# pairlab/SlotFormer

Hardware: AMD Instinct MI355X
Metric: rollout frames/sec at B=32, 128x128, 7 slots, 6+50 steps (SAVi-encode + SlotFormer rollout) (higher is better)
Workload: dtype f32 storage; matmul/conv on split-bf16 MFMA (bf16x3: hi*hi+hi*lo+lo*hi, f32 accumulate)

## Files before the change

include/slotformer_hip.h:

```cpp
#ifndef SLOTFORMER_HIP_H
#define SLOTFORMER_HIP_H
#include <stddef.h>

#ifdef __cplusplus
extern "C" {
#endif

int sf_version(void);
const char* sf_last_error_string(void);

int sf_get_precision(void);
int sf_set_precision(int mode);

int sf_profile_enable(int class_mask);
int sf_set_seam_fused(int on);
int sf_get_seam_fused(void);
int sf_set_ffn_rows64(int on);
int sf_get_ffn_rows64(void);
int sf_profile_sample(int every);
int sf_profile_read(int kernel_class, double* total_ms, long long* launches, double* work);


int sf_linear_f32(const float* A, int lda, const float* W, const float* bias, const float* ln_gamma,
                  const float* ln_beta, float ln_eps, const float* residual, int ldr, float* C, int ldc,
// ... 76 lines not shown
int sf_rle_label_maps(const unsigned* run_ends, const int* object_offsets, const int* frame_offsets, const void* tables, long long* labels_i64,
                      unsigned char* labels_u8, int* extents, int F, int num_objects, int num_runs, int h, int w, int H, int W, void* stream);
int sf_rle_boxes_pad(const int* extents, float* bbox, unsigned char* pres_mask, unsigned* flag, int F, int num, void* stream);

enum { SF_EGRESS_TRUNC = 0, SF_EGRESS_NEAREST_EVEN = 1 };
enum { SF_EGRESS_F32_CHW = 0, SF_EGRESS_U8_CHW = 1, SF_EGRESS_U8_HWC = 2 };
enum { SF_EGRESS_IMG = 0, SF_EGRESS_SLOTS = 1, SF_EGRESS_IDS = 2 };
int sf_egress_frames_u8(const float* x, unsigned char* out, long long F, int H, int W, int hwc, int to_rgb, int rounding, void* stream);
typedef struct {
  int kind;
  int N;
  const void* a;
  const void* b;
  float scale;
  int ids_i64;
  int P;
  int history_len;
} sf_egress_tile;
int sf_egress_grid_shape(int K, int H, int W, int nrow, int padding, int border, int* CH, int* CW);
int sf_egress_grid(const sf_egress_tile* tiles, int n_entries, void* out, int out_mode, int T, int H, int W, int nrow, int padding,
                   float pad_value, int border, void* stream);
int sf_egress_draw_boxes(unsigned char* frames, const float* boxes, const unsigned char* pres, const unsigned char* palette, int P, int F, int M,
                         int H, int W, int width, void* stream);

int sf_pos_embed_table_f32(const float* grid, const float* dense_w, const float* dense_b, float* table, int HW,
                           int C, void* stream);

int sf_slot_attn_num_partials(int HW);
int sf_slot_attn_iter_f32(const float* k, const float* v, int ld, long long batch_stride, const float* q,
                          float* part_num, float* part_den, float* attn_out, int B, int HW, int N, int D,
                          float scale, float eps, void* stream);
int sf_slot_attn_iter_planes_f32(const void* planes, long long batch_stride_rows, const float* q, float* part_num, float* part_den,
                                 float* attn_out, long long attn_batch_stride, int B, int HW, int N, float scale, float eps, void* stream);
int sf_slot_prologue_f32(const float* prev, const float* init, const float* pm_ln_g, const float* pm_ln_b, const float* pm_w0_t,
                         const float* pm_b0, const float* pm_w2_t, const float* pm_b2, int norm_first, const float* kd_w_t,
                         const float* kd_b, const float* noise, long long noise_bs, float* kdist_out, long long kdist_bs,
                         const float* q_ln_g, const float* q_ln_b, const float* q_w_t, float* slots_out, float* q_out, int B, int N,
                         int D, float ln_eps, void* stream);

int sf_slot_attn_iter_bf16(const void* k, const void* v, int ld, long long batch_stride, const float* q, float* part_num,
                           float* part_den, float* attn_out, int B, int HW, int N, int D, float scale, float eps, void* stream);
int sf_set_slot_attn_tile16(int on);
int sf_get_slot_attn_tile16(void);

size_t sf_slot_attn_iter_bwd_workspace_bytes(int B, int HW, int N, int D);
int sf_slot_attn_iter_bwd_f32(const float* k, const float* v, int ld, long long batch_stride, const float* q,
                              const float* part_num, const float* part_den, int P, const float* d_updates, float* dk,
                              float* dv, int accumulate, float* dq, int B, int HW, int N, int D, float scale, float eps,
                              void* ws, size_t ws_bytes, void* stream);
size_t sf_slot_attn_iter_bwd16_workspace_bytes(int B, int HW, int N, int D);
int sf_slot_attn_iter_bwd16_f32(const float* k, const float* v, int ld, long long batch_stride, const float* q,
                                const float* part_num, const float* part_den, int P, const float* d_updates, float* dk,
                                float* dv, int accumulate, float* dq, int B, int HW, int N, int D, float scale, float eps,
                                void* ws, size_t ws_bytes, void* stream);

int sf_slot_update_f32(const float* part_num, const float* part_den, int P, const float* slots_prev,
                       const float* gru_w_ih, const float* gru_w_hh, const float* gru_b_ih,
                       const float* gru_b_hh, const float* ln_g, const float* ln_b, const float* mlp_w1,
                       const float* mlp_b1, const float* mlp_w2, const float* mlp_b2, float* slots_out, int B,
                       int N, int D, int H, float ln_eps, void* stream);

int sf_slot_update_packed_f32(const float* part_num, const float* part_den, int P, const float* slots_prev,
                              const void* gru_ih_packed, const void* gru_hh_packed, const float* gru_b_ih,
                              const float* gru_b_hh, const float* ln_g, const float* ln_b, const void* mlp_w1_packed,
                              const float* mlp_b1, const void* mlp_w2_packed, const float* mlp_b2, float* slots_out,
                              const float* q_ln_g, const float* q_ln_b, const void* q_w_packed, float* q_out, int B, int N,
// ... 354 lines not shown
  const float *mlp_ln_g, *mlp_ln_b, *mlp_w1, *mlp_b1, *mlp_w2, *mlp_b2;
  const float* init_latents;
  int kd_mode;
  const float *kd_w0, *kd_b0, *kd_ln_g, *kd_ln_b, *kd_w3, *kd_b3;
  int pred_type;
  int pred_rnn, pred_norm_first, pred_num_layers, pred_num_heads, pred_ffn_dim, pred_hidden;
  const float *pm_ln_g, *pm_ln_b, *pm_w0, *pm_b0, *pm_w2, *pm_b2;
  const sf_tfm_layer* pred_layers;
  const float *lstm_w_ih, *lstm_w_hh, *lstm_b_ih, *lstm_b_hh, *proj_w, *proj_b;
  float sa_eps;
  const float* sa_q_w_t;
  const float *pm_w0_t, *pm_w2_t, *kd_w0_t;
  const void *sa_gru_ih_p, *sa_gru_hh_p, *sa_mlp_w1_p, *sa_mlp_w2_p, *sa_q_w_p;
  const float *sa_fold_q_w, *sa_fold_q_w_t, *sa_fold_gru_ih_t;
  const void *sa_fold_q_w_p, *sa_fold_gru_ih_p;
  const void** pred_packed;
  const void *enc_fc1_p, *enc_fc2_p;
  const void* conv_w_frag[8];
  const void *pm_w0_p, *pm_w2_p, *kd_w0_p;
} sf_savi_encoder;

size_t sf_savi_encode_workspace_bytes(const sf_savi_encoder* m, int B);
int sf_savi_encode_f32(const sf_savi_encoder* m, const float* img, const float* noise, const float* prev_slots,
                       float* lstm_h, float* lstm_c, int state_valid, float* post_slots, float* kernel_dist,
                       float* attn, int B, int T, void* ws, size_t ws_bytes, void* stream);

size_t sf_savi_cnn_workspace_bytes(const sf_savi_encoder* m, int B);
int sf_savi_cnn_f32(const sf_savi_encoder* m, const float* img, int B, int T, int t0, int t1, float* feat, void* ws,
                    size_t ws_bytes, void* stream);
int sf_savi_encode_pre_f32(const sf_savi_encoder* m, const float* img, const float* feat_pre, int n_pre, const float* noise,
                           const float* prev_slots, float* lstm_h, float* lstm_c, int state_valid, float* post_slots,
                           float* kernel_dist, float* attn, int B, int T, void* ws, size_t ws_bytes, void* stream);
size_t sf_savi_encode_fork_workspace_bytes(const sf_savi_encoder* m, int B, int T);
size_t sf_savi_encode_batched_workspace_bytes(const sf_savi_encoder* m, int B, int T);
int sf_set_encode_fuse_next(int on);
int sf_get_encode_fuse_next(void);
int sf_set_slot_chain(int on);
int sf_get_slot_chain(void);
int sf_set_slot_attn_planes(int on);
int sf_get_slot_attn_planes(void);
int sf_set_pixel_tok(int on);
int sf_get_pixel_tok(void);
int sf_savi_chain_ok(const sf_savi_encoder* m, int B, int T);
size_t sf_savi_planes_bytes(const sf_savi_encoder* m, int B, int T);
size_t sf_savi_features_workspace_bytes(const sf_savi_encoder* m, int B, int T);
int sf_savi_features_planes_f32(const sf_savi_encoder* m, const float* img, int B, int T, void* planes, void* ws, size_t ws_bytes, void* stream);
size_t sf_savi_slots_chain_workspace_bytes(const sf_savi_encoder* m, int videos);
int sf_savi_slots_chain_f32(const sf_savi_encoder* m, const void* planes, const float* noise, const float* prev_slots, float* post, long long post_bs,
                            float* kernel_dist, float* attn, int NB, int B, int T, void* ws, size_t ws_bytes, void* stream);
int sf_savi_encode_fork_f32(const sf_savi_encoder* m, const float* img, const float* feat_pre, int n_pre, const float* noise,
                            const float* prev_slots, float* lstm_h, float* lstm_c, int state_valid, float* post_slots,
                            float* kernel_dist, float* attn, int B, int T, void* ws, size_t ws_bytes, void* stream, void* side_stream);

typedef struct {
  int resolution;
  int dec_layers;
  int dec_channels[9];
  int dec_strides[8];
  int dec_ks, dec_res;
  int num_slots, slot_size;
  const float* deconv_w[8];
  const float* deconv_b[8];
  const float *out_w, *out_b;
  const float* pos_table;
  const float* deconv_w_flipped[8];
  const void* deconv_w_frag[8];
  const float* l0_weff;
  const float* l0_posterm;
} sf_savi_decoder;

size_t sf_savi_decode_workspace_bytes(const sf_savi_decoder* m, int F);
int sf_savi_decode_f32(const sf_savi_decoder* m, const float* slots, float* recon_combined, float* recons,
                       float* masks, int F, void* ws, size_t ws_bytes, void* stream);
int sf_savi_decode_seg_f32(const sf_savi_decoder* m, const float* slots, float* recon_combined, float* recons, float* masks,
                           long long* seg_i64, unsigned char* seg_u8, float fg_thre, int F, void* ws, size_t ws_bytes, void* stream);
// ... 78 lines not shown
```

slotformer_amd/_lib.py:

```python
import ctypes as C
import os

_HERE = os.path.dirname(os.path.abspath(__file__))
LIB_PATH = os.environ.get('SF_LIB_PATH') or os.path.join(_HERE, 'libslotformer_hip.so')

FP = C.c_void_p


class sf_tfm_layer(C.Structure):
    _fields_ = [(n, FP) for n in (
        'norm1_g', 'norm1_b', 'in_proj_w', 'in_proj_b', 'out_proj_w', 'out_proj_b',
        'norm2_g', 'norm2_b', 'lin1_w', 'lin1_b', 'lin2_w', 'lin2_b', 'lin1_packed', 'lin2_packed', 'attn_in_packed', 'attn_out_packed', 'tok_packed')]


class sf_rollouter(C.Structure):
    _fields_ = [(n, C.c_int) for n in (
        'num_slots', 'slot_size', 'd_model', 'num_layers', 'num_heads', 'ffn_dim', 'norm_first',
        'window_len', 'single_step')] + [(n, FP) for n in (
            'in_proj_w', 'in_proj_b', 'out_proj_w', 'out_proj_b', 'pe_tok')] + [
                ('layers', C.POINTER(sf_tfm_layer)), ('in_proj_packed', C.c_void_p), ('out_proj_packed', C.c_void_p)]


class sf_aloe(C.Structure):
    _fields_ = [(n, C.c_int) for n in ('num_slots', 'slot_size', 'T', 'text_len', 'question_len', 'd_model', 'num_heads', 'ffn_dim', 'num_layers',
# ... 53 lines not shown
        ('conv_w', FP * 8), ('conv_b', FP * 8)] + [(n, FP) for n in ('pos_grid', 'pos_w', 'pos_b', 'ln_g', 'ln_b', 'fc1_w', 'fc1_b',
                                                                      'fc2_w', 'fc2_b')]


class sf_savi_features_grads(C.Structure):
    _fields_ = [('conv_w', FP * 8), ('conv_b', FP * 8)] + [(n, FP) for n in ('pos_w', 'pos_b', 'ln_g', 'ln_b', 'fc1_w', 'fc1_b',
                                                                              'fc2_w', 'fc2_b')]


class sf_savi_encoder(C.Structure):
    _fields_ = (
        [('resolution', C.c_int), ('enc_layers', C.c_int), ('enc_channels', C.c_int * 9),
         ('enc_ks', C.c_int)] +
        [(n, C.c_int) for n in ('enc_out_channels', 'num_slots', 'slot_size', 'slot_mlp_size',
                                'num_iterations')] +
        [('conv_w', FP * 8), ('conv_b', FP * 8), ('pos_table', FP)] +
        [(n, FP) for n in ('enc_ln_g', 'enc_ln_b', 'enc_fc1_w', 'enc_fc1_b', 'enc_fc2_w', 'enc_fc2_b',
                           'sa_norm_in_g', 'sa_norm_in_b', 'sa_q_ln_g', 'sa_q_ln_b', 'sa_q_w', 'sa_kv_w',
                           'gru_w_ih', 'gru_w_hh', 'gru_b_ih', 'gru_b_hh',
                           'mlp_ln_g', 'mlp_ln_b', 'mlp_w1', 'mlp_b1', 'mlp_w2', 'mlp_b2',
                           'init_latents')] +
        [('kd_mode', C.c_int)] +
        [(n, FP) for n in ('kd_w0', 'kd_b0', 'kd_ln_g', 'kd_ln_b', 'kd_w3', 'kd_b3')] +
        [(n, C.c_int) for n in ('pred_type', 'pred_rnn', 'pred_norm_first', 'pred_num_layers',
                                'pred_num_heads', 'pred_ffn_dim', 'pred_hidden')] +
        [(n, FP) for n in ('pm_ln_g', 'pm_ln_b', 'pm_w0', 'pm_b0', 'pm_w2', 'pm_b2')] +
        [('pred_layers', C.POINTER(sf_tfm_layer))] +
        [(n, FP) for n in ('lstm_w_ih', 'lstm_w_hh', 'lstm_b_ih', 'lstm_b_hh', 'proj_w', 'proj_b')] +
        [('sa_eps', C.c_float), ('sa_q_w_t', FP), ('pm_w0_t', FP), ('pm_w2_t', FP), ('kd_w0_t', FP),
         ('sa_gru_ih_p', C.c_void_p), ('sa_gru_hh_p', C.c_void_p), ('sa_mlp_w1_p', C.c_void_p), ('sa_mlp_w2_p', C.c_void_p),
         ('sa_q_w_p', C.c_void_p), ('sa_fold_q_w', FP), ('sa_fold_q_w_t', FP), ('sa_fold_gru_ih_t', FP), ('sa_fold_q_w_p', C.c_void_p),
         ('sa_fold_gru_ih_p', C.c_void_p), ('pred_packed', C.POINTER(C.c_void_p)), ('enc_fc1_p', C.c_void_p), ('enc_fc2_p', C.c_void_p),
         ('conv_w_frag', C.c_void_p * 8), ('pm_w0_p', C.c_void_p), ('pm_w2_p', C.c_void_p), ('kd_w0_p', C.c_void_p)])


class sf_slate_block(C.Structure):
    _fields_ = [(n, FP) for n in ('ln1_g', 'ln1_b', 'wqkv', 'wo', 'ln2_g', 'ln2_b', 'wq_c', 'wkv_c', 'wo_c', 'ln3_g', 'ln3_b',
                                  'w1', 'b1', 'w2', 'b2')] + [('is_first', C.c_int)]


class sf_slate_decoder(C.Structure):
    _fields_ = [(n, C.c_int) for n in ('d_model', 'num_heads', 'num_layers', 'vocab_size', 'num_slots', 'max_len')] + [
        (n, FP) for n in ('in_proj_w', 'in_proj_b', 'tok_emb', 'pos_emb', 'lnf_g', 'lnf_b', 'head_w')] + [
            ('blocks', C.POINTER(sf_slate_block))]


class sf_savi_decoder(C.Structure):
    _fields_ = ([('resolution', C.c_int), ('dec_layers', C.c_int), ('dec_channels', C.c_int * 9),
                 ('dec_strides', C.c_int * 8), ('dec_ks', C.c_int), ('dec_res', C.c_int), ('num_slots', C.c_int),
                 ('slot_size', C.c_int), ('deconv_w', FP * 8), ('deconv_b', FP * 8), ('out_w', FP), ('out_b', FP),
                 ('pos_table', FP), ('deconv_w_flipped', FP * 8), ('deconv_w_frag', C.c_void_p * 8), ('l0_weff', FP), ('l0_posterm', FP)])


class sf_egress_tile(C.Structure):
    _fields_ = [('kind', C.c_int), ('N', C.c_int), ('a', C.c_void_p), ('b', C.c_void_p), ('scale', C.c_float), ('ids_i64', C.c_int), ('P', C.c_int),
                ('history_len', C.c_int)]


class sf_lpips_model(C.Structure):
    _fields_ = [('conv_w', C.c_void_p * 13), ('conv_b', FP * 13), ('lin_w', FP * 5), ('shift', FP), ('scale', FP)]


I, LL, F32, SZ, VP = C.c_int, C.c_longlong, C.c_float, C.c_size_t, C.c_void_p

SIGNATURES = {
    'sf_version': (I, []),
# ... 31 lines not shown
    'sf_decode_combine_f32': (I, [FP, FP, FP, FP, I, I, I, VP]),
    'sf_savi_decode_workspace_bytes': (SZ, [C.POINTER(sf_savi_decoder), I]),
    'sf_savi_decode_f32': (I, [C.POINTER(sf_savi_decoder), FP, FP, FP, FP, I, VP, SZ, VP]),
    'sf_savi_decode_seg_f32': (I, [C.POINTER(sf_savi_decoder), FP, FP, FP, FP, VP, VP, F32, I, VP, SZ, VP]),
    'sf_decode_combine_seg_f32': (I, [FP, FP, FP, FP, VP, VP, F32, VP, I, I, I, VP]),
    'sf_postproc_mask_f32': (I, [FP, VP, VP, F32, VP, I, I, I, VP]),
    'sf_vp_metrics_workspace_bytes': (SZ, [I, I, I]),
    'sf_vp_image_metrics_f32': (I, [FP, FP, VP, VP, VP, I, I, I, I, VP, SZ, VP]),
    'sf_vp_mask_metrics': (I, [VP, VP, I, VP, FP, VP, VP, VP, VP, I, I, I, I, VP, SZ, VP]),
    'sf_vp_bbox_pr_f32': (I, [FP, VP, FP, VP, VP, I, I, I, F32, VP]),
    'sf_masks_to_boxes': (I, [VP, I, FP, VP, I, I, I, I, VP]),
    'sf_vp_mean_over_videos_f64': (I, [VP, VP, I, I, I, VP]),
    'sf_lpips_pack_conv_weights': (I, [FP, VP, I, I, VP]),
    'sf_lpips_pack_conv_weights_host': (I, [VP, VP, I, I]),
    'sf_lpips_workspace_bytes': (SZ, [I, I, I]),
    'sf_lpips_f32': (I, [C.POINTER(sf_lpips_model), FP, FP, FP, I, I, I, I, I, VP, SZ, VP]),
    'sf_lpips_mean_over_videos_f32': (I, [FP, VP, VP, I, I, VP]),
    'sf_ingest_tables_bytes': (SZ, [I, I, I, I, I]),
    'sf_ingest_tables_host': (I, [VP, SZ, I, I, I, I, I]),
    'sf_ingest_frames_u8': (I, [VP, VP, I, VP, FP, FP, FP, I, I, I, I, I, I, I, VP]),
    'sf_resize_masks_nearest': (I, [VP, I, VP, VP, VP, I, I, I, I, I, VP]),
    'sf_rle_label_maps': (I, [VP, VP, VP, VP, VP, VP, VP, I, I, I, I, I, I, I, VP]),
    'sf_rle_boxes_pad': (I, [VP, FP, VP, VP, I, I, VP]),
    'sf_egress_frames_u8': (I, [FP, VP, LL, I, I, I, I, I, VP]),
    'sf_egress_grid_shape': (I, [I, I, I, I, I, I, C.POINTER(I), C.POINTER(I)]),
    'sf_egress_grid': (I, [C.POINTER(sf_egress_tile), I, VP, I, I, I, I, I, I, F32, I, VP]),
    'sf_egress_draw_boxes': (I, [VP, FP, VP, VP, I, I, I, I, I, I, VP]),
    'sf_pos_embed_table_f32': (I, [FP, FP, FP, FP, I, I, VP]),
    'sf_slot_attn_num_partials': (I, [I]),
    'sf_slot_attn_iter_f32': (I, [FP, FP, I, LL, FP, FP, FP, FP, I, I, I, I, F32, F32, VP]),
    'sf_slot_update_f32': (I, [FP, FP, I, FP] + [FP] * 10 + [FP, I, I, I, I, F32, VP]),
    'sf_slot_update_packed_f32': (I, [FP, FP, I, FP, VP, VP, FP, FP, FP, FP, VP, FP, VP, FP, FP, FP, FP, VP, FP, I, I, I, I, F32, VP]),
    'sf_slot_attn_iter_planes_f32': (I, [VP, LL, FP, FP, FP, FP, LL, I, I, I, F32, F32, VP]),
    'sf_slot_prologue_f32': (I, [FP] * 8 + [I, FP, FP, FP, LL, FP, LL, FP, FP, FP, FP, FP, I, I, I, F32, VP]),
    'sf_slot_update_packed_next_f32': (I, [FP, FP, I, FP, VP, VP, FP, FP, FP, FP, VP, FP, VP, FP, FP, FP, FP, VP, FP, I, I, I, I, F32,
                                           FP, LL, I, FP, FP, VP, FP, VP, FP, I, VP, FP, FP, LL, FP, LL, FP, VP]),
    'sf_mha_f32': (I, [FP, FP, I, I, I, I, I, VP]),
    'sf_qkv_attention_f32': (I, [FP, FP, FP, F32, FP, FP, FP, I, I, I, I, I, VP]),
    'sf_lstm_pointwise_f32': (I, [FP, FP, FP, FP, I, I, VP]),
    'sf_sample_dist_f32': (I, [FP, FP, FP, I, I, VP]),
    'sf_bilinear_resize_f32': (I, [FP, FP, LL, I, I, I, I, VP]),
    'sf_rollout_workspace_bytes': (SZ, [C.POINTER(sf_rollouter), I]),
    'sf_rollout_f32': (I, [C.POINTER(sf_rollouter), FP, I, I, I, VP, SZ, VP]),
    'sf_rollout_opts_f32': (I, [C.POINTER(sf_rollouter), FP, I, I, I, VP, SZ, VP, C.POINTER(sf_rollout_opts)]),
    'sf_rollout_phases_workspace_bytes': (SZ, [C.POINTER(sf_rollouter), I, I]),
    'sf_rollout_phases_f32': (I, [C.POINTER(sf_rollouter), FP, I, I, I, I, I, VP, SZ, VP, C.POINTER(sf_rollout_opts)]),
    'sf_rollout_uses_seam': (I, [C.POINTER(sf_rollouter), I]),
    'sf_rollout_uses_seam_opts': (I, [C.POINTER(sf_rollouter), I, C.POINTER(sf_rollout_opts)]),
    'sf_rollout_is_fused': (I, [C.POINTER(sf_rollouter)]),
    'sf_rollout_tok_ok': (I, [C.POINTER(sf_rollouter)]),
    'sf_rollout_tok_layers': (I, [C.POINTER(sf_rollouter), I, C.POINTER(sf_rollout_opts)]),
    'sf_ffn_chunk_partials_f32': (I, [C.POINTER(sf_tfm_layer), FP, LL, FP, LL, I, I, I, VP]),
    'sf_attn_block_f32': (I, [C.POINTER(sf_tfm_layer), FP, FP, I, I, I, I, VP]),
    'sf_ffn_block_rows_f32': (I, [C.POINTER(sf_tfm_layer), FP, FP, I, I, VP]),
    'sf_set_layer_tok': (I, [I]),
    'sf_get_layer_tok': (I, []),
    'sf_layer_tok_packed_bytes': (SZ, []),
    'sf_layer_tok_packed_bytes_ex': (SZ, [I, I, I]),
    'sf_pack_layer_tok_weights': (I, [C.POINTER(sf_tfm_layer), VP, I, I, I, VP]),
    'sf_layer_tok_block_f32': (I, [C.POINTER(sf_tfm_layer), I, FP, FP, I, I, VP]),
    'sf_layer_tok_block_ex_f32': (I, [C.POINTER(sf_tfm_layer), I, I, I, I, FP, FP, I, I, VP]),
    'sf_debug_read_ts_layer_tok': (I, [C.POINTER(C.c_longlong)]),
    'sf_attn_rows_planes_bytes': (SZ, [I]),
    'sf_attn_block_rows_f32': (I, [C.POINTER(sf_tfm_layer), FP, FP, VP, I, I, I, VP]),
    'sf_slot_attn_iter_bwd_workspace_bytes': (SZ, [I, I, I, I]),
    'sf_slot_attn_iter_bwd_f32': (I, [FP, FP, I, LL, FP, FP, FP, I, FP, FP, FP, I, FP, I, I, I, I, F32, F32, VP, SZ, VP]),
# ... 83 lines not shown
    'sf_head_ce_bwd_f32': (I, [FP, LL, VP, VP, VP, FP, I, FP, FP, FP, LL, LL, I, I, VP]),
    'sf_physion_readout_ok': (I, [I, I, I]),
    'sf_physion_readout_fwd_f32': (I, [FP, LL, LL, I, VP, FP, FP, FP, FP, FP, VP, FP, VP, I, I, I, I, I, I, I, VP]),
    'sf_physion_readout_bwd_workspace_bytes': (SZ, [I, I, I]),
    'sf_physion_readout_bwd_f32': (I, [FP, LL, LL, I, VP, FP, FP, FP, FP, VP, VP, FP, FP, FP, FP, I, I, I, I, I, I, VP, SZ, VP]),
    'sf_physion_readout_score_f32': (I, [FP, FP, VP, C.POINTER(F32), I, I, FP, FP, VP, VP, I, I, VP]),
    'sf_phyre_readout_ok': (I, [I, I, I, I, I, I, I]),
    'sf_phyre_readout_workspace_bytes': (SZ, [I, I, I]),
    'sf_phyre_readout_fwd_f32': (I, [FP, LL, LL, I, I, VP, C.POINTER(C.c_int), FP, FP, FP, FP, C.POINTER(sf_tfm_layer), I, I, I, I, FP, FP, FP, FP, FP,
                                     FP, VP, FP, LL, I, I, I, I, VP, SZ, VP]),
    'sf_phyre_auccess_f32': (I, [FP, VP, VP, I, I, VP]),
    'sf_phyre_readout_train_workspace_bytes': (SZ, [C.POINTER(sf_phyre_readout_model), I, I]),
    'sf_phyre_readout_train_fwd_f32': (I, [C.POINTER(sf_phyre_readout_model), FP, LL, LL, I, I, VP, C.POINTER(C.c_int), I, I, F32, C.c_ulonglong, FP,
                                           VP, VP, VP, SZ, VP]),
    'sf_phyre_readout_train_bwd_f32': (I, [C.POINTER(sf_phyre_readout_model), FP, LL, LL, I, I, VP, C.POINTER(C.c_int), I, I, FP,
                                           C.POINTER(sf_phyre_readout_grads), F32, C.c_ulonglong, VP, SZ, VP]),
    'sf_aloe_ok': (I, [I, I, I, I, I, I, I, I]),
    'sf_aloe_workspace_bytes': (SZ, [I, I, I, I, I, I]),
    'sf_aloe_text_table_f32': (I, [FP, FP, FP, FP, I, I, I, VP]),
    'sf_aloe_fwd_f32': (I, [C.POINTER(sf_aloe), FP, LL, LL, I, I, VP, VP, I, VP, VP, I, FP, FP, FP, FP, I, I, FP, VP, I, VP, SZ, VP]),
    'sf_aloe_score_f32': (I, [FP, VP, I, I, FP, FP, VP, I, VP, I, FP, VP, VP, VP]),
    'sf_packed_linear_bytes': (SZ, [I, I]),
    'sf_pack_linear_weights': (I, [FP, VP, I, I, VP]),
    'sf_attn_packed_bytes': (SZ, [I, I]),
    'sf_pack_attn_weights': (I, [FP, FP, VP, VP, I, I, VP]),
    'sf_ffn_packed_bytes': (SZ, [I, I]),
    'sf_pack_ffn_weights': (I, [FP, FP, VP, VP, I, I, VP]),
    'sf_savi_cnn_workspace_bytes': (SZ, [C.POINTER(sf_savi_encoder), I]),
    'sf_savi_cnn_f32': (I, [C.POINTER(sf_savi_encoder), FP, I, I, I, I, FP, VP, SZ, VP]),
    'sf_savi_encode_pre_f32': (I, [C.POINTER(sf_savi_encoder), FP, FP, I, FP, FP, FP, FP, I, FP, FP, FP, I, I, VP, SZ,
                                   VP]),
    'sf_savi_encode_fork_workspace_bytes': (SZ, [C.POINTER(sf_savi_encoder), I, I]),
    'sf_savi_encode_batched_workspace_bytes': (SZ, [C.POINTER(sf_savi_encoder), I, I]),
    'sf_set_encode_fuse_next': (I, [I]),
    'sf_get_encode_fuse_next': (I, []),
    'sf_set_slot_chain': (I, [I]),
    'sf_get_slot_chain': (I, []),
    'sf_set_slot_attn_planes': (I, [I]),
    'sf_get_slot_attn_planes': (I, []),
    'sf_set_pixel_tok': (I, [I]),
    'sf_get_pixel_tok': (I, []),
    'sf_savi_chain_ok': (I, [C.POINTER(sf_savi_encoder), I, I]),
    'sf_savi_planes_bytes': (SZ, [C.POINTER(sf_savi_encoder), I, I]),
    'sf_savi_features_workspace_bytes': (SZ, [C.POINTER(sf_savi_encoder), I, I]),
    'sf_savi_features_planes_f32': (I, [C.POINTER(sf_savi_encoder), FP, I, I, VP, VP, SZ, VP]),
    'sf_savi_slots_chain_workspace_bytes': (SZ, [C.POINTER(sf_savi_encoder), I]),
    'sf_savi_slots_chain_f32': (I, [C.POINTER(sf_savi_encoder), VP, FP, FP, FP, LL, FP, FP, I, I, I, VP, SZ, VP]),
    'sf_savi_encode_fork_f32': (I, [C.POINTER(sf_savi_encoder), FP, FP, I, FP, FP, FP, FP, I, FP, FP, FP, I, I, VP, SZ,
                                    VP, VP]),
    'sf_kv_producer_workspace_bytes': (SZ, [I, I]),
    'sf_kv_producer_f32': (I, [FP] * 11 + [I, I, I, I, F32, VP, SZ, VP]),
    'sf_device_alloc': (I, [C.POINTER(VP), SZ]),
    'sf_device_free': (I, [VP]),
    'sf_device_upload': (I, [VP, VP, SZ]),
    'sf_device_download': (I, [VP, VP, SZ]),
    'sf_device_synchronize': (I, []),
    'sf_stream_create_cu_mask': (I, [C.POINTER(VP), C.POINTER(C.c_uint), I]),
    'sf_stream_cus': (I, [VP]),
    'sf_stream_set_cus': (I, [VP, I]),
    'sf_debug_spin': (I, [I, VP]),
    'sf_debug_clock_probe': (I, [I, VP, VP]),
    'sf_stream_destroy': (I, [VP]),
    'sf_slot_attn_iter_f32_host': (I, [FP, FP, I, LL, FP, FP, FP, FP, I, I, I, I, F32, F32, VP]),
    'sf_rollout_f32_host': (I, [C.POINTER(sf_rollouter), FP, I, I, I, VP, SZ, VP]),
    'sf_savi_encode_f32_host': (I, [C.POINTER(sf_savi_encoder), FP, FP, FP, FP, FP, I, FP, FP, FP, I, I, VP, SZ,
                                    VP]),
    'sf_savi_decode_f32_host': (I, [C.POINTER(sf_savi_decoder), FP, FP, FP, FP, I, VP, SZ, VP]),
    'sf_seam_timeouts': (I, []),
    'sf_slot_attn_iter_bf16': (I, [VP, VP, I, LL, FP, FP, FP, FP, I, I, I, I, F32, F32, VP]),
    'sf_rollout_bf16': (I, [C.POINTER(sf_rollouter), FP, I, I, I, VP, SZ, VP]),
    'sf_rollout_bf16_host': (I, [C.POINTER(sf_rollouter), FP, I, I, I, VP, SZ, VP]),
    'sf_slot_update_f32_host': (I, [FP, FP, I, FP] + [FP] * 10 + [FP, I, I, I, I, F32, VP]),
    'sf_kv_producer_f32_host': (I, [FP] * 11 + [I, I, I, I, F32, VP, SZ, VP]),
}
# ... 99 lines not shown
```

slotformer_amd/csrc/conv_first.hip:

```cpp
#include "sf_internal.h"

namespace {
constexpr int CF_NT = 512, CF_CO = 64, CF_CI = 3, CF_KS = 5, CF_K = CF_CI * CF_KS * CF_KS, CF_KP = 80;
constexpr int CF_TW = 64, CF_TR = 2;
constexpr int CF_PP = CF_KP + 8;

template <int STRIDE>
struct CfGeo {
  static constexpr int HR = (CF_TR - 1) * STRIDE + CF_KS;
  static constexpr int HC = (CF_TW - 1) * STRIDE + CF_KS;
  static constexpr int HCP = (HC + 3) / 4 * 4 + 4;
  static constexpr size_t lds = (size_t)(CF_CI * HR * HCP + 4) * 4 + (size_t)2 * (CF_TR * CF_TW + CF_CO) * CF_PP * 2;
};

}

#ifndef CF_WPS
#define CF_WPS 4
#endif
template <int STRIDE>
__global__ __launch_bounds__(CF_NT, CF_WPS) void conv_first_kernel(const float* __restrict__ img, long long frame_stride,
                                                           const float* __restrict__ w, const float* __restrict__ bias,
                                                           const float* __restrict__ add, float* __restrict__ out, int Ho,
                                                           int Hin, int Win, int relu, int fgroup, long long group_stride, int ntiles) {
  using G = CfGeo<STRIDE>;
  constexpr int HR = G::HR, HC = G::HC, HCP = G::HCP;
  constexpr int NH = (CF_CI * HR * HC + CF_NT - 1) / CF_NT;
  extern __shared__ __attribute__((aligned(16))) float smem[];
  float* In = smem;
  constexpr int ZERO = CF_CI * HR * HCP;
  __bf16* Ah = (__bf16*)(In + ZERO + 4);
  __bf16* Al = Ah + CF_TR * CF_TW * CF_PP;
  __bf16* Wh = Al + CF_TR * CF_TW * CF_PP;
  __bf16* Wl = Wh + CF_CO * CF_PP;
  const int t = threadIdx.x, lane = t & 63, wave = t >> 6;
  const int tiles = Ho / CF_TR;
  if (t < 4) In[ZERO + t] = 0.f;

  for (int idx = t; idx < CF_CO * (CF_KP / 4); idx += CF_NT) {
    const int co = idx / (CF_KP / 4), k4 = idx - co * (CF_KP / 4);
    f32x4 v;
#pragma unroll
    for (int e = 0; e < 4; ++e) {
      const int k = 4 * k4 + e;
      v[e] = k < CF_K ? w[co * CF_K + k] : 0.f;
    }
    sf_split4(Wh, Wl, co * CF_PP + 4 * k4, v);
  }
  const int p = t & 127, kg = t >> 7;
  unsigned poff[10];
  {
    const int prow = p >> 6, x = p & 63;
#pragma unroll
    for (int q = 0; q < 10; ++q) {
      unsigned pr[2];
#pragma unroll
      for (int e = 0; e < 2; ++e) {
        const int k = kg * 20 + 2 * q + e;
// ... 47 lines not shown
    if (tile + (int)gridDim.x < ntiles) fetch(tile + gridDim.x);
#pragma unroll
    for (int q = 0; q < 5; ++q) {
      f32x4 v;
#pragma unroll
      for (int e = 0; e < 4; ++e) v[e] = In[(poff[2 * q + (e >> 1)] >> (16 * (e & 1))) & 0xffffu];
      sf_split4(Ah, Al, p * CF_PP + kg * 20 + 4 * q, v);
    }
    __syncthreads();
    f32x16 acc;
#pragma unroll
    for (int r = 0; r < 16; ++r) acc[r] = 0.f;
#pragma unroll
    for (int ks = 0; ks < CF_KP / 16; ++ks) {
      const bf16x8 xh = *(const bf16x8*)(Ah + ao + ks * 16), xl = *(const bf16x8*)(Al + ao + ks * 16);
      const bf16x8 yh = *(const bf16x8*)(Wh + bo + ks * 16), yl = *(const bf16x8*)(Wl + bo + ks * 16);
      acc = __builtin_amdgcn_mfma_f32_32x32x16_bf16(xl, yh, acc, 0, 0, 0);
      acc = __builtin_amdgcn_mfma_f32_32x32x16_bf16(xh, yl, acc, 0, 0, 0);
      acc = __builtin_amdgcn_mfma_f32_32x32x16_bf16(xh, yh, acc, 0, 0, 0);
    }
    const int f = tile / tiles, y = (tile % tiles) * CF_TR + row;
#pragma unroll
    for (int r = 0; r < 16; ++r) {
      const int px = pxb + (r & 3) + 8 * (r >> 2) + 4 * (lane >> 5);
      float v = fmaxf(acc[r] + bv, lo);
      if (add) v += add[((long long)y * CF_TW + px) * CF_CO + co];
      out[(((long long)f * Ho + y) * CF_TW + px) * CF_CO + co] = v;
    }
  }
}

template <int STRIDE>
static int launch_cf(const float* img, long long frame_stride, const float* w, const float* bias, const float* add,
                     float* out, int F, int Ho, int Hin, int Win, int relu, int fgroup, long long group_stride, hipStream_t st) {
  auto kern = conv_first_kernel<STRIDE>;
  constexpr size_t lds = CfGeo<STRIDE>::lds;
  static_assert(lds <= 80 * 1024, "first conv: two workgroups per CU");
  SF_TRY(sf_ensure_dyn_lds((const void*)kern, (size_t)(lds)));
  sf_prof_begin(SF_K_CONV_FIRST, st, 2.0 * (double)F * Ho * CF_TW * CF_CO * CF_K);
  const int ntiles = F * (Ho / CF_TR);
  int grid = (CF_WPS / 2) * sf_stream_cus((void*)st);
  if (grid > ntiles) grid = ntiles;
  if (grid < 1) grid = 1;
  hipLaunchKernelGGL(kern, dim3(grid), dim3(CF_NT), lds, st, img, frame_stride, w, bias, add, out, Ho, Hin, Win, relu, fgroup, group_stride, ntiles);
  sf_prof_end(SF_K_CONV_FIRST, st);
  SF_CHECK_LAUNCH();
  return 0;
}

int sf_conv_first_ex(const float* img, long long frame_stride, const float* w, const float* bias, const float* add,
                     float* out, int F, int Cin, int Hin, int Win, int Cout, int ks, int stride, int relu, hipStream_t st) {
  return sf_conv_first_grouped_ex(img, frame_stride, F > 0 ? F : 1, 0, w, bias, add, out, F, Cin, Hin, Win, Cout, ks, stride, relu, st);
}
int sf_conv_first_grouped_ex(const float* img, long long frame_stride, int fgroup, long long group_stride, const float* w, const float* bias,
                             const float* add, float* out, int F, int Cin, int Hin, int Win, int Cout, int ks, int stride, int relu, hipStream_t st) {
  if (Cin != CF_CI || Cout != CF_CO || ks != CF_KS || F <= 0 || fgroup <= 0) return 1;
  if (stride == 2 && Hin == 128 && Win == 128) return launch_cf<2>(img, frame_stride, w, bias, add, out, F, 64, Hin, Win, relu, fgroup, group_stride, st);
  if (stride == 1 && Hin == 64 && Win == 64) return launch_cf<1>(img, frame_stride, w, bias, add, out, F, 64, Hin, Win, relu, fgroup, group_stride, st);
  return 1;
}

extern "C" int sf_conv2d_nchw_in_grouped_f32(const float* img, long long frame_stride, int fgroup, long long group_stride, const float* weight,
                                             const float* bias, const float* add, float* out, int F, int Cin, int Hin, int Win, int Cout, int ks,
                                             int stride, int relu, void* stream) {
  SF_REQUIRE(img && weight && out, "sf_conv2d_nchw_in_grouped_f32: null pointer");
  SF_REQUIRE(sf_get_precision() >= 1, "sf_conv2d_nchw_in_grouped_f32: split-bf16 mode only");
  const int rc = sf_conv_first_grouped_ex(img, frame_stride, fgroup, group_stride, weight, bias, add, out, F, Cin, Hin, Win, Cout, ks, stride, relu,
                                          (hipStream_t)stream);
  SF_REQUIRE(rc != 1, "sf_conv2d_nchw_in_grouped_f32: 3 -> 64 channels, 5 x 5, 64 x 64 at stride 1 or 128 x 128 at stride 2, F >= 1, fgroup >= 1");
  return rc;
}
```

slotformer_amd/csrc/engine.hip:

```cpp
#include "../../include/slotformer_hip.h"
#include "sf_internal.h"
#include "sf_arena.h"
#include <map>
#include <vector>
#include "layer_fused.h"
#include "slot_chain.h"
#include <stdlib.h>

namespace {

inline bool plain_gemms(const SfThreadOpts& o) { return o.precision == 2 || o.precision == 3; }

struct TfmWs {
  float *x2, *qkv, *att, *hid, *y;
};

bool tfm_ws_take(SfArena& bp, TfmWs& w, int M, int d, int ffn) {
  w.x2 = bp.take((size_t)M * d);
  w.qkv = bp.take((size_t)M * 3 * d);
  w.att = bp.take((size_t)M * d);
  w.hid = bp.take((size_t)M * ffn);
  w.y = bp.take((size_t)M * d);
  return bp.ok;
}
// ... 489 lines not shown

}

namespace {
int enc_chunk(int B) { return B < 32 ? B : 32; }
constexpr int ENC_FORK_AHEAD = 4;
int enc_fork_steps(int T) { return T < 2 ? 2 : (T < ENC_FORK_AHEAD ? T : ENC_FORK_AHEAD); }
constexpr int ENC_HW = 64 * 64;

int enc_cmax(const sf_savi_encoder* m) {
  int cmax = 0;
  for (int i = 1; i <= m->enc_layers && i < 9; ++i) cmax = m->enc_channels[i] > cmax ? m->enc_channels[i] : cmax;
  return cmax;
}
void enc_cnn_take(SfArena& bp, float** buf, int n, const sf_savi_encoder* m, size_t frames) {
  for (int i = 0; i < n; ++i) buf[i] = bp.take(frames * ENC_HW * enc_cmax(m));
}

struct SlotRows { float *a, *b, *lat, *q; };
void slot_rows_take(SfArena& bp, SlotRows& r, size_t rows, int D) {
  for (float** f : {&r.a, &r.b, &r.lat, &r.q}) *f = bp.take(rows * D);
}

struct EncodePlan {
  bool fork = false;
  int KV = 2;
  int n_pre = 0;
  bool batched = false;
  enum Feat { KV_GEMMS, KV_FUSED, FOLD_ROWS, FOLD_192, FOLD_PLANES } feat = KV_GEMMS;
  const float *q_w = nullptr, *q_w_t = nullptr, *gru_ih_t = nullptr;
  const void *q_w_p = nullptr, *gru_ih_p = nullptr;
  enum Update { VALU, WIDE, MFMA } update = VALU;
  int p_step = 1;
  bool pred_step = false;
  bool prologue = false;
  bool fuse_next = false;
  bool chain_model = false;
  bool chain = false;
  bool fold() const { return feat >= FOLD_ROWS; }
};

struct EncodeWs {
  float* feat[2];
  float *h1, *h2;
  float* kv;
  SlotRows rows;
  float *lnbuf, *px;
  float *kdist, *kdtmp;
  float *pnum, *pden;
  TfmWs tw;
  float* gates;
  float* big[3];
  float* planes;
};

bool enc_ws_take(SfArena& bp, EncodeWs& w, const sf_savi_encoder* m, int B, int T, const EncodePlan& p) {
  const int N = m->num_slots, D = m->slot_size, Ce = m->enc_out_channels, P = sf_sa_pick_partials(ENC_HW);
  const size_t R = (size_t)B * N, Bc = enc_chunk(B), HW = ENC_HW;
  enc_cnn_take(bp, w.feat, 2, m, Bc);
  w.h1 = bp.take(Bc * HW * Ce);
  w.h2 = bp.take(Bc * HW * Ce);
  w.kv = bp.take((size_t)p.KV * B * HW * 2 * D);
  slot_rows_take(bp, w.rows, R, D);
  w.lnbuf = bp.take(R * D);
  w.px = bp.take(R * D);
  w.kdist = bp.take(R * 2 * D);
// ... 14 lines not shown
  return bp.bytes() + 8192;
}

bool enc_batched_ok(const sf_savi_encoder* m, int B, int T, int precision) {
  if (T < 2 || B > enc_chunk(B) || (long long)B * T > 384 || m->enc_layers < 2 || precision != 1) return false;
  for (int i = 1; i < m->enc_layers; ++i)
    if (!m->conv_w_frag[i] || m->enc_channels[i] != 64 || m->enc_channels[i + 1] != 64) return false;
  return true;
}

EncodePlan plan_encode(const sf_savi_encoder* m, int B, int T, int n_pre, bool fork, size_t ws_bytes) {
  EncodePlan p;
  p.fork = fork;
  p.KV = fork ? enc_fork_steps(T) : 2;
  p.n_pre = n_pre;
  if (!m || m->enc_layers < 1 || m->enc_layers > 8) return p;
  const int precision = sf_get_precision();
  const int HW = ENC_HW, N = m->num_slots, D = m->slot_size, Ce = m->enc_out_channels, Hm = m->slot_mlp_size, P = sf_sa_pick_partials(HW);
  const int Cl = m->enc_channels[m->enc_layers];
  const bool feat192 = Cl == 64 && Ce == 192 && m->enc_fc1_p && m->enc_fc2_p;
  const bool fold = precision >= 1 && m->sa_fold_q_w && m->sa_fold_q_w_t && m->sa_fold_gru_ih_t && Ce == D && (sf_pixel_mlp_feat_ok(Cl, Ce) || feat192);
  const bool planes = fold && !feat192 && sf_switch(SF_SW_SLOT_ATTN_PLANES) && sf_slot_attn_planes_ok(HW, D, N) && Cl == 64 && P == HW / 256;
  p.feat = fold ? (feat192 ? EncodePlan::FOLD_192 : planes ? EncodePlan::FOLD_PLANES : EncodePlan::FOLD_ROWS)
                : (precision >= 1 ? EncodePlan::KV_FUSED : EncodePlan::KV_GEMMS);
  p.q_w = fold ? m->sa_fold_q_w : m->sa_q_w;
  p.q_w_t = fold ? m->sa_fold_q_w_t : m->sa_q_w_t;
  p.gru_ih_t = fold ? m->sa_fold_gru_ih_t : m->gru_w_ih;
  p.q_w_p = fold ? m->sa_fold_q_w_p : m->sa_q_w_p;
  p.gru_ih_p = fold ? m->sa_fold_gru_ih_p : m->sa_gru_ih_p;
  const bool su_packed = precision >= 1 && p.gru_ih_p && m->sa_gru_hh_p && m->sa_mlp_w1_p && m->sa_mlp_w2_p && p.q_w_p;
  p.update = !su_packed ? EncodePlan::VALU : sf_slot_update_mfma_ok(D, Hm, P) ? EncodePlan::MFMA
            : sf_slot_update_wide_ok(D, Hm, P) ? EncodePlan::WIDE : EncodePlan::VALU;
  if (fold && P == HW / 256 && (planes || sf_slot_attn_sparse_records_n(nullptr, nullptr, HW, D, N))) p.p_step = 2;
  p.pred_step = m->pred_type == 1 && m->pred_packed && precision >= 1;
  p.prologue = m->pred_type == 0 && !m->pred_rnn && m->kd_mode == 1 && m->pm_w0_t && m->pm_w2_t && m->kd_w0_t && p.q_w_t;
  p.fuse_next = p.prologue && p.update == EncodePlan::MFMA && m->pm_w0_p && m->pm_w2_p && m->kd_w0_p && m->pm_ln_g && m->pm_ln_b && m->pm_b0 &&
                m->pm_b2 && m->kd_b0 && sf_switch(SF_SW_ENCODE_FUSE_NEXT);
  p.chain_model = precision == 1 && fold && p.feat != EncodePlan::FOLD_192 && p.update == EncodePlan::MFMA && p.fuse_next &&
                  sf_slot_chain_ok(D, Hm, HW, N) && m->init_latents && m->enc_fc1_w && m->enc_fc2_w;
  p.batched = !fork && n_pre == 0 && enc_batched_ok(m, B, T, precision);
  p.chain = p.batched && p.chain_model && sf_switch(SF_SW_SLOT_CHAIN);
  if (p.chain && ws_bytes < enc_ws_bytes(m, B, T, p)) p.chain = false;
  if (p.batched && ws_bytes < enc_ws_bytes(m, B, T, p)) p.batched = false;
  return p;
}

int run_cnn_layers(const sf_savi_encoder* m, const float* src, long long frame_stride, int nb, float* dst, float* featA, float* featB,
                   int i0, int i1, hipStream_t st) {
  const int res = m->resolution;
  for (int i = i0; i < i1; ++i) {
    const bool lastc = (i == m->enc_layers - 1);
    const int cin = m->enc_channels[i], cout = m->enc_channels[i + 1];
    const float* add = lastc ? m->pos_table : nullptr;
    float* out = lastc ? dst : ((i & 1) ? featB : featA);
    const float* cur = i == 0 ? nullptr : (((i - 1) & 1) ? featB : featA);
    if (i == 0) {
      SF_TRY(sf_conv2d_nchw_in_f32(src, frame_stride, m->conv_w[0], m->conv_b[0], add, out, nb, cin, res, res, cout,
                                   m->enc_ks, res == 128 ? 2 : 1, lastc ? 0 : 1, st));
    } else {
      int rc = 1;
      if (rc == 1 && m->conv_w_frag[i])
        rc = sf_conv5x5_ws_ex(cur, m->conv_w_frag[i], m->conv_b[i], add, out, nb, 64, 64, cin, cout, m->enc_ks, lastc ? 0 : 1, 0, st);
      if (rc == 1 && m->conv_w_frag[i])
        rc = sf_conv5x5_rows4_ex(cur, m->conv_w_frag[i], m->conv_b[i], add, out, nb, 64, 64, cin, cout, m->enc_ks, lastc ? 0 : 1, st);
      if (rc < 0 || rc > 1) return rc;
      if (rc == 1)
        SF_TRY(sf_conv2d_nhwc_f32(cur, m->conv_w[i], m->conv_b[i], add, out, nb, 64, 64, cin, cout, m->enc_ks, lastc ? 0 : 1, st));
    }
  }
  return 0;
}

int enc_cnn_all_steps(const sf_savi_encoder* m, const float* img, int B, int T, float* const* big, hipStream_t st) {
  const int res = m->resolution, c1 = m->enc_channels[1];
  const long long frame_elems = (long long)3 * res * res;
  const int rc = sf_conv_first_grouped_ex(img, (long long)T * frame_elems, B, frame_elems, m->conv_w[0], m->conv_b[0], nullptr, big[0], B * T,
                                          m->enc_channels[0], res, res, c1, m->enc_ks, res == 128 ? 2 : 1, 1, st);
  if (rc < 0 || rc > 1) return rc;
  for (int t = 0; t < T && rc == 1; ++t)
    SF_TRY(sf_conv2d_nchw_in_f32(img + (long long)t * frame_elems, (long long)T * frame_elems, m->conv_w[0], m->conv_b[0], nullptr,
                                 big[0] + (long long)t * B * ENC_HW * c1, B, m->enc_channels[0], res, res, c1, m->enc_ks, res == 128 ? 2 : 1, 1, st));
  return run_cnn_layers(m, nullptr, 0, B * T, big[2], big[0], big[1], 1, m->enc_layers, st);
}

int enc_feature_planes(const sf_savi_encoder* m, const float* img, int B, int T, float* const* big, void* planes, hipStream_t st) {
  SF_TRY(enc_cnn_all_steps(m, img, B, T, big, st));
  return sf_pixel_mlp_feat_planes_ex(big[2], m->enc_ln_g, m->enc_ln_b, m->enc_fc1_w, m->enc_fc1_b, m->enc_fc2_w, m->enc_fc2_b, m->sa_norm_in_g, m->sa_norm_in_b,
                                     planes, B * T * ENC_HW, 1e-5f, st);
}
int enc_slots_chain(const sf_savi_encoder* m, const void* planes, const float* noise, const float* prev, float* post, long long post_bs, float* kernel_dist,
                    float* attn, int NB, int B, int T, const SlotRows& r, hipStream_t st) {
  const int N = m->num_slots, D = m->slot_size;
  const float ln_eps = 1e-5f;
  const int pr = sf_slot_prologue_ex(prev, m->init_latents, m->pm_ln_g, m->pm_ln_b, m->pm_w0_t, m->pm_b0, m->pm_w2_t, m->pm_b2, m->pred_norm_first, m->kd_w0_t,
                                     m->kd_b0, noise, (long long)T * N * D, kernel_dist, (long long)T * N * 2 * D, m->sa_q_ln_g, m->sa_q_ln_b, m->sa_fold_q_w_t,
                                     r.a, r.q, NB * B, N, D, ln_eps, st);
  if (pr != 0) return pr < 0 ? pr : sf_set_err(-1, "the one-launch slot prologue does not apply to this model", __FILE__, __LINE__);
  SfChainWeights cw;
  cw.gru_ih_p = m->sa_fold_gru_ih_p; cw.gru_hh_p = m->sa_gru_hh_p; cw.gru_b_ih = m->gru_b_ih; cw.gru_b_hh = m->gru_b_hh; cw.ln_g = m->mlp_ln_g; cw.ln_b = m->mlp_ln_b;
  cw.w1_p = m->sa_mlp_w1_p; cw.b1 = m->mlp_b1; cw.w2_p = m->sa_mlp_w2_p; cw.b2 = m->mlp_b2; cw.q_ln_g = m->sa_q_ln_g; cw.q_ln_b = m->sa_q_ln_b; cw.q_w_p = m->sa_fold_q_w_p;
  cw.pm_ln_g = m->pm_ln_g; cw.pm_ln_b = m->pm_ln_b; cw.pm_w0_p = m->pm_w0_p; cw.pm_b0 = m->pm_b0; cw.pm_w2_p = m->pm_w2_p; cw.pm_b2 = m->pm_b2;
  cw.pm_norm_first = m->pred_norm_first; cw.kd_w_p = m->kd_w0_p; cw.kd_b = m->kd_b0;
  return sf_slot_chain_ex(planes, NB, B, T, ENC_HW, N, m->num_iterations, 1.0f / sqrtf((float)D), m->sa_eps, ln_eps, r.a, r.b, r.lat, r.q, post, post_bs, attn,
                          noise, kernel_dist, &cw, st);
}

hipEvent_t enc_fork_event(int i) {
  thread_local std::map<int, std::vector<hipEvent_t>> per_dev;
  int dev = 0;
  if (hipGetDevice(&dev) != hipSuccess) return nullptr;
  std::vector<hipEvent_t>& ev = per_dev[dev];
  while ((int)ev.size() <= i) {
    hipEvent_t e = nullptr;
    if (hipEventCreateWithFlags(&e, hipEventDisableTiming) != hipSuccess) return nullptr;
    ev.push_back(e);
  }
  return ev[i];
}
int enc_fork_record(int i, hipStream_t s) {
  const hipEvent_t e = enc_fork_event(i);
  SF_REQUIRE(e != nullptr, "hipEventCreate failed");
  return hipEventRecord(e, s) == hipSuccess ? 0 : sf_set_err((int)hipGetLastError(), "hipEventRecord", __FILE__, __LINE__);
}
int enc_fork_wait(int i, hipStream_t s) {
  return hipStreamWaitEvent(s, enc_fork_event(i), 0) == hipSuccess ? 0 : sf_set_err((int)hipGetLastError(), "hipStreamWaitEvent", __FILE__, __LINE__);
}

struct EncodeArgs {
  const sf_savi_encoder* m;
  const float *img, *feat_pre, *noise;
  float *lstm_h, *lstm_c, *post, *kernel_dist, *attn;
  int B, T;
};

int enc_step_features(const EncodeArgs& a, const EncodePlan& p, const EncodeWs& w, int t, float* kv, hipStream_t st) {
  const sf_savi_encoder* m = a.m;
  const int HW = ENC_HW, B = a.B, Bc = enc_chunk(B), Cl = m->enc_channels[m->enc_layers], Ce = m->enc_out_channels, D = m->slot_size;
  const long long frame_elems = (long long)3 * m->resolution * m->resolution;
  const float ln_eps = 1e-5f;
  for (int b0 = 0; b0 < B; b0 += Bc) {
    const int nb = (B - b0 < Bc) ? (B - b0) : Bc, Mp = nb * HW;
    const float* cur;
    if (t < p.n_pre) {
      cur = a.feat_pre + ((long long)t * B + b0) * HW * Cl;
    } else if (p.batched) {
      cur = w.big[2] + ((long long)t * B + b0) * HW * Cl;
    } else {
      float* dstf = (m->enc_layers & 1) ? w.feat[0] : w.feat[1];
      SF_TRY(run_cnn_layers(m, a.img + ((long long)b0 * a.T + t) * frame_elems, (long long)a.T * frame_elems, nb, dstf, w.feat[0], w.feat[1], 0,
                            m->enc_layers, st));
      cur = dstf;
    }
    if (p.feat == EncodePlan::FOLD_192) {
      SF_TRY(sf_pixel_mlp_feat192_ex(cur, m->enc_ln_g, m->enc_ln_b, m->enc_fc1_p, m->enc_fc1_b, m->enc_fc2_p, m->enc_fc2_b,
                                     m->sa_norm_in_g, m->sa_norm_in_b, kv + (long long)b0 * HW * Ce, Mp, ln_eps, st));
    } else if (p.feat == EncodePlan::FOLD_PLANES) {
      SF_TRY(sf_pixel_mlp_feat_planes_ex(cur, m->enc_ln_g, m->enc_ln_b, m->enc_fc1_w, m->enc_fc1_b, m->enc_fc2_w, m->enc_fc2_b, m->sa_norm_in_g, m->sa_norm_in_b,
                                         (char*)kv + (size_t)b0 * HW * 512, Mp, ln_eps, st));
    } else if (p.feat == EncodePlan::FOLD_ROWS) {
      SF_TRY(sf_pixel_mlp_feat_ex(cur, m->enc_ln_g, m->enc_ln_b, m->enc_fc1_w, m->enc_fc1_b, m->enc_fc2_w, m->enc_fc2_b,
                                  m->sa_norm_in_g, m->sa_norm_in_b, kv + (long long)b0 * HW * Ce, Mp, ln_eps, st));
    } else {
      float* kv_dst = kv + (long long)b0 * HW * 2 * D;
      int rc = 1;
      if (p.feat == EncodePlan::KV_FUSED)
// ... 32 lines not shown
                        w.tw.hid, sf_rows(2 * D), R, 2 * D, D, 1, st));
    SF_TRY(sf_linear_ex(w.tw.hid, sf_rows(2 * D), m->pm_w2, m->pm_b2, nullptr, nullptr, ln_eps,
                        m->pred_norm_first ? w.lnbuf : prev, sf_rows(D), 0, w.px, sf_rows(D), R, D, 2 * D, 0, st));
    pout = w.px;
  } else {
    SF_TRY(sf_copy_rows_ex(prev, sf_rows(D), w.px, sf_rows(D), R, D, st));
    float* cur = w.px;
    TfmWs tw = w.tw;
    for (int l = 0; l < m->pred_num_layers; ++l)
      SF_TRY(tfm_layer(m->pred_layers[l], cur, tw, a.B, N, N, D, m->pred_num_heads, m->pred_ffn_dim, m->pred_norm_first, st, &cur));
    pout = cur;
  }
  *lat = m->pred_rnn ? w.rows.lat : pout;
  if (!m->pred_rnn) return 0;
  const int Hh = m->pred_hidden;
  SF_TRY(sf_linear_ex(pout, sf_rows(D), m->lstm_w_ih, m->lstm_b_ih, nullptr, nullptr, ln_eps, nullptr,
                      sf_rows(4 * Hh), 0, w.gates, sf_rows(4 * Hh), R, 4 * Hh, D, 0, st));
  SF_TRY(sf_linear_ex(a.lstm_h, sf_rows(Hh), m->lstm_w_hh, m->lstm_b_hh, nullptr, nullptr, ln_eps, w.gates,
                      sf_rows(4 * Hh), 0, w.gates, sf_rows(4 * Hh), R, 4 * Hh, Hh, 0, st));
  SF_TRY(sf_lstm_pointwise_ex(w.gates, a.lstm_c, a.lstm_h, a.lstm_c, R, Hh, st));
  return sf_linear_ex(a.lstm_h, sf_rows(Hh), m->proj_w, m->proj_b, nullptr, nullptr, ln_eps, nullptr,
                      sf_rows(D), 0, w.rows.lat, sf_rows(D), R, D, Hh, 0, st);
}

int enc_slot_init(const EncodeArgs& a, const EncodePlan& p, const EncodeWs& w, const float* prev, int t, hipStream_t st, bool* one_launch) {
  const sf_savi_encoder* m = a.m;
  const int N = m->num_slots, D = m->slot_size, R = a.B * N, T = a.T;
  const float ln_eps = 1e-5f;
  int rc = 1;
  if (p.prologue)
    rc = sf_slot_prologue_ex(prev, m->init_latents, m->pm_ln_g, m->pm_ln_b, m->pm_w0_t, m->pm_b0, m->pm_w2_t, m->pm_b2, m->pred_norm_first, m->kd_w0_t,
                             m->kd_b0, a.noise ? a.noise + (long long)t * N * D : nullptr, (long long)T * N * D,
                             a.kernel_dist ? a.kernel_dist + (long long)t * N * 2 * D : nullptr, (long long)T * N * 2 * D, m->sa_q_ln_g, m->sa_q_ln_b,
                             p.q_w_t, w.rows.a, w.rows.q, a.B, N, D, ln_eps, st);
  *one_launch = rc == 0;
  if (rc != 1) return rc;
  const float* lat;
  SF_TRY(enc_predict(a, p, w, prev, st, &lat));
  if (m->kd_mode == 0) {
    SF_TRY(sf_copy_rows_ex(lat, sf_rows(D), w.rows.a, sf_rows(D), R, D, st));
  } else {
    SF_TRY(sf_linear_ex(lat, sf_rows(D), m->kd_w0, m->kd_b0, nullptr, nullptr, ln_eps, nullptr, sf_rows(2 * D), 0,
                        m->kd_mode == 1 ? w.kdist : w.kdtmp, sf_rows(2 * D), R, 2 * D, D, 0, st));
    if (m->kd_mode == 2)
      SF_TRY(sf_linear_ex(w.kdtmp, sf_rows(2 * D), m->kd_w3, m->kd_b3, m->kd_ln_g, m->kd_ln_b, ln_eps, nullptr,
                          sf_rows(2 * D), 0, w.kdist, sf_rows(2 * D), R, 2 * D, 2 * D, 0, st, 1));
    const SfRowMap nmap = sf_rows_batched(D, N, (long long)T * N * D, (long long)t * N * D);
    SF_TRY(sf_sample_dist_ex(w.kdist, a.noise, nmap, w.rows.a, R, D, st));
    if (a.kernel_dist)
      SF_TRY(sf_copy_rows_ex(w.kdist, sf_rows(2 * D), a.kernel_dist, sf_rows_batched(2 * D, N, (long long)T * N * 2 * D, (long long)t * N * 2 * D), R,
                             2 * D, st));
  }
  return sf_linear_ex(w.rows.a, sf_rows(D), p.q_w, nullptr, m->sa_q_ln_g, m->sa_q_ln_b, ln_eps, nullptr, sf_rows(D), 0, w.rows.q, sf_rows(D), R, D, D, 0, st);
}

int enc_iterations(const EncodeArgs& a, const EncodePlan& p, const EncodeWs& w, const float* kv, int t, bool next, hipStream_t st, const float** out) {
  const sf_savi_encoder* m = a.m;
  const int HW = ENC_HW, N = m->num_slots, D = m->slot_size, Hm = m->slot_mlp_size, Ce = m->enc_out_channels, T = a.T, B = a.B, P = sf_sa_pick_partials(HW);
  const float ln_eps = 1e-5f, scale = 1.0f / sqrtf((float)D);
  const long long attn_bs = (long long)T * N * HW, post_bs = (long long)T * N * D;
  float *s_in = w.rows.a, *s_out = w.rows.b;
  for (int it = 0; it < m->num_iterations; ++it) {
    const bool last_it = (it == m->num_iterations - 1), nx_on = next && last_it;
    float* aout = (a.attn && last_it) ? a.attn + (long long)t * N * HW : nullptr;
    float* post = last_it ? a.post + (long long)t * N * D : nullptr;
    if (p.feat == EncodePlan::FOLD_PLANES)
      SF_TRY(sf_slot_attn_planes_ex(kv, HW, w.rows.q, w.pnum, w.pden, aout, attn_bs, B, HW, N, scale, m->sa_eps, st));
    else if (p.fold())
      SF_TRY(sf_slot_attn_iter_ex(kv, kv, Ce, (long long)HW * Ce, w.rows.q, w.pnum, w.pden, aout, attn_bs, B, HW, N, D, scale, m->sa_eps, st));
    else
      SF_TRY(sf_slot_attn_iter_ex(kv, kv + D, 2 * D, (long long)HW * 2 * D, w.rows.q, w.pnum, w.pden, aout, attn_bs, B, HW, N, D, scale, m->sa_eps, st));
    if (p.update == EncodePlan::MFMA) {
      SfNextStep nx;
      nx.pm_ln_g = m->pm_ln_g; nx.pm_ln_b = m->pm_ln_b; nx.pm_w0_p = m->pm_w0_p; nx.pm_b0 = m->pm_b0; nx.pm_w2_p = m->pm_w2_p; nx.pm_b2 = m->pm_b2;
      nx.norm_first = m->pred_norm_first; nx.kd_w_p = m->kd_w0_p; nx.kd_b = m->kd_b0;
      nx.noise = a.noise ? a.noise + (long long)(t + 1) * N * D : nullptr; nx.noise_bs = (long long)T * N * D;
      nx.kdist_out = a.kernel_dist ? a.kernel_dist + (long long)(t + 1) * N * 2 * D : nullptr; nx.kdist_bs = (long long)T * N * 2 * D;
      nx.slots = w.rows.a;
      SF_TRY(sf_slot_update_mfma_ex(w.pnum, w.pden, P, s_in, p.gru_ih_p, m->sa_gru_hh_p, m->gru_b_ih, m->gru_b_hh, m->mlp_ln_g, m->mlp_ln_b,
                                    m->sa_mlp_w1_p, m->mlp_b1, m->sa_mlp_w2_p, m->mlp_b2, (nx_on && s_out == w.rows.a) ? w.rows.lat : s_out, post, post_bs,
                                    m->sa_q_ln_g, m->sa_q_ln_b, p.q_w_p, (last_it && !nx_on) ? nullptr : w.rows.q, B, N, ln_eps, st, nx_on ? &nx : nullptr,
                                    p.p_step));
    } else if (p.update == EncodePlan::WIDE) {
      SF_TRY(sf_slot_update_wide_ex(w.pnum, w.pden, P, s_in, p.gru_ih_p, m->sa_gru_hh_p, m->gru_b_ih, m->gru_b_hh, m->mlp_ln_g, m->mlp_ln_b,
                                    m->sa_mlp_w1_p, m->mlp_b1, m->sa_mlp_w2_p, m->mlp_b2, s_out, post, post_bs, m->sa_q_ln_g, m->sa_q_ln_b,
                                    p.q_w_p, last_it ? nullptr : w.rows.q, B, N, ln_eps, st));
    } else {
      SF_TRY(sf_slot_update_ex(w.pnum, w.pden, P, s_in, p.gru_ih_t, m->gru_w_hh, m->gru_b_ih, m->gru_b_hh, m->mlp_ln_g, m->mlp_ln_b, m->mlp_w1,
                               m->mlp_b1, m->mlp_w2, m->mlp_b2, s_out, post, post_bs, m->sa_q_ln_g, m->sa_q_ln_b, p.q_w_t,
                               (last_it || !p.q_w_t) ? nullptr : w.rows.q, B, N, D, Hm, ln_eps, st));
      if (!last_it && !p.q_w_t)
        SF_TRY(sf_linear_ex(s_out, sf_rows(D), p.q_w, nullptr, m->sa_q_ln_g, m->sa_q_ln_b, ln_eps, nullptr, sf_rows(D), 0, w.rows.q,
                            sf_rows(D), B * N, D, D, 0, st));
    }
    std::swap(s_in, s_out);
  }
  *out = s_in;
  return 0;
}
}

extern "C" {

size_t sf_savi_encode_workspace_bytes(const sf_savi_encoder* m, int B) {
  return (m && B > 0) ? enc_ws_bytes(m, B, 1, plan_encode(m, B, 1, 0, false, 0)) : 0;
}
size_t sf_savi_encode_fork_workspace_bytes(const sf_savi_encoder* m, int B, int T) {
  return (m && B > 0 && T >= 1) ? enc_ws_bytes(m, B, T, plan_encode(m, B, T, 0, true, 0)) : 0;
}
size_t sf_savi_encode_batched_workspace_bytes(const sf_savi_encoder* m, int B, int T) {
  return (m && B > 0 && T > 0) ? enc_ws_bytes(m, B, T, plan_encode(m, B, T, 0, false, ~(size_t)0)) : 0;
}

size_t sf_savi_cnn_workspace_bytes(const sf_savi_encoder* m, int B) {
  if (!m || B <= 0) return 0;
// ... 57 lines not shown
  SlotRows r;
  slot_rows_take(bp, r, (size_t)videos * m->num_slots, m->slot_size);
  return bp.bytes() + 4096;
}
int sf_savi_slots_chain_f32(const sf_savi_encoder* m, const void* planes, const float* noise, const float* prev_slots, float* post, long long post_bs,
                            float* kernel_dist, float* attn, int NB, int B, int T, void* ws, size_t ws_bytes, void* stream) {
  SF_REQUIRE(m && planes && post && ws, "sf_savi_slots_chain_f32: null pointer");
  SF_REQUIRE(NB >= 1 && B >= 1 && T >= 1 && plan_encode(m, B, T, 0, false, 0).chain_model,
             "sf_savi_slots_chain_f32: the video-stationary slot branch does not apply (sf_savi_chain_ok)");
  SF_REQUIRE(noise == nullptr || m->kd_mode != 0, "noise given but the model has no kernel_dist layer");
  SF_REQUIRE(ws_bytes >= sf_savi_slots_chain_workspace_bytes(m, NB * B), "workspace too small");
  SfArena bp(ws, ws_bytes);
  SlotRows r;
  slot_rows_take(bp, r, (size_t)NB * B * m->num_slots, m->slot_size);
  if (!bp.ok) return sf_set_err(-1, "workspace too small", __FILE__, __LINE__);
  return enc_slots_chain(m, planes, noise, prev_slots, post, post_bs, kernel_dist, attn, NB, B, T, r, (hipStream_t)stream);
}

int sf_savi_encode_f32(const sf_savi_encoder* m, const float* img, const float* noise, const float* prev_slots,
                       float* lstm_h, float* lstm_c, int state_valid, float* post_slots, float* kernel_dist,
                       float* attn, int B, int T, void* ws, size_t ws_bytes, void* stream) {
  return sf_savi_encode_pre_f32(m, img, nullptr, 0, noise, prev_slots, lstm_h, lstm_c, state_valid, post_slots, kernel_dist,
                                attn, B, T, ws, ws_bytes, stream);
}

int sf_savi_encode_pre_f32(const sf_savi_encoder* m, const float* img, const float* feat_pre, int n_pre, const float* noise,
                           const float* prev_slots, float* lstm_h, float* lstm_c, int state_valid, float* post_slots,
                           float* kernel_dist, float* attn, int B, int T, void* ws, size_t ws_bytes, void* stream) {
  return sf_savi_encode_fork_f32(m, img, feat_pre, n_pre, noise, prev_slots, lstm_h, lstm_c, state_valid, post_slots, kernel_dist, attn,
                                 B, T, ws, ws_bytes, stream, nullptr);
}


int sf_savi_encode_fork_f32(const sf_savi_encoder* m, const float* img, const float* feat_pre, int n_pre, const float* noise,
                            const float* prev_slots, float* lstm_h, float* lstm_c, int state_valid, float* post_slots,
                            float* kernel_dist, float* attn, int B, int T, void* ws, size_t ws_bytes, void* stream, void* side_stream) {
  SF_REQUIRE(m && img && post_slots && ws, "null pointer");
  SF_REQUIRE(n_pre >= 0 && n_pre <= T && (n_pre == 0 || feat_pre != nullptr), "bad precomputed-feature arguments");
  SF_REQUIRE(B >= 1 && T >= 1, "bad batch / clip length");
  SF_REQUIRE(m->resolution == 64 || m->resolution == 128, "resolution must be 64 or 128 (savi.py:226,236)");
  SF_REQUIRE(m->enc_layers >= 1 && m->enc_layers <= 8 && m->enc_channels[0] > 0 && (m->enc_ks & 1), "bad CNN config");
  SF_REQUIRE(m->num_slots >= 1 && m->num_slots <= 16 && m->num_iterations >= 1, "bad slot config (1 <= num_slots <= 16)");
  SF_REQUIRE(m->pos_table && m->enc_ln_g && m->enc_ln_b && m->enc_fc1_w && m->enc_fc1_b && m->enc_fc2_w &&
                 m->enc_fc2_b && m->sa_norm_in_g && m->sa_norm_in_b && m->sa_q_ln_g && m->sa_q_ln_b &&
                 m->sa_q_w && m->sa_kv_w && m->init_latents, "null encoder weight");
  SF_REQUIRE(m->kd_mode >= 0 && m->kd_mode <= 2, "bad kd_mode");
  SF_REQUIRE(m->kd_mode == 0 || (m->kd_w0 && m->kd_b0), "null kernel_dist weight");
  SF_REQUIRE(m->kd_mode != 2 || (m->kd_ln_g && m->kd_ln_b && m->kd_w3 && m->kd_b3), "null kernel_dist weight");
  SF_REQUIRE(noise == nullptr || m->kd_mode != 0, "noise given but the model has no kernel_dist layer");
  if (m->pred_type == 0)
    SF_REQUIRE(m->pm_ln_g && m->pm_ln_b && m->pm_w0 && m->pm_b0 && m->pm_w2 && m->pm_b2, "null predictor weight");
  else
    SF_REQUIRE(check_layers(m->pred_layers, m->pred_num_layers) == 0, "null predictor weight");
  if (m->pred_rnn)
    SF_REQUIRE(lstm_h && lstm_c && m->pred_hidden > 0 && m->lstm_w_ih && m->lstm_w_hh && m->lstm_b_ih &&
                   m->lstm_b_hh && m->proj_w && m->proj_b, "null LSTM state / weight");
  const EncodePlan p = plan_encode(m, B, T, n_pre, side_stream != nullptr && side_stream != stream, ws_bytes);
  for (int i = 0; i < m->enc_layers; ++i) SF_REQUIRE(m->conv_w[i] != nullptr, "null conv weight");
  SfArena bp(ws, ws_bytes);
  EncodeWs w;
  SF_REQUIRE(ws_bytes >= enc_ws_bytes(m, B, T, p) && enc_ws_take(bp, w, m, B, T, p), "workspace too small");
  const hipStream_t st_main = (hipStream_t)stream, st = p.fork ? (hipStream_t)side_stream : st_main;
  const EncodeArgs a{m, img, feat_pre, noise, lstm_h, lstm_c, post_slots, kernel_dist, attn, B, T};
  const int N = m->num_slots, D = m->slot_size;
  const float* prev = prev_slots;
  if (m->pred_rnn && (prev == nullptr || !state_valid)) {
    const long long nz = (long long)B * N * m->pred_hidden;
    hipLaunchKernelGGL(zero_f32_kernel, dim3((unsigned)(((nz + 3) / 4 + 255) / 256)), dim3(256), 0, st_main, lstm_h, lstm_c, nz);
    SF_CHECK_LAUNCH();
  }
  if (p.chain) {
    SF_TRY(enc_feature_planes(m, img, B, T, w.big, w.planes, st_main));
    return enc_slots_chain(m, w.planes, noise, prev, post_slots, (long long)T * N * D, kernel_dist, attn, 1, B, T, w.rows, st_main);
  }
  if (p.batched) SF_TRY(enc_cnn_all_steps(m, img, B, T, w.big, st_main));
  bool next_done = false;
  for (int t = 0; t < T; ++t) {
    float* kv = w.kv + (size_t)(t % p.KV) * B * ENC_HW * 2 * D;
    if (p.fork && t >= p.KV) SF_TRY(enc_fork_wait(T + 1 + (t - p.KV), st_main));
    SF_TRY(enc_step_features(a, p, w, t, kv, st_main));
    if (p.fork) {
      SF_TRY(enc_fork_record(t, st_main));
      SF_TRY(enc_fork_wait(t, st));
    }
    bool one_launch = next_done;
    if (!next_done) SF_TRY(enc_slot_init(a, p, w, prev, t, st, &one_launch));
    next_done = p.fuse_next && one_launch && t + 1 < T;
    SF_TRY(enc_iterations(a, p, w, kv, t, next_done, st, &prev));
    if (p.fork && t + p.KV < T) SF_TRY(enc_fork_record(T + 1 + t, st));
  }
  if (p.fork) {
    SF_TRY(enc_fork_record(T, st));
    SF_TRY(enc_fork_wait(T, st_main));
  }
  return 0;
}

static size_t dec_maxact(const sf_savi_decoder* m) {
  size_t best = (size_t)m->dec_res * m->dec_res * m->dec_channels[0];
  int size = m->dec_res;
  for (int i = 0; i < m->dec_layers && i < 8; ++i) {
    size *= m->dec_strides[i] > 0 ? m->dec_strides[i] : 1;
    const size_t a = (size_t)size * size * m->dec_channels[i + 1];
    best = a > best ? a : best;
  }
  const size_t tab = (size_t)25 * m->dec_channels[1];
  return best > tab ? best : tab;
}
// ... 108 lines not shown
```

slotformer_amd/csrc/sf_internal.h:

```cpp
#pragma once
#include "../../include/slotformer_hip.h"
#include "sf_common.h"
#include "sf_switches.h"

struct SfThreadOpts {
  int precision = -1;
  int seam = -1;
  int ffn_rows = 0;
  int attn_heads = 0;
  int attn_rows = 0;
  int ffn_tile = 0;
  int layer_tok = 0;
  int cus = 0;
};
SfThreadOpts& sf_thread_opts();
inline int sf_precision(const SfThreadOpts& o) { return o.precision < 0 ? sf_switch(SF_SW_PRECISION) : o.precision; }
inline bool sf_seam_on(const SfThreadOpts& o) { return (o.seam < 0 ? sf_switch(SF_SW_SEAM_FUSED) : o.seam) != 0; }
inline bool sf_layer_tok_on(const SfThreadOpts& o) { return (o.layer_tok == 0 ? sf_switch(SF_SW_LAYER_TOK) : o.layer_tok) > 0; }
inline int sf_ffn_rows(const SfThreadOpts& o) { return o.ffn_rows > 0 ? o.ffn_rows : (sf_switch(SF_SW_FFN_ROWS64) ? 64 : 32); }
int sf_ensure_dyn_lds(const void* kernel, size_t bytes);

int sf_linear_ex(const float* A, SfRowMap amap, const float* W, const float* bias, const float* ln_g,
                 const float* ln_b, float ln_eps, const float* res, SfRowMap rmap, int res_mod,
                 float* C, SfRowMap cmap, int M, int N, int K, int relu, hipStream_t stream, int ln_relu = 0);
// ... 4 lines not shown
int sf_mha_ex(const float* qkv, float* out, int B, int L, int Lq, int d, int nheads, hipStream_t st);
int sf_lstm_pointwise_ex(const float* gates, const float* c_prev, float* h_out, float* c_out, int R, int H,
                         hipStream_t st);
int sf_sample_dist_ex(const float* dist, const float* noise, SfRowMap nmap, float* out, int R, int D,
                      hipStream_t st);
int sf_copy_rows_ex(const float* src, SfRowMap smap, float* dst, SfRowMap dmap, int rows, int cols,
                    hipStream_t st);
int sf_sa_pick_partials(int HW);
bool sf_pixel_mlp_feat_ok(int C0, int C1);
int sf_pixel_mlp_feat192_ex(const float* x, const float* ln0_g, const float* ln0_b, const void* w1p, const float* b1, const void* w2p,
                            const float* b2, const float* ln1_g, const float* ln1_b, float* feat, int M, float eps, hipStream_t st);
int sf_pixel_mlp_feat_ex(const float* x, const float* ln0_g, const float* ln0_b, const float* w1, const float* b1, const float* w2,
                         const float* b2, const float* ln1_g, const float* ln1_b, float* feat, int M, float eps, hipStream_t st);
bool sf_slot_update_mfma_ok(int D, int H, int P);
struct SfNextStep {
  const float *pm_ln_g, *pm_ln_b;
  const void* pm_w0_p;
  const float* pm_b0;
  const void* pm_w2_p;
  const float* pm_b2;
  int norm_first;
  const void* kd_w_p;
  const float* kd_b;
  const float* noise;
  long long noise_bs;
  float* kdist_out;
  long long kdist_bs;
  float* slots;
};
int sf_slot_update_mfma_ex(const float* part_num, const float* part_den, int P, const float* slots_prev, const void* gru_ih_p,
                           const void* gru_hh_p, const float* gru_b_ih, const float* gru_b_hh, const float* ln_g, const float* ln_b,
                           const void* w1_p, const float* b1, const void* w2_p, const float* b2, float* slots_out, float* out2,
                           long long out2_bs, const float* q_ln_g, const float* q_ln_b, const void* q_w_p, float* q_out, int B, int N,
                           float ln_eps, hipStream_t st, const SfNextStep* next = nullptr, int p_step = 1);
bool sf_slot_attn_sparse_records(const float* k, const float* v, int HW, int D);
bool sf_slot_attn_sparse_records_n(const float* k, const float* v, int HW, int D, int N);
bool sf_slot_update_wide_ok(int D, int H, int P);
int sf_slot_update_wide_ex(const float* part_num, const float* part_den, int P, const float* slots_prev, const void* gru_ih_p, const void* gru_hh_p,
                           const float* gru_b_ih, const float* gru_b_hh, const float* ln_g, const float* ln_b, const void* w1_p, const float* b1,
                           const void* w2_p, const float* b2, float* slots_out, float* out2, long long out2_bs, const float* q_ln_g,
                           const float* q_ln_b, const void* q_w_p, float* q_out, int B, int N, float ln_eps, hipStream_t st);
int sf_slot_update_ex(const float* part_num, const float* part_den, int P, const float* slots_prev,
                      const float* gru_w_ih, const float* gru_w_hh, const float* gru_b_ih, const float* gru_b_hh,
                      const float* ln_g, const float* ln_b, const float* mlp_w1, const float* mlp_b1, const float* mlp_w2,
                      const float* mlp_b2, float* slots_out, float* out2, long long out2_bs, const float* q_ln_g,
                      const float* q_ln_b, const float* q_w, float* q_out, int B, int N, int D, int H, float ln_eps,
                      hipStream_t st);
int sf_slot_prologue_ex(const float* prev, const float* init, const float* pm_ln_g, const float* pm_ln_b, const float* pm_w0_t,
                        const float* pm_b0, const float* pm_w2_t, const float* pm_b2, int norm_first, const float* kd_w_t,
                        const float* kd_b, const float* noise, long long noise_bs, float* kdist_out, long long kdist_bs,
                        const float* q_ln_g, const float* q_ln_b, const float* q_w_t, float* slots_out, float* q_out, int B,
                        int N, int D, float ln_eps, hipStream_t st);
int sf_slot_attn_iter_ex(const float* k, const float* v, int ld, long long batch_stride, const float* q,
                         float* part_num, float* part_den, float* attn_out, long long attn_batch_stride, int B,
                         int HW, int N, int D, float scale, float eps, hipStream_t st);

enum { SF_K_CONV_NHWC = 0, SF_K_CONV_FIRST = 1, SF_K_LINEAR = 2, SF_K_SA_ITER = 3, SF_K_SA_UPDATE = 4,
       SF_K_MHA = 5, SF_K_FFN = 6, SF_K_SEAM = 7, SF_K_DECONV = 8, SF_K_LAYER_TOK = 9, SF_K_NUM = 10 };
void sf_prof_begin(int cls, hipStream_t st, double work);
void sf_prof_end(int cls, hipStream_t st);
void sf_prof_suppress(int on);
int sf_qkv_attn_ex(const float* x, const float* ln_g, const float* ln_b, float ln_eps, const float* in_proj_w,
                   const float* in_proj_b, float* out, int B, int L, int Lq, int d, int nheads, hipStream_t st);
int sf_conv5x5_ws_ex(const float* in, const void* w_frag, const float* bias, const float* add, float* out, int F, int H, int W, int Cin, int Cout, int ks,
                     int relu, int n_workgroups, hipStream_t st);
extern "C" int sf_stream_cus(void* stream);
int sf_dbg(const char* key);
extern "C" int sf_stream_cus_known(void* stream);
int sf_conv5x5_rows4_ex(const float* in, const void* w_frag, const float* bias, const float* add, float* out, int F, int H, int W,
                        int Cin, int Cout, int ks, int relu, hipStream_t st);
int sf_conv5x5_rows4_ohwi_ex(const float* in, const float* w_ohwi, void* w_frag, const float* bias, const float* add, float* out, int F, int H,
                             int W, int Cin, int Cout, int ks, int relu, hipStream_t st);
struct SfSlateGenWs {
  float *mem, *memkv[16], *cache[16], *x, *xn, *att, *qc, *x2, *x3, *hid, *lg;
  size_t bytes;
};
SfSlateGenWs sf_slate_gen_carve(void* ws, const sf_slate_decoder* m, int B, int steps, size_t cache_w, bool chain);
int sf_deconv5x5s2_ex(const float* in, const void* w_frag, const float* bias, const float* head_w, const float* head_b, float* out, int R,
                      int H, int W, int Cin, int Cout, int ks, int stride, int relu, hipStream_t st);
int sf_conv5x5_rows4_head_ex(const float* in, const void* w_frag, const float* bias, const float* head_w, const float* head_b, float* dec,
                             int F, int H, int W, int Cin, int Cout, int ks, hipStream_t st);
int sf_conv5x5_halo_ex(const float* in, const float* w_packed, const float* bias, const float* add, float* out, int F,
                       int H, int W, int Cin, int Cout, int ks, int relu, hipStream_t st);
int sf_pixel_mlp_kv_ex(const float* x, const float* ln0_g, const float* ln0_b, const float* w1, const float* b1,
                       const float* w2, const float* b2, const float* ln1_g, const float* ln1_b, const float* wkv,
                       float* kv, int M, int C0, int C1, int ND, float eps, hipStream_t st);

bool sf_layer_fused_ok(int d, int heads, int ffn, int L);
int sf_conv_first_grouped_ex(const float* img, long long frame_stride, int fgroup, long long group_stride, const float* w, const float* bias,
                             const float* add, float* out, int F, int Cin, int Hin, int Win, int Cout, int ks, int stride, int relu, hipStream_t st);
int sf_conv_first_ex(const float* img, long long frame_stride, const float* w, const float* bias, const float* add,
                     float* out, int F, int Cin, int Hin, int Win, int Cout, int ks, int stride, int relu, hipStream_t st);
```

slotformer_amd/csrc/sf_switches.cpp:

```cpp
#include <stdlib.h>
#include <atomic>

#include "../../include/slotformer_hip.h"
#include "sf_internal.h"

namespace {
enum Parse { NO_ENV, FLAG, PRECISION };
struct Row {
  const char* env;
  int def;
  Parse parse;
};
constexpr Row ROWS[SF_SW_NUM] = {
     {"SF_PRECISION", 1, PRECISION},
     {"SF_LAYER_TOK", 0, FLAG},
     {"SF_SEAM_FUSED", 1, FLAG},
     {nullptr, 0, NO_ENV},
     {"SF_CONV_FP16X2", 0, FLAG},
     {nullptr, 1, NO_ENV},
     {nullptr, 1, NO_ENV},
     {nullptr, 0, NO_ENV},
     {nullptr, 1, NO_ENV},
     {nullptr, 1, NO_ENV},
     {"SF_CONV_WS", 1, FLAG},
};

std::atomic<int> g_slot[SF_SW_NUM];

int initial(const Row& r) {
  const char* e = r.env ? getenv(r.env) : nullptr;
  if (!e) return r.def;
  if (r.parse == PRECISION) return (e[0] == 'f' || e[0] == '0') ? 0 : (strcmp(e, "bf16") == 0 ? 2 : 1);
  return r.def ? e[0] != '0' : e[0] == '1';
}
}

int sf_switch(SfSwitch s) {
  int v = g_slot[s].load(std::memory_order_relaxed);
  if (v == 0) {
    v = initial(ROWS[s]) + 1;
    int seen = 0;
    if (!g_slot[s].compare_exchange_strong(seen, v, std::memory_order_relaxed)) v = seen;
  }
  return v - 1;
}

int sf_switch_set(SfSwitch s, int v) {
  g_slot[s].store(v + 1, std::memory_order_relaxed);
  return 0;
}

extern "C" {
int sf_get_precision(void) { return sf_precision(sf_thread_opts()); }
int sf_set_precision(int mode) {
  if (mode < 0 || mode > 2) return sf_set_err(-1, "invalid argument: precision mode must be 0 (f32), 1 (bf16x3) or 2 (bf16)", __FILE__, __LINE__);
  return sf_switch_set(SF_SW_PRECISION, mode);
}
int sf_get_layer_tok(void) { return sf_switch(SF_SW_LAYER_TOK); }
int sf_set_layer_tok(int on) { return sf_switch_set(SF_SW_LAYER_TOK, on != 0); }
int sf_get_seam_fused(void) { return sf_switch(SF_SW_SEAM_FUSED); }
int sf_set_seam_fused(int on) { return sf_switch_set(SF_SW_SEAM_FUSED, on != 0); }
int sf_get_ffn_rows64(void) { return sf_switch(SF_SW_FFN_ROWS64); }
int sf_set_ffn_rows64(int on) { return sf_switch_set(SF_SW_FFN_ROWS64, on != 0); }
int sf_get_conv_fp16x2(void) { return sf_switch(SF_SW_CONV_FP16X2); }
int sf_set_conv_fp16x2(int on) { return sf_switch_set(SF_SW_CONV_FP16X2, on != 0); }
int sf_get_slot_attn_tile16(void) { return sf_switch(SF_SW_SLOT_ATTN_TILE16); }
int sf_set_slot_attn_tile16(int on) { return sf_switch_set(SF_SW_SLOT_ATTN_TILE16, on != 0); }
int sf_get_encode_fuse_next(void) { return sf_switch(SF_SW_ENCODE_FUSE_NEXT); }
int sf_set_encode_fuse_next(int on) { return sf_switch_set(SF_SW_ENCODE_FUSE_NEXT, on != 0); }
int sf_get_slot_chain(void) { return sf_switch(SF_SW_SLOT_CHAIN); }
int sf_set_slot_chain(int on) { return sf_switch_set(SF_SW_SLOT_CHAIN, on != 0); }
int sf_get_slot_attn_planes(void) { return sf_switch(SF_SW_SLOT_ATTN_PLANES); }
int sf_set_slot_attn_planes(int on) { return sf_switch_set(SF_SW_SLOT_ATTN_PLANES, on != 0); }
int sf_get_pixel_tok(void) { return sf_switch(SF_SW_PIXEL_TOK); }
int sf_set_pixel_tok(int on) { return sf_switch_set(SF_SW_PIXEL_TOK, on != 0); }
}
```

slotformer_amd/csrc/sf_switches.h:

```cpp
#pragma once

enum SfSwitch {
  SF_SW_PRECISION,
  SF_SW_LAYER_TOK,
  SF_SW_SEAM_FUSED,
  SF_SW_FFN_ROWS64,
  SF_SW_CONV_FP16X2,
  SF_SW_SLOT_ATTN_TILE16,
  SF_SW_ENCODE_FUSE_NEXT,
  SF_SW_SLOT_CHAIN,
  SF_SW_SLOT_ATTN_PLANES,
  SF_SW_PIXEL_TOK,
  SF_SW_CONV_WS,
  SF_SW_NUM
};

int sf_switch(SfSwitch s);
int sf_switch_set(SfSwitch s, int v);

extern "C" int sf_get_precision(void);
```

slotformer_amd/csrc/slot_attn.hip:

```cpp
#include "sf_internal.h"
#include <stdlib.h>

#define SA_NMAX 8
#define SA_NMAX16 16
#define SA_DMAX 256
#define SA_HMAX 512


template <int VPT, int NS = SA_NMAX>
__global__ __launch_bounds__(256) void sa_attn_partial_kernel(
    const float* __restrict__ k, const float* __restrict__ v, int ld, long long batch_stride,
    const float* __restrict__ q, float scale, float eps, float* __restrict__ part_num,
    float* __restrict__ part_den, float* __restrict__ attn_out, long long attn_bs, int HW, int N,
    int P) {
  constexpr int D = 64 * VPT;
  const int b = blockIdx.y, chunk = blockIdx.x;
  const int lane = threadIdx.x & 63, wave = threadIdx.x >> 6;
  const int pix_per_wg = HW / P, pix_per_wave = pix_per_wg / 4;
  const int pix0 = chunk * pix_per_wg + wave * pix_per_wave;

  float qr[NS][VPT], num[NS][VPT], den[NS];
#pragma unroll
  for (int n = 0; n < NS; ++n) {
#pragma unroll
// ... 441 lines not shown
  su_ln_stats(s_u, s_stat, D, ln_eps, wave, lane, nwaves);
  __syncthreads();
  for (int idx = t; idx < SU_R * D; idx += nt) {
    const int d = idx / SU_R, r = idx - d * SU_R;
    s_ln[idx] = (s_u[idx] - s_stat[2 * r]) * s_stat[2 * r + 1] * ex.q_ln_g[d] + ex.q_ln_b[d];
  }
  __syncthreads();
  su_gemm(ex.q_w, D, D, s_ln, s_pa, t, nt);
  __syncthreads();
  {
    const int ks = su_kslices(nt, D, D);
    for (int idx = t; idx < SU_R * D; idx += nt) {
      const int r = idx / D, d = idx - r * D;
      if (row0 + r < R) ex.q_out[(long long)(row0 + r) * D + d] = su_sum(s_pa, ks, D, d, r);
    }
  }
}

struct SpArgs {
  const float* prev;
  const float* init;
  const float *pm_ln_g, *pm_ln_b, *pm_w0_t, *pm_b0, *pm_w2_t, *pm_b2;
  int norm_first;
  const float *kd_w_t, *kd_b;
  const float* noise;
  long long noise_bs;
  float* kdist_out;
  long long kdist_bs;
  const float *q_ln_g, *q_ln_b, *q_w_t;
  float* slots_out;
  float* q_out;
};

__global__ __launch_bounds__(768) void sa_slot_prologue_kernel(SpArgs a, int R, int N, int D, int pmax, float ln_eps) {
  extern __shared__ __attribute__((aligned(16))) float su_lds[];
  const int D2 = 2 * D;
  float* s_x = su_lds;
  float* s_ln = s_x + D * SU_R;
  float* s_lat = s_ln + D * SU_R;
  float* s_hid = s_lat + D * SU_R;
  float* s_stat = s_hid + D2 * SU_R;
  float* s_pa = s_stat + 2 * SU_R;
  const int row0 = blockIdx.x * SU_R;
  const int t = threadIdx.x, lane = t & 63, wave = t >> 6, nt = blockDim.x, nwaves = nt >> 6;
  for (int idx = t; idx < SU_R * D; idx += nt) {
    const int r = idx / D, d = idx - r * D, row = row0 + r;
    float v = 0.f;
    if (row < R) v = a.prev ? a.prev[(long long)row * D + d] : a.init[(long long)(row % N) * D + d];
    s_x[d * SU_R + r] = v;
  }
  __syncthreads();
  if (a.prev) {
    su_ln_stats(s_x, s_stat, D, ln_eps, wave, lane, nwaves);
    __syncthreads();
    for (int idx = t; idx < SU_R * D; idx += nt) {
      const int d = idx / SU_R, r = idx - d * SU_R;
      s_ln[idx] = (s_x[idx] - s_stat[2 * r]) * s_stat[2 * r + 1] * a.pm_ln_g[d] + a.pm_ln_b[d];
    }
    __syncthreads();
    su_gemm(a.pm_w0_t, D2, D, s_ln, s_pa, t, nt);
    __syncthreads();
    {
      const int ks = su_kslices(nt, D2, D);
      for (int idx = t; idx < SU_R * D2; idx += nt) {
        const int j = idx / SU_R, r = idx - j * SU_R;
        s_hid[idx] = fmaxf(su_sum(s_pa, ks, D2, j, r) + a.pm_b0[j], 0.f);
      }
    }
// ... 24 lines not shown
  }
  __syncthreads();
  for (int idx = t; idx < SU_R * D; idx += nt) {
    const int r = idx / D, d = idx - r * D, row = row0 + r;
    float v = s_hid[d * SU_R + r];
    if (a.noise && row < R)
      v += a.noise[(long long)(row / N) * a.noise_bs + (long long)(row % N) * D + d] * expf(s_hid[(D + d) * SU_R + r] * 0.5f);
    s_x[d * SU_R + r] = v;
    if (row < R) a.slots_out[(long long)row * D + d] = v;
  }
  __syncthreads();
  su_ln_stats(s_x, s_stat, D, ln_eps, wave, lane, nwaves);
  __syncthreads();
  for (int idx = t; idx < SU_R * D; idx += nt) {
    const int d = idx / SU_R, r = idx - d * SU_R;
    s_ln[idx] = (s_x[idx] - s_stat[2 * r]) * s_stat[2 * r + 1] * a.q_ln_g[d] + a.q_ln_b[d];
  }
  __syncthreads();
  su_gemm(a.q_w_t, D, D, s_ln, s_pa, t, nt);
  __syncthreads();
  {
    const int ks = su_kslices(nt, D, D);
    for (int idx = t; idx < SU_R * D; idx += nt) {
      const int r = idx / D, d = idx - r * D;
      if (row0 + r < R) a.q_out[(long long)(row0 + r) * D + d] = su_sum(s_pa, ks, D, d, r);
    }
  }
}

int sf_slot_prologue_ex(const float* prev, const float* init, const float* pm_ln_g, const float* pm_ln_b, const float* pm_w0_t,
                        const float* pm_b0, const float* pm_w2_t, const float* pm_b2, int norm_first, const float* kd_w_t,
                        const float* kd_b, const float* noise, long long noise_bs, float* kdist_out, long long kdist_bs,
                        const float* q_ln_g, const float* q_ln_b, const float* q_w_t, float* slots_out, float* q_out, int B,
                        int N, int D, float ln_eps, hipStream_t st) {
  if ((D % 64) != 0 || 2 * D > 768 || !kd_w_t || !kd_b || !q_w_t || !q_ln_g || !q_ln_b || !slots_out || !q_out || !init) return 1;
  if (prev && (!pm_ln_g || !pm_ln_b || !pm_w0_t || !pm_b0 || !pm_w2_t || !pm_b2)) return 1;
  if (B == 0) return 0;
  const int threads = 768, R = B * N, D2 = 2 * D;
  auto pmaxf = [&](int Nout, int K) { return su_kslices(threads, Nout, K) * Nout * SU_R; };
  int pmax = pmaxf(D2, D);
  if (pmaxf(D, D2) > pmax) pmax = pmaxf(D, D2);
  if (pmaxf(D, D) > pmax) pmax = pmaxf(D, D);
  const size_t lds = ((size_t)3 * D * SU_R + (size_t)D2 * SU_R + 2 * SU_R + (size_t)pmax) * sizeof(float);
  SF_TRY(sf_ensure_dyn_lds((const void*)sa_slot_prologue_kernel, lds));
  SpArgs a{prev, init, pm_ln_g, pm_ln_b, pm_w0_t, pm_b0, pm_w2_t, pm_b2, norm_first, kd_w_t, kd_b, noise, noise_bs, kdist_out,
           kdist_bs, q_ln_g, q_ln_b, q_w_t, slots_out, q_out};
  hipLaunchKernelGGL(sa_slot_prologue_kernel, dim3((R + SU_R - 1) / SU_R), dim3(threads), lds, st, a, R, N, D, pmax, ln_eps);
  SF_CHECK_LAUNCH();
  return 0;
}

int sf_sa_pick_partials(int HW) {
  if (HW % 256 == 0) return HW / 256;
  int P = HW / 128;
  while (P > 1 && (HW % P != 0 || (HW / P) % 16 != 0)) --P;
  if (P < 1) P = 1;
  return P;
}

extern "C" {

int sf_slot_attn_num_partials(int HW) { return sf_sa_pick_partials(HW); }

int sf_slot_attn_iter_f32(const float* k, const float* v, int ld, long long batch_stride, const float* q,
                          float* part_num, float* part_den, float* attn_out, int B, int HW, int N, int D,
                          float scale, float eps, void* stream) {
  return sf_slot_attn_iter_ex(k, v, ld, batch_stride, q, part_num, part_den, attn_out, (long long)N * HW, B, HW,
                              N, D, scale, eps, (hipStream_t)stream);
}

int sf_slot_prologue_f32(const float* prev, const float* init, const float* pm_ln_g, const float* pm_ln_b, const float* pm_w0_t,
                         const float* pm_b0, const float* pm_w2_t, const float* pm_b2, int norm_first, const float* kd_w_t,
                         const float* kd_b, const float* noise, long long noise_bs, float* kdist_out, long long kdist_bs,
                         const float* q_ln_g, const float* q_ln_b, const float* q_w_t, float* slots_out, float* q_out, int B, int N,
                         int D, float ln_eps, void* stream) {
  SF_REQUIRE(B >= 0 && N >= 1 && D >= 1, "sf_slot_prologue_f32: bad shape");
  const int rc = sf_slot_prologue_ex(prev, init, pm_ln_g, pm_ln_b, pm_w0_t, pm_b0, pm_w2_t, pm_b2, norm_first, kd_w_t, kd_b, noise, noise_bs,
                                     kdist_out, kdist_bs, q_ln_g, q_ln_b, q_w_t, slots_out, q_out, B, N, D, ln_eps, (hipStream_t)stream);
  SF_REQUIRE(rc != 1, "sf_slot_prologue_f32: slot size 64, 128, 192, ... 384; init, the kernel-distribution and q operands, and with prev the predictor's");
  return rc;
// ... 301 lines not shown
```

slotformer_amd/csrc/slot_chain.h:

```cpp
#pragma once
#include "sf_internal.h"

struct SfChainWeights {
  const void *gru_ih_p, *gru_hh_p;
  const float *gru_b_ih, *gru_b_hh, *ln_g, *ln_b;
  const void* w1_p;
  const float* b1;
  const void* w2_p;
  const float* b2;
  const float *q_ln_g, *q_ln_b;
  const void* q_w_p;
  const float *pm_ln_g, *pm_ln_b;
  const void* pm_w0_p;
  const float* pm_b0;
  const void* pm_w2_p;
  const float* pm_b2;
  int pm_norm_first;
  const void* kd_w_p;
  const float* kd_b;
};

bool sf_slot_chain_ok(int D, int H, int HW, int N);
int sf_slot_chain_ex(const void* feat_planes, int NB, int B, int T, int HW, int N, int iters, float scale, float eps, float ln_eps, float* slotsA, float* slotsB,
                     float* lat, float* q, float* post, long long post_bs, float* attn, const float* noise, float* kdist, const SfChainWeights* w,
                     hipStream_t st);
bool sf_slot_attn_planes_ok(int HW, int D, int N);
int sf_slot_attn_planes_ex(const void* planes, long long batch_stride_rows, const float* q, float* part_num, float* part_den, float* attn_out,
                           long long attn_batch_stride, int B, int HW, int N, float scale, float eps, hipStream_t st);
int sf_pixel_mlp_feat_planes_ex(const float* x, const float* ln0_g, const float* ln0_b, const float* w1, const float* b1, const float* w2,
                                const float* b2, const float* ln1_g, const float* ln1_b, void* planes, int M, float eps, hipStream_t st);
```

slotformer_amd/csrc/slot_chain.hip:

```cpp
#include "slot_update_body.h"
#include "slot_chain.h"

namespace {

constexpr int SC_D = 128, SC_NT = 512, SC_NW = 8, SC_TP = 32;
constexpr int SC_TILE = 2 * SC_TP * 256;
constexpr int SC_ATP = 20;
constexpr int SC_AT = SC_TP * SC_ATP * 4;
constexpr int SC_REDP = SC_D + 4;
constexpr size_t SC_LDS_SA = (size_t)SC_NW * (SC_TILE + SC_AT);
static_assert((size_t)SC_NW * 8 * SC_REDP * 4 + SC_NW * 8 * 4 <= (size_t)SC_NW * SC_TILE, "the reduction rows fit over the dead tiles");
constexpr size_t SC_REC = SC_LDS_SA > UM_LDS_NEXT ? SC_LDS_SA : UM_LDS_NEXT;
constexpr size_t SC_ARGS = SC_REC + (size_t)(8 * SC_D + 32 + 8 * SC_D) * 4;
constexpr size_t SC_LDS = SC_ARGS + ((sizeof(UmArgs) + 15) / 16) * 16 + ((sizeof(UmVar) + 15) / 16) * 16;
static_assert(SC_LDS <= 160 * 1024, "slot chain: LDS budget");

__device__ __forceinline__ int sc_swz(int row) { return 2 * ((row & 3) | (((row >> 3) & 1) << 2)); }

#define SC_MFMA(a, b, c) __builtin_amdgcn_mfma_f32_16x16x32_bf16(a, b, c, 0, 0, 0)

#ifdef SC_STAMPS
__device__ long long sc_ts[32];
__device__ int sc_tsn;
#define SCTS() do { if (blockIdx.x == 0 && threadIdx.x == 0 && sc_tsn < 32) sc_ts[sc_tsn++] = wall_clock64(); } while (0)
// ... 138 lines not shown
      const bf16x4 h0 = __builtin_amdgcn_ds_read_tr16_b64_v4bf16((lp)(bp)), h1 = __builtin_amdgcn_ds_read_tr16_b64_v4bf16((lp)(bp + 1024));
      const bf16x4 l0 = __builtin_amdgcn_ds_read_tr16_b64_v4bf16((lp)(bp + 8192)), l1 = __builtin_amdgcn_ds_read_tr16_b64_v4bf16((lp)(bp + 8192 + 1024));
      const bf16x8 bh = __builtin_shufflevector(h0, h1, 0, 1, 2, 3, 4, 5, 6, 7), bl = __builtin_shufflevector(l0, l1, 0, 1, 2, 3, 4, 5, 6, 7);
      nacc[cb] = SC_MFMA(ath, bl, nacc[cb]);
      nacc[cb] = SC_MFMA(atl, bh, nacc[cb]);
      nacc[cb] = SC_MFMA(ath, bh, nacc[cb]);
    }
    __builtin_amdgcn_wave_barrier();
  }
  SCTS();
#pragma unroll
  for (int r = 0; r < 4; ++r) den4[r] = sf_sum16(den4[r]);
  float* red = (float*)smem;
  float* redd = red + NW * 8 * SC_REDP;
  __syncthreads();
  if (sl0 < 8) {
#pragma unroll
    for (int cb = 0; cb < 8; ++cb)
#pragma unroll
      for (int r = 0; r < 4; ++r) red[(wave * 8 + sl0 + r) * SC_REDP + 16 * cb + i16] = nacc[cb][r];
  }
  if (sl0 < 8 && i16 == 0) {
#pragma unroll
    for (int r = 0; r < 4; ++r) redd[wave * 8 + sl0 + r] = den4[r];
  }
  __syncthreads();
  for (int idx = t; idx < N * SC_D; idx += 64 * NW) {
    const int n = idx >> 7, d = idx & 127;
    float s = 0.f;
#pragma unroll
    for (int w = 0; w < NW; ++w) s += red[(w * 8 + n) * SC_REDP + d];
    if constexpr (GIO) {
      ((float __attribute__((address_space(1)))*)pnum)[idx] = s;
      ((float __attribute__((address_space(1)))*)pnum)[zero_off_num + idx] = 0.f;
    } else {
      pnL[idx] = s;
    }
  }
  if (t < N) {
    float s = 0.f;
#pragma unroll
    for (int w = 0; w < NW; ++w) s += redd[w * 8 + t];
    if constexpr (GIO) {
      ((float __attribute__((address_space(1)))*)pden)[t] = s;
      ((float __attribute__((address_space(1)))*)pden)[zero_off_den + t] = 0.f;
    } else {
      pdL[t] = s;
    }
  }
}

template <bool ATTN>
__device__ __attribute__((noinline)) void sc_attend(const __bf16* __restrict__ frame, const float* qg, float scale, float eps, int HW, int N, float* pnum,
                                                    float* pden, float* __restrict__ attn, char* smem, int rev) {
  HW = __builtin_amdgcn_readfirstlane(HW);
  N = __builtin_amdgcn_readfirstlane(N);
  rev = __builtin_amdgcn_readfirstlane(rev);
  sc_attend_core<ATTN, SC_NW, false>(frame, qg, scale, eps, HW, N, 0, HW / SC_NW, pnum, pden, 0, 0, attn, smem, rev);
}

typedef __attribute__((address_space(3))) UmArgs LUmArgs;
typedef __attribute__((address_space(3))) UmVar LUmVar;
template <bool NEXT>
__device__ __attribute__((noinline)) void sc_update(const LUmArgs* ap, const LUmVar* vp, float* lds) {
  um_rows<NEXT, LUmArgs, LUmVar>(*ap, *vp, lds, 0);
}

__device__ __forceinline__ void sc_put_var(LUmVar* lv, const UmVar& um) {
  static_assert(sizeof(UmVar) % 4 == 0 && sizeof(UmVar) / 4 <= 64, "UmVar: one word per lane of a wave");
  const unsigned* srcw = (const unsigned*)&um;
  unsigned __attribute__((address_space(3)))* dstw = (unsigned __attribute__((address_space(3)))*)lv;
  unsigned w = 0;
#pragma unroll
  for (int i = 0; i < (int)(sizeof(UmVar) / 4); ++i)
    if ((int)threadIdx.x == i) w = srcw[i];
  if (threadIdx.x < sizeof(UmVar) / 4) dstw[threadIdx.x] = w;
}

// ... 59 lines not shown
        um.out2 = post_t;
        um.q_out = qv;
        um.nx_slots = sA;
        um.noise = A.noise ? A.noise + (((long long)v * T + t + 1) * N) * SC_D : nullptr;
        um.kdist_out = A.kdist ? A.kdist + (((long long)v * T + t + 1) * N) * 2 * SC_D : nullptr;
        sc_put_var(lv, um);
        __syncthreads();
        sc_update<true>(la, lv, sc_lds);
      } else {
        um.slots_out = s_out;
        um.out2 = last_it ? post_t : nullptr;
        um.q_out = last_it ? nullptr : qv;
        um.noise = nullptr;
        um.kdist_out = nullptr;
        um.nx_slots = nullptr;
        sc_put_var(lv, um);
        __syncthreads();
        sc_update<false>(la, lv, sc_lds);
      }
      __syncthreads();
      SCTS();
      float* tmp = s_in;
      s_in = s_out;
      s_out = tmp;
    }
  }
}

constexpr int SP_NW = 4, SP_PIX = 512;
constexpr size_t SP_LDS = (size_t)SP_NW * (SC_TILE + SC_AT);
template <bool ATTN>
__global__ __launch_bounds__(64 * SP_NW, 2) void sa_attn_planes_kernel(const __bf16* __restrict__ planes, long long batch_stride_rows, const float* __restrict__ q,
                                                                       float scale, float eps, float* __restrict__ part_num, float* __restrict__ part_den,
                                                                       float* __restrict__ attn, long long attn_bs, int HW, int N, int P) {
  extern __shared__ __attribute__((aligned(16))) float sp_lds[];
  const int b = blockIdx.y, chunk = blockIdx.x;
  const __bf16* frame = planes + (long long)b * batch_stride_rows * 256;
  float* pn = part_num + (((long long)b * P + 2 * chunk) * N) * SC_D;
  float* pd = part_den + ((long long)b * P + 2 * chunk) * N;
  sc_attend_core<ATTN, SP_NW, true>(frame, q + (long long)b * N * SC_D, scale, eps, HW, N, chunk * SP_PIX, SP_PIX / SP_NW, pn, pd, (long long)N * SC_D, N,
                                    ATTN ? attn + (long long)b * attn_bs : nullptr, (char*)sp_lds, 0);
}

bool sf_slot_attn_planes_ok(int HW, int D, int N) { return D == SC_D && HW % SP_PIX == 0 && N >= 1 && N <= 8; }

int sf_slot_attn_planes_ex(const void* planes, long long batch_stride_rows, const float* q, float* part_num, float* part_den, float* attn_out,
                           long long attn_batch_stride, int B, int HW, int N, float scale, float eps, hipStream_t st) {
  SF_REQUIRE(planes && q && part_num && part_den, "sf_slot_attn_planes_ex: null pointer");
  SF_REQUIRE(sf_slot_attn_planes_ok(HW, SC_D, N) && B >= 0, "sf_slot_attn_planes_ex: slot size 128, HW a multiple of 512, at most 8 slots");
  if (B == 0) return 0;
  const int P = HW / 256;
  sf_prof_begin(SF_K_SA_ITER, st, (double)B * HW * 512.0);
  if (attn_out) {
    SF_TRY(sf_ensure_dyn_lds((const void*)sa_attn_planes_kernel<true>, SP_LDS));
    hipLaunchKernelGGL(sa_attn_planes_kernel<true>, dim3(HW / SP_PIX, B), dim3(64 * SP_NW), SP_LDS, st, (const __bf16*)planes, batch_stride_rows, q, scale, eps,
                       part_num, part_den, attn_out, attn_batch_stride, HW, N, P);
  } else {
    SF_TRY(sf_ensure_dyn_lds((const void*)sa_attn_planes_kernel<false>, SP_LDS));
    hipLaunchKernelGGL(sa_attn_planes_kernel<false>, dim3(HW / SP_PIX, B), dim3(64 * SP_NW), SP_LDS, st, (const __bf16*)planes, batch_stride_rows, q, scale, eps,
                       part_num, part_den, nullptr, 0, HW, N, P);
  }
  sf_prof_end(SF_K_SA_ITER, st);
  SF_CHECK_LAUNCH();
  return 0;
}

extern "C" int sf_slot_attn_iter_planes_f32(const void* planes, long long batch_stride_rows, const float* q, float* part_num, float* part_den,
                                            float* attn_out, long long attn_batch_stride, int B, int HW, int N, float scale, float eps, void* stream) {
  return sf_slot_attn_planes_ex(planes, batch_stride_rows, q, part_num, part_den, attn_out, attn_batch_stride, B, HW, N, scale, eps, (hipStream_t)stream);
}

bool sf_slot_chain_ok(int D, int H, int HW, int N) { return D == SC_D && H == UM_H && HW >= 256 && HW % (SC_NW * SC_TP) == 0 && N >= 1 && N <= 8; }

int sf_slot_chain_ex(const void* feat_planes, int NB, int B, int T, int HW, int N, int iters, float scale, float eps, float ln_eps, float* slotsA, float* slotsB,
                     float* lat, float* q, float* post, long long post_bs, float* attn, const float* noise, float* kdist, const SfChainWeights* w,
                     hipStream_t st) {
  SF_REQUIRE(feat_planes && slotsA && slotsB && lat && q && post && w, "sf_slot_chain_ex: null pointer");
  SF_REQUIRE(sf_slot_chain_ok(SC_D, UM_H, HW, N) && NB >= 1 && B >= 1 && T >= 1 && iters >= 1 && post_bs >= (long long)T * N * SC_D, "sf_slot_chain_ex: bad shape");
  SF_REQUIRE(w->gru_ih_p && w->gru_hh_p && w->gru_b_ih && w->gru_b_hh && w->ln_g && w->ln_b && w->w1_p && w->b1 && w->w2_p && w->b2 && w->q_ln_g && w->q_ln_b &&
                 w->q_w_p && w->pm_ln_g && w->pm_ln_b && w->pm_w0_p && w->pm_b0 && w->pm_w2_p && w->pm_b2 && w->kd_w_p && w->kd_b,
             "sf_slot_chain_ex: null weight");
  ScArgs A;
  memset(&A, 0, sizeof(A));
  A.feat = (const __bf16*)feat_planes; A.B = B; A.T = T; A.HW = HW; A.N = N; A.iters = iters; A.scale = scale; A.eps = eps;
  A.slotsA = slotsA; A.slotsB = slotsB; A.lat = lat; A.q = q; A.post = post; A.post_bs = post_bs; A.attn = attn; A.noise = noise; A.kdist = kdist;
  UmArgs& a = A.um;
  a.w_ih_p = (const uint4*)w->gru_ih_p; a.w_hh_p = (const uint4*)w->gru_hh_p; a.b_ih = w->gru_b_ih; a.b_hh = w->gru_b_hh; a.ln_g = w->ln_g; a.ln_b = w->ln_b;
  a.w1_p = (const uint4*)w->w1_p; a.b1 = w->b1; a.w2_p = (const uint4*)w->w2_p; a.b2 = w->b2; a.q_ln_g = w->q_ln_g; a.q_ln_b = w->q_ln_b;
  a.q_w_p = (const uint4*)w->q_w_p; a.ln_eps = ln_eps; a.N = N; a.out2_bs = 0; a.noise_bs = 0; a.kdist_bs = 0;
  a.pm_ln_g = w->pm_ln_g; a.pm_ln_b = w->pm_ln_b; a.pm_w0_p = (const uint4*)w->pm_w0_p; a.pm_b0 = w->pm_b0; a.pm_w2_p = (const uint4*)w->pm_w2_p; a.pm_b2 = w->pm_b2;
  a.pm_norm_first = w->pm_norm_first; a.kd_w_p = (const uint4*)w->kd_w_p; a.kd_b = w->kd_b;
  SF_TRY(sf_ensure_dyn_lds((const void*)slot_chain_kernel, SC_LDS));
  sf_prof_begin(SF_K_SA_ITER, st, (double)NB * B * T * iters * HW * 512.0);
  hipLaunchKernelGGL(slot_chain_kernel, dim3(NB * B), dim3(SC_NT), SC_LDS, st, A);
  sf_prof_end(SF_K_SA_ITER, st);
  SF_CHECK_LAUNCH();
  return 0;
}

#ifdef SC_STAMPS
extern "C" int sf_debug_read_ts_chain(long long* out32) {
  int zero = 0;
// ... 6 lines not shown
```

slotformer_amd/csrc/slot_update_mfma.hip:

```cpp
#include "slot_update_body.h"

template <bool NEXT>
__global__ __launch_bounds__(UM_NT) void sa_slot_update_mfma_kernel(UmArgs a) {
  extern __shared__ __attribute__((aligned(16))) float um_lds[];
  um_body<NEXT>(a, um_lds, blockIdx.x);
}

bool sf_slot_update_mfma_ok(int D, int H, int P) { return D == UM_D && H == UM_H && P >= 1 && P <= 64; }

int sf_slot_update_mfma_ex(const float* part_num, const float* part_den, int P, const float* slots_prev, const void* gru_ih_p,
                           const void* gru_hh_p, const float* gru_b_ih, const float* gru_b_hh, const float* ln_g, const float* ln_b,
                           const void* w1_p, const float* b1, const void* w2_p, const float* b2, float* slots_out, float* out2,
                           long long out2_bs, const float* q_ln_g, const float* q_ln_b, const void* q_w_p, float* q_out, int B, int N,
                           float ln_eps, hipStream_t st, const SfNextStep* next, int p_step) {
  SF_REQUIRE(part_num && part_den && slots_prev && slots_out && gru_ih_p && gru_hh_p && gru_b_ih && gru_b_hh && ln_g && ln_b && w1_p &&
                 b1 && w2_p && b2, "sf_slot_update_mfma_ex: null pointer");
  SF_REQUIRE(!next || (q_out && next->pm_ln_g && next->pm_ln_b && next->pm_w0_p && next->pm_b0 && next->pm_w2_p && next->pm_b2 && next->kd_w_p &&
                       next->kd_b && next->slots && next->slots != slots_out),
             "sf_slot_update_mfma_ex: the next-step form needs q_out, the predictor / kernel-distribution operands and its own slot buffer");
  SF_REQUIRE(q_out == nullptr || (q_ln_g && q_ln_b && q_w_p), "q projection requested without its weights");
  SF_REQUIRE(N >= 1 && P >= 1 && P <= 64 && (p_step == 1 || (p_step == 2 && P % 2 == 0)), "bad slot shape");
  if (B == 0) return 0;
  static_assert(UM_LDS_NEXT <= 160 * 1024, "slot update: LDS budget");
  SF_TRY(next ? sf_ensure_dyn_lds((const void*)sa_slot_update_mfma_kernel<true>, (size_t)(UM_LDS_NEXT))
              : sf_ensure_dyn_lds((const void*)sa_slot_update_mfma_kernel<false>, (size_t)(UM_LDS)));
  UmArgs a;
  memset(&a, 0, sizeof(a));
  a.part_num = part_num; a.part_den = part_den; a.P = P / p_step; a.pstep = p_step; a.slots_prev = slots_prev;
  a.w_ih_p = (const uint4*)gru_ih_p; a.w_hh_p = (const uint4*)gru_hh_p; a.b_ih = gru_b_ih; a.b_hh = gru_b_hh; a.ln_g = ln_g; a.ln_b = ln_b;
  a.w1_p = (const uint4*)w1_p; a.b1 = b1; a.w2_p = (const uint4*)w2_p; a.b2 = b2; a.slots_out = slots_out; a.out2 = out2; a.out2_bs = out2_bs;
  a.q_ln_g = q_ln_g; a.q_ln_b = q_ln_b; a.q_w_p = (const uint4*)q_w_p; a.q_out = q_out; a.R = B * N; a.N = N; a.ln_eps = ln_eps;
  const int R = B * N;
  if (next) {
    a.pm_ln_g = next->pm_ln_g; a.pm_ln_b = next->pm_ln_b; a.pm_w0_p = (const uint4*)next->pm_w0_p; a.pm_b0 = next->pm_b0;
    a.pm_w2_p = (const uint4*)next->pm_w2_p; a.pm_b2 = next->pm_b2; a.pm_norm_first = next->norm_first; a.kd_w_p = (const uint4*)next->kd_w_p;
    a.kd_b = next->kd_b; a.noise = next->noise; a.noise_bs = next->noise_bs; a.kdist_out = next->kdist_out; a.kdist_bs = next->kdist_bs;
    a.nx_slots = next->slots;
  }
  sf_prof_begin(SF_K_SA_UPDATE, st,
                2.0 * R * ((double)6 * UM_D * UM_D + 2.0 * UM_D * UM_H + (q_out ? (double)UM_D * UM_D : 0.0) + (next ? 6.0 * UM_D * UM_D : 0.0)));
  if (next)
    hipLaunchKernelGGL(sa_slot_update_mfma_kernel<true>, dim3((R + UM_ROWS - 1) / UM_ROWS), dim3(UM_NT), UM_LDS_NEXT, st, a);
  else
    hipLaunchKernelGGL(sa_slot_update_mfma_kernel<false>, dim3((R + UM_ROWS - 1) / UM_ROWS), dim3(UM_NT), UM_LDS, st, a);
  sf_prof_end(SF_K_SA_UPDATE, st);
  SF_CHECK_LAUNCH();
  return 0;
}

extern "C" int sf_slot_update_packed_f32(const float* part_num, const float* part_den, int P, const float* slots_prev, const void* gru_ih_packed,
                                         const void* gru_hh_packed, const float* gru_b_ih, const float* gru_b_hh, const float* ln_g,
                                         const float* ln_b, const void* mlp_w1_packed, const float* mlp_b1, const void* mlp_w2_packed,
                                         const float* mlp_b2, float* slots_out, const float* q_ln_g, const float* q_ln_b,
                                         const void* q_w_packed, float* q_out, int B, int N, int D, int H, float ln_eps, void* stream) {
  if (sf_slot_update_wide_ok(D, H, P))
    return sf_slot_update_wide_ex(part_num, part_den, P, slots_prev, gru_ih_packed, gru_hh_packed, gru_b_ih, gru_b_hh, ln_g, ln_b, mlp_w1_packed,
                                  mlp_b1, mlp_w2_packed, mlp_b2, slots_out, nullptr, 0, q_ln_g, q_ln_b, q_w_packed, q_out, B, N, ln_eps,
                                  (hipStream_t)stream);
  SF_REQUIRE(sf_slot_update_mfma_ok(D, H, P),
             "sf_slot_update_packed_f32: slot size 128 with slot MLP size 256, or 192 with 384, and at most 64 partial records");
  return sf_slot_update_mfma_ex(part_num, part_den, P, slots_prev, gru_ih_packed, gru_hh_packed, gru_b_ih, gru_b_hh, ln_g, ln_b, mlp_w1_packed,
                                mlp_b1, mlp_w2_packed, mlp_b2, slots_out, nullptr, 0, q_ln_g, q_ln_b, q_w_packed, q_out, B, N, ln_eps,
                                (hipStream_t)stream);
}

extern "C" int sf_slot_update_packed_next_f32(const float* part_num, const float* part_den, int P, const float* slots_prev, const void* gru_ih_packed,
                                              const void* gru_hh_packed, const float* gru_b_ih, const float* gru_b_hh, const float* ln_g,
                                              const float* ln_b, const void* mlp_w1_packed, const float* mlp_b1, const void* mlp_w2_packed,
                                              const float* mlp_b2, float* slots_out, const float* q_ln_g, const float* q_ln_b,
                                              const void* q_w_packed, float* q_out, int B, int N, int D, int H, float ln_eps, float* out2,
                                              long long out2_bs, int p_step, const float* pm_ln_g, const float* pm_ln_b, const void* pm_w0_packed,
                                              const float* pm_b0, const void* pm_w2_packed, const float* pm_b2, int norm_first,
                                              const void* kd_w_packed, const float* kd_b, const float* noise, long long noise_bs, float* kdist_out,
                                              long long kdist_bs, float* next_slots, void* stream) {
// ... 17 lines not shown
```

slotformer_amd/engine.py:

```python
import ctypes as C
import os

import torch

from . import _lib
from ._call import ptr, require_device, scratch, stream
from ._lib import lib, check, sf_tfm_layer, sf_rollouter, sf_savi_encoder, sf_savi_decoder
from . import ops, plans

_WORKSPACES = {}


def workspace(device, nbytes, slot=0):
    key = (device.type, device.index, slot)
    cur = _WORKSPACES.get(key)
    if cur is None or cur.numel() < nbytes:
        cur = torch.empty(int(nbytes), dtype=torch.uint8, device=device)
        _WORKSPACES[key] = cur
    return cur


def workspace_for(device, slot, query, *args, at_least=0):
    key = (device.type, device.index, slot)
    ws = _WORKSPACES[key] = scratch(query, *args, device=device, reuse=_WORKSPACES.get(key), at_least=at_least)
# ... 333 lines not shown
    if s.pred_rnn:
        pred = m.predictor
        if prev_slots is None:
            pred.reset()
        st = pred.hidden_state
        if st is not None and st[0].shape[1] == B * N and st[0].device == dev:
            h, c, valid = st[0], st[1], 1
        else:
            h = torch.empty(1, B * N, s.pred_hidden, device=dev, dtype=torch.float32)
            c = torch.empty_like(h)
        pred.hidden_state = (h, c)
        pred.step += T if prev_slots is not None else T - 1
    if isinstance(side_stream, str):
        side_stream = _auto_side_stream(dev) if side_stream == 'auto' else None
    if side_stream is not None:
        query = (lib().sf_savi_encode_fork_workspace_bytes, C.byref(plan.struct), B, T)
    elif feat_pre is None:
        query = (lib().sf_savi_encode_batched_workspace_bytes, C.byref(plan.struct), B, T)
    else:
        query = (lib().sf_savi_encode_workspace_bytes, C.byref(plan.struct), B)
    ws = workspace_for(dev, ('enc', ws_slot), *query)
    n_pre = 0
    if feat_pre is not None:
        ops._chk(feat_pre)
        n_pre = feat_pre.shape[0]
        if feat_pre.shape[1] != B or feat_pre.shape[2] != 64 * 64:
            raise RuntimeError(f'feat_pre must be [n_pre,{B},4096,C], got {tuple(feat_pre.shape)}')
    check(lib().sf_savi_encode_fork_f32(C.byref(plan.struct), img.data_ptr(), ptr(feat_pre), n_pre, ptr(noise), ptr(prev_slots), ptr(h),
                                        ptr(c), valid, post.data_ptr(), ptr(kdist), ptr(attn), B, T, ws.data_ptr(), ws.numel(),
                                        stream(), None if side_stream is None else side_stream.cuda_stream))
    return post, kdist, attn


def savi_chain_ok(m, B, T):
    plan = encoder_plan(m)
    return bool(lib().sf_savi_chain_ok(C.byref(plan.struct), int(B), int(T)))


def savi_planes_bytes(m, B, T):
    return int(lib().sf_savi_planes_bytes(C.byref(encoder_plan(m).struct), int(B), int(T)))


def savi_features(m, img, out, ws_slot=0):
    _require_inference(m, img)
    ops._chk(img)
    plan = encoder_plan(m)
    B, T = img.shape[:2]
    ws = workspace_for(img.device, ('encf', ws_slot), lib().sf_savi_features_workspace_bytes, C.byref(plan.struct), B, T)
    check(lib().sf_savi_features_planes_f32(C.byref(plan.struct), img.data_ptr(), B, T, out.data_ptr(), ws.data_ptr(), ws.numel(),
                                            stream()))
    return out


def savi_slots_chain(m, planes, nb, B, T, post, noise=None, prev_slots=None, kdist=None, attn=None, ws_slot=0):
    plan = encoder_plan(m)
    s = plan.struct
    ops._chk(post, noise, prev_slots, kdist, attn)
    V = int(nb) * int(B)
    if post.shape[0] != V or post.shape[1] < T or post.stride(0) < T * s.num_slots * s.slot_size or post.stride(1) != s.num_slots * s.slot_size:
        raise RuntimeError(f'post must be [{V}, >= {T}, N, D] float32 with contiguous steps, got {tuple(post.shape)} strides {post.stride()}')
    ws = workspace_for(post.device, ('encs', ws_slot), lib().sf_savi_slots_chain_workspace_bytes, C.byref(plan.struct), V)
    check(lib().sf_savi_slots_chain_f32(C.byref(plan.struct), planes.data_ptr(), ptr(noise), ptr(prev_slots), post.data_ptr(), post.stride(0), ptr(kdist),
                                        ptr(attn), int(nb), int(B), int(T), ws.data_ptr(), ws.numel(), stream()))
    return post


# ... 106 lines not shown
```

slotformer_amd/ops.py:

```python
import torch

from ._call import ptr, scratch, stream
from ._lib import lib, check


def _chk(*ts):
    for t in ts:
        if t is None:
            continue
        if not (torch.is_tensor(t) and t.is_cuda and t.dtype == torch.float32 and t.is_contiguous()):
            raise RuntimeError('slotformer_amd ops need contiguous float32 tensors on a HIP device '
                               f'(got {type(t).__name__} {getattr(t, "dtype", None)} '
                               f'{getattr(t, "device", None)}); there is no CPU fallback')


def linear(x, weight, bias=None, ln=None, residual=None, relu=False, ln_eps=1e-5):
    _chk(x, weight, bias, residual, *(ln or ()))
    K = x.shape[-1]
    N = weight.shape[0]
    M = x.numel() // K
    out = torch.empty(*x.shape[:-1], N, device=x.device, dtype=torch.float32)
    g, b = (ln if ln is not None else (None, None))
    check(lib().sf_linear_f32(ptr(x), K, ptr(weight), ptr(bias), ptr(g), ptr(b), ln_eps, ptr(residual), N, ptr(out), N,
                              M, N, K, int(relu), stream()))
# ... 174 lines not shown
    F_, HW, C_ = d.shape
    dw, db = torch.empty(C_, 4, device=d.device), torch.empty(C_, device=d.device)
    dtab = torch.empty(HW, C_, device=d.device)
    check(lib().sf_pos_dense_grad_f32(ptr(d), F_, HW, C_, ptr(grid), ptr(dw), ptr(db), ptr(dtab), stream()))
    return dw, db, dtab


def savi_decode_head_bwd(dec, d_recon, act, out_w, want_param_grads=True):
    _chk(dec, d_recon, act, out_w)
    F_, N, HW, _ = dec.shape
    Cl = out_w.shape[1]
    d_dec, d_act = torch.empty_like(dec), torch.empty_like(act)
    gw = torch.empty(4, Cl, device=dec.device) if want_param_grads else None
    gb = torch.empty(4, device=dec.device) if want_param_grads else None
    ws = scratch(lib().sf_savi_decode_head_bwd_workspace_bytes, Cl, device=dec.device, at_least=16)
    check(lib().sf_savi_decode_head_bwd_f32(ptr(dec), ptr(d_recon), ptr(act), ptr(out_w), ptr(d_dec), ptr(d_act), ptr(gw), ptr(gb), F_, N, HW, Cl,
                                            ws.data_ptr(), ws.numel(), stream()))
    return d_dec, d_act, gw, gb


def slot_attn_iter(k, v, q, eps=1e-6, want_attn=False):
    _chk(k, v, q)
    B, HW, D = k.shape
    N = q.shape[1]
    P = lib().sf_slot_attn_num_partials(HW)
    pn = torch.empty(B, P, N, D, device=k.device, dtype=torch.float32)
    pd = torch.empty(B, P, N, device=k.device, dtype=torch.float32)
    attn = torch.empty(B, N, HW, device=k.device, dtype=torch.float32) if want_attn else None
    check(lib().sf_slot_attn_iter_f32(ptr(k), ptr(v), D, HW * D, ptr(q), ptr(pn), ptr(pd), ptr(attn), B, HW, N, D,
                                      float(D)**-0.5, eps, stream()))
    return pn, pd, attn


def slot_attn_iter_planes(planes, q, eps=1e-6, want_attn=False):
    _chk(q)
    if not (planes.is_cuda and planes.dtype == torch.bfloat16 and planes.is_contiguous() and planes.shape[-1] == 256):
        raise RuntimeError('slot_attn_iter_planes needs contiguous bfloat16 rows [B, HW, 256] on a HIP device')
    B, HW, _ = planes.shape
    N, P = q.shape[1], HW // 256
    pn = torch.empty(B, P, N, 128, device=q.device, dtype=torch.float32)
    pd = torch.empty(B, P, N, device=q.device, dtype=torch.float32)
    attn = torch.empty(B, N, HW, device=q.device, dtype=torch.float32) if want_attn else None
    check(lib().sf_slot_attn_iter_planes_f32(planes.data_ptr(), HW, ptr(q), ptr(pn), ptr(pd), ptr(attn), N * HW, B, HW, N, 128.0**-0.5, eps,
                                             stream()))
    return pn, pd, attn


def slot_prologue(prev, init, pm, kd, q, noise=None, norm_first=True, want_kdist=False, B=None, ln_eps=1e-5):
    pm = pm or (None, ) * 6
    _chk(prev, init, *pm, *kd, *q, noise)
    N, D = init.shape
    B = prev.shape[0] if prev is not None else B
    t = lambda w: None if w is None else w.t().contiguous()
    w0_t, w2_t, kd_t, q_t = t(pm[2]), t(pm[4]), t(kd[0]), t(q[2])
    slots, q_out = torch.empty(B, N, D, device=init.device), torch.empty(B, N, D, device=init.device)
    kdist = torch.empty(B, N, 2 * D, device=init.device) if want_kdist else None
    check(lib().sf_slot_prologue_f32(ptr(prev), ptr(init), ptr(pm[0]), ptr(pm[1]), ptr(w0_t), ptr(pm[3]), ptr(w2_t), ptr(pm[5]), int(norm_first), ptr(kd_t),
                                     ptr(kd[1]), ptr(noise), N * D, ptr(kdist), N * 2 * D, ptr(q[0]), ptr(q[1]), ptr(q_t), ptr(slots), ptr(q_out), B, N, D,
                                     ln_eps, stream()))
    return slots, q_out, kdist


def slot_attn_iter_bwd(k, v, q, pn, pd, d_updates, dk=None, dv=None, eps=1e-6):
    _chk(k, v, q, pn, pd, d_updates)
    B, HW, D = k.shape
    N, P = q.shape[1], pn.shape[1]
    acc = dk is not None
    if not acc:
        dk, dv = torch.empty_like(k), torch.empty_like(v)
    dq = torch.empty_like(q)
    ws_bytes, bwd = ((lib().sf_slot_attn_iter_bwd_workspace_bytes, lib().sf_slot_attn_iter_bwd_f32) if N <= 8 else
                     (lib().sf_slot_attn_iter_bwd16_workspace_bytes, lib().sf_slot_attn_iter_bwd16_f32))
    ws = scratch(ws_bytes, B, HW, N, D, device=k.device)
    check(bwd(ptr(k), ptr(v), D, HW * D, ptr(q), ptr(pn), ptr(pd), P, ptr(d_updates), ptr(dk), ptr(dv),
              int(acc), ptr(dq), B, HW, N, D, float(D)**-0.5, eps, ws.data_ptr(), ws.numel(), stream()))
    return dq, dk, dv

# ... 613 lines not shown
```

slotformer_amd/pipeline.py:

```python
import ctypes as C
import math
import os
import threading
import time

import torch

from . import _lib, engine

_STREAMS = {}
_STREAMS_LOCK = threading.Lock()
_POOL = True


def encode_mask_words(spec):
    if isinstance(spec, str) and spec.startswith('rows'):
        r = int(spec[4:])
        if not 1 <= r <= 7:
            raise ValueError('slotformer_amd: rows<R> needs 1 <= R <= 7')
        return [0xffffffff if w < r else 0 for w in range(8)]
    if isinstance(spec, str):
        spec = int(spec, 16)
    if isinstance(spec, (list, tuple)):
        if len(spec) != 8:
# ... 160 lines not shown
        self._masked_taken = {}
        self._lib = _lib.lib()
        self._enc_words_pair = ENC_WORDS_P
        if partition == 'pair':
            if isinstance(encode_cu_word, str) and encode_cu_word.startswith('rows'):
                self._enc_words_pair = encode_mask_words(encode_cu_word)
            elif os.environ.get('SF_PIPE_CU_SPLIT'):
                self._enc_words_pair = encode_mask_words(os.environ['SF_PIPE_CU_SPLIT'])
            elif self._encode_rows() != 4:
                self._enc_words_pair = encode_mask_words(f'rows{self._encode_rows()}')
        if rollout_opts is None and partition == 'pair':
            roll_cus = 256 - sum(bin(w).count('1') for w in self._enc_words_pair)
            rollout_opts = pair_unit_options(self.roll, self.B, self.G, roll_cus, self.tok, self.T)
            self._row_tiles = bool(rollout_opts['attn_rows'])
        if partition in ('three', 'two') and (rollout_opts is None or (isinstance(rollout_opts, dict) and 'cus' not in rollout_opts)):
            cus = 168 if partition == 'three' else 256 - sum(bin(w).count('1') for w in encode_mask_words(encode_cu_word))
            rollout_opts = dict(rollout_opts or {}, cus=cus)
        if isinstance(rollout_opts, dict) and 'layer_tok' not in rollout_opts:
            rollout_opts = dict(rollout_opts, layer_tok=False)
        self.rollout_opts = engine.rollout_opts(rollout_opts)
        self.tok = self.tok and self.rollout_opts is not None and self.rollout_opts.layer_tok > 0
        self.row_opts = self.rollout_opts
        if self.tok:
            o = self.rollout_opts
            self.row_opts = _lib.sf_rollout_opts(o.precision, o.seam_fused, o.ffn_rows, o.attn_heads_per_wg, o.attn_qkv_rows, o.ffn_tile, o.cus_available, -1)
        self.tail_opts = self.rollout_opts
        if self.rollout_opts is not None and (self.rollout_opts.ffn_rows > 64 or self.rollout_opts.attn_heads_per_wg == 8 or
                                              self.rollout_opts.attn_qkv_rows or self.rollout_opts.ffn_tile):
            self.tail_opts = _lib.sf_rollout_opts(self.rollout_opts.precision, self.rollout_opts.seam_fused, min(self.rollout_opts.ffn_rows or 64, 64), 2, 0, 0,
                                                  self.rollout_opts.cus_available, -1)
        self.use_graph = bool(use_graph)
        self.encode_graph = bool(int(os.environ.get('SF_PIPE_ENCODE_GRAPH', '1'))) if encode_graph is None else bool(encode_graph)
        self._enc_graphs = {}
        self.encode_fork = bool(encode_fork)
        self.drain_latency_form = self.G * self.B < 128
        self._key = ('pipe', id(self))
        want_split = bool(split)
        self.split = bool(want_split and partition == 'pair' and self.fused and engine.savi_chain_ok(savi, self.B, self.T))
        self._with_noise = engine.kernel_noise(self.savi, torch.empty(0), 1, self.T, self.dev) is not None
        self.chain_on = 'roll' if chain_on == 'roll' else 'enc'
        if self.split:
            self.steal = 0.0
        self._plan = None
        self.units = []
        self.spread_remainder = True
        hist_ = getattr(rollouter, 'cond_len', None) or getattr(rollouter, 'history_len', None) or self.T
        self._rows_per_batch = self.B * int(rollouter.num_slots) * int(hist_)
        self._tails = {}
        self._capture_all()
        self.cu_split = False
        self.partition = 'none'
        self.s_roll = None
        self.roll_streams = []
        self.lanes = []
        if partition != 'none':
            try:
                if partition == 'pair':
                    enc_words = self._enc_words_pair
                    roll_words = [~w & 0xffffffff for w in enc_words]
                    self.roll_streams = [self._masked_stream(roll_words) for _ in range(self._nroll)]
                    self.s_roll = self.roll_streams[0]
                    self.lanes = [(self._masked_stream(enc_words), 0, self.B)]
                    self.encode_cus = sum(bin(w).count('1') for w in enc_words)
                    self.rollout_cus = 256 - self.encode_cus
                elif partition == 'three':
                    nb = max(1, round(self.B * 24 / 88))
# ... 221 lines not shown
        if self.tok:
            if u.buf.shape[0] < 96 or u.latency_form:
                opts = self.tail_opts
            elif u.row_form:
                opts = self.row_opts
            else:
                opts = self.rollout_opts
        elif full and not u.latency_form:
            opts = self.rollout_opts
        else:
            opts = self.tail_opts
        engine.rollout(self.roll, u.buf, self.T, self.H, ws_slot=u.key, opts=opts)

    def _rollout(self, u):
        if u.graph is not None:
            u.graph.replay()
        else:
            self._rollout_eager(u)

    def _encode(self, img, noise, dst, feat_pre, lo=0, hi=None, lane=0, unit=None):
        hi = self.B if hi is None else hi
        if self.split:
            u, h = unit
            if u.noise is not None:
                u.noise[h * self.B:(h + 1) * self.B].copy_(engine.kernel_noise(self.savi, noise, self.B, self.T, self.dev))
            engine.savi_features(self.savi, img, u.planes[h], ws_slot=self._key + ('feat', lane))
            return
        if lo != 0 or hi != self.B:
            img = img[lo:hi]
            noise = None if noise is None else noise[lo:hi]
        noise = engine.kernel_noise(self.savi, noise, hi - lo, self.T, self.dev)
        if self.encode_graph:
            eg = self._encode_graph_for(lane, hi - lo, 0 if feat_pre is None else feat_pre.shape[0], img.shape[-1], noise is not None)
            eg['img'].copy_(img)
            if noise is not None:
                eg['noise'].copy_(noise)
            if feat_pre is not None:
                eg['feat'].copy_(feat_pre)
            eg['graph'].replay()
            dst[lo:hi, :self.T].copy_(eg['post'])
            return
        side = None
        if self.encode_fork:
            cache = self.__dict__.setdefault('_fork_side', {})
            side = cache.get(lane)
            if side is None:
                if isinstance(lane, int) and self.cu_split:
                    side = self._masked_stream(self._lane_words(lane))
                else:
                    side = self._pool_stream('fork', k=len(cache))
                cache[lane] = side
        post, _, _ = engine.savi_encode(self.savi, img, noise=noise, feat_pre=feat_pre, ws_slot=self._key + ('enc', lane), side_stream=side)
        dst[lo:hi, :self.T].copy_(post)

    def _lane_words(self, lane):
        if self.partition == 'pair':
            return self._enc_words_pair
        if self.partition == 'three':
            return LANE0_WORDS_3 if lane == 0 else LANE1_WORDS_3
        return [0xffffffff] * 8

    def _encode_graph_for(self, lane, nv, k, res, with_noise):
        key = (lane, nv, k, res, with_noise)
        eg = self._enc_graphs.get(key)
        if eg is None:
            cur = torch.cuda.current_stream(self.dev)
            cl = list(self.savi.enc_channels)[-1]
            eg = {'img': torch.zeros(nv, self.T, 3, res, res, device=self.dev),
                  'noise': torch.zeros(nv, self.T, self.N, self.D, device=self.dev) if with_noise else None,
                  'feat': torch.zeros(k, nv, 64 * 64, cl, device=self.dev) if k else None}
            ws = self._key + ('encg', ) + key
            side = torch.cuda.Stream(device=self.dev)
            side.wait_stream(cur)
            fork_here = self.encode_fork
            side2 = torch.cuda.Stream(device=self.dev) if fork_here else None
            lane_cus = int(self.encode_cus // max(len(self.lanes), 1)) if (isinstance(lane, int) and self.cu_split) else 0
            if not isinstance(lane, int) and self.cu_split and self.tok:
                lane_cus = int(self._lib.sf_stream_cus(None))
            if lane_cus:
                self._lib.sf_stream_set_cus(C.c_void_p(side.cuda_stream), lane_cus)
            try:
                with torch.cuda.stream(side):
                    engine.savi_encode(self.savi, eg['img'], noise=eg['noise'], feat_pre=eg['feat'], ws_slot=ws, side_stream=side2)
                    side.synchronize()
                    g = torch.cuda.CUDAGraph()
                    with _lib.CAPTURE_GATE, torch.cuda.graph(g, stream=side, capture_error_mode='thread_local'):
                        post, _, _ = engine.savi_encode(self.savi, eg['img'], noise=eg['noise'], feat_pre=eg['feat'], ws_slot=ws, side_stream=side2)
                cur.wait_stream(side)
            finally:
                if lane_cus:
                    self._lib.sf_stream_set_cus(C.c_void_p(side.cuda_stream), 0)
            eg['graph'], eg['post'] = g, post
            self._enc_graphs[key] = eg
        return eg

    def _unit_plan(self, n):
        G = self.G
        sizes, n_tail = unit_sizes_for(n, G, self._rows_per_batch, ramp=self.ramp, spread=self.spread_remainder)
        probe = getattr(self, 'unit_sizes_override', None)
        if probe and sum(int(x) for x in probe.split(',')) == n:
            sizes = [int(x) for x in probe.split(',')]
        plan, u0, nfull, ntail = [], 0, 0, {}
        n_drain = n_tail
        if self.tok and len(sizes) >= 3 and sizes[-1] <= getattr(self, 'hybrid_tail', 2):
            n_drain = max(n_drain, 2)
        for i, nb in enumerate(sizes):
            if nb == G:
                u = self.units[nfull % self.NU]
                nfull += 1
            else:
                u = self._tail_unit(nb, ntail.get(nb, 0) % 2, row_form=self.tok and i == len(sizes) - 1)
                ntail[nb] = ntail.get(nb, 0) + 1
            drain = i >= len(sizes) - max(n_drain, 1)
            if drain and nb == G and len(sizes) > 1 and self.tail_opts is not self.rollout_opts and self.drain_latency_form:
                if 'drain' not in self._tails:
                    self._tails['drain'] = self._new_unit(G, ('drain', ), latency_form=True)
                u = self._tails['drain']
            elif drain and nb == G and len(sizes) > 1 and self.tok and i == len(sizes) - 1:
                if 'drain' not in self._tails:
                    self._tails['drain'] = self._new_unit(G, ('drain', ), row_form=True)
# ... 359 lines not shown
```

slotformer_amd/switches.py:

```python
import os

SWITCHES = {
    'SF_PRECISION': ('product', "process default of the matrix arithmetic: 'bf16x3' (default; split-bf16, fp32-equivalent) | 'f32' (exact-f32 MFMA) | 'bf16' (single pass)"),
    'SF_LAYER_TOK': ('product', "process default of sf_rollout_opts.layer_tok for DIRECT rollout calls (0, default: the row-tile / latency forms; 1: the layers before the last as token-stationary launches -- d_model 256 rollouters on the fused / long-window paths, and the OBJ3D shape (128, 8, 512) on the generic path, where it pays from ~64 videos per call and costs 7 % at 32: `sf_rollout_tok_layers` tells what a call takes). The pipeline passes its own choice per unit"),
    'SF_SEAM_FUSED': ('product', "process default of the seam launches of the latency forms (1; 0: two launches instead)"),
    'SF_CONV_FP16X2': ('product', "OPT-IN two-product fp16 form of the 5x5 convolutions (weights rounded to fp16: 3-6e-5 from the fixtures instead of 1e-5); default 0"),
    'SF_CONV_WS': ('product', "0: the 4-row-tile convolution everywhere (default 1: the weights-stationary kernel on streams with CUs of their own; the same bits)"),
    'SF_ENCODE_FORK': ('product', "direct encode calls as two branches on two streams (1, default) or one stream (0)"),
    'SF_PIPE_TOK': ('product', "0: the pipeline never uses the token-stationary layer launches (every unit bit-identical to the serial module calls)"),
    'SF_PIPE_GROUP': ('product', "batches per rollout unit (default: 6 for token-stationary units of 32-video batches, else 4 / unit_batches_for)"),
    'SF_PIPE_HYBRID': ('product', "every k-th batch behind the fill is encoded on an unmasked stream beside the CU-masked lane (default 8 with token-stationary units, 3 / 5 / 0 otherwise)"),
    'SF_PIPE_FILL': ('product', "batches encoded on the whole chip at the start of a run (default: three units' worth)"),
    'SF_PIPE_CU_SPLIT': ('product', "CU mask of the encode partition, e.g. rows4 (default: sized from the two sides' CU time)"),
    'SF_PIPE_ENCODE_GRAPH': ('product', "replay the encode of a batch from a hipGraph (1, default) or launch it eagerly (0)"),
    'SF_PIPE_TRACE': ('tools', "record the device timeline of a run (tools/pipe_timeline.py)"),
    'SF_LIB_PATH': ('tools', "load another build of libslotformer_hip.so (tools/build_variant.sh: -D variants of a kernel)"),
    'SF_DBG': ('tools', "in-kernel time stamps and tuning overrides of the probes, comma separated: conv, lt, lf=<bits>, deconv, gemm, gemmcfg=<id>, convcfg=<id>, sab1 / flash1 (the packed-word attention backward / exact-f32 flash forward the bf16-plane kernels replaced), sabts (tools/*_probe.py)"),
}

PROCESS = {
    'precision': ('sf_set_precision', 'sf_get_precision', 'SF_PRECISION', 1, "matrix arithmetic: 0 exact-f32 MFMA, 1 split-bf16 (bf16x3), 2 single-pass bf16; the getter answers the calling thread's per-call precision while one is set"),
    'layer_tok': ('sf_set_layer_tok', 'sf_get_layer_tok', 'SF_LAYER_TOK', 0, "sf_rollout_opts.layer_tok == 0: the layers before the last of a rollout as token-stationary launches"),
    'seam_fused': ('sf_set_seam_fused', 'sf_get_seam_fused', 'SF_SEAM_FUSED', 1, "sf_rollout_opts.seam_fused == -1: seam launches of the rollout's latency forms"),
    'ffn_rows64': ('sf_set_ffn_rows64', 'sf_get_ffn_rows64', None, 0, "sf_rollout_opts.ffn_rows == 0: 64 instead of 32 rows per workgroup of the chunk-partial FFN launches (the same bits)"),
    'conv_fp16x2': ('sf_set_conv_fp16x2', 'sf_get_conv_fp16x2', 'SF_CONV_FP16X2', 0, "OPT-IN two-product fp16 arithmetic of the 64 -> 64 5x5 convolutions"),
    'slot_attn_tile16': ('sf_set_slot_attn_tile16', 'sf_get_slot_attn_tile16', None, 1, "9 .. 16 slots, keys == values: the one-pass tile kernel of Slot Attention (0: the two-pass kernel)"),
    'encode_fuse_next': ('sf_set_encode_fuse_next', 'sf_get_encode_fuse_next', None, 1, "the slot prologue of step t + 1 at the tail of step t's last slot update (0: its own launch; split-bf16 rounding apart)"),
    'slot_chain': ('sf_set_slot_chain', 'sf_get_slot_chain', None, 0, "OPT-IN: the slot branch of a batched encode as one video-stationary launch"),
    'slot_attn_planes': ('sf_set_slot_attn_planes', 'sf_get_slot_attn_planes', None, 1, "Slot-Attention iterations of the encode on feature rows kept as two bf16 planes, split-bf16 MFMAs (0: f32 rows, exact-f32 tile kernel)"),
    'pixel_tok': ('sf_set_pixel_tok', 'sf_get_pixel_tok', None, 1, "the per-pixel chain of the encoder in its pixel-stationary form (0: the tile kernels; another summation order)"),
}


def check_environment(environ=None):
    environ = os.environ if environ is None else environ
    seen = {k: v for k, v in environ.items() if k.startswith('SF_')}
    return {k: v for k, v in seen.items() if k in SWITCHES}, sorted(k for k in seen if k not in SWITCHES)


def markdown_table():
    rows = ['| variable | kind | what it does |', '|---|---|---|']
    rows += [f'| `{k}` | {kind} | {text} |' for k, (kind, text) in SWITCHES.items()]
    return '\n'.join(rows)


def process_table():
    rows = ['| switch | setter / getter | environment | default | what it selects |', '|---|---|---|---|---|']
    rows += [f"| {k} | `{s}` / `{g}` | {f'`{env}`' if env else '-'} | {default} | {text} |" for k, (s, g, env, default, text) in PROCESS.items()]
    return '\n'.join(rows)


if __name__ == '__main__':
    print(markdown_table())
    print()
    print(process_table())
```

Baseline: 725,500.

## Read encode inputs and outputs through a device pointer record to skip staging copies

Adds an sf_encode_io pointer record that the captured encode graph's kernels (first conv, slot prologue, slot update) dereference at run time. The pipeline can then point a replayed graph straight at the caller's image, noise and output tensors instead of copying into and out of graph-owned buffers. It also adds a dense-records variant of the plane Slot-Attention kernel that emits P/2 partial records rather than interleaved zero records, so the slot update reads fewer partials. Each replay now pays a small pointer-set launch, and the kernels do an extra pointer indirection.

```diff
diff --git a/include/slotformer_hip.h b/include/slotformer_hip.h
--- a/include/slotformer_hip.h
+++ b/include/slotformer_hip.h
@@ -132,6 +132,8 @@
                           float scale, float eps, void* stream);
 int sf_slot_attn_iter_planes_f32(const void* planes, long long batch_stride_rows, const float* q, float* part_num, float* part_den,
                                  float* attn_out, long long attn_batch_stride, int B, int HW, int N, float scale, float eps, void* stream);
+int sf_slot_attn_iter_planes_dense_f32(const void* planes, long long batch_stride_rows, const float* q, float* part_num, float* part_den,
+                                       float* attn_out, long long attn_batch_stride, int B, int HW, int N, float scale, float eps, void* stream);
 int sf_slot_prologue_f32(const float* prev, const float* init, const float* pm_ln_g, const float* pm_ln_b, const float* pm_w0_t,
                          const float* pm_b0, const float* pm_w2_t, const float* pm_b2, int norm_first, const float* kd_w_t,
                          const float* kd_b, const float* noise, long long noise_bs, float* kdist_out, long long kdist_bs,
@@ -552,6 +554,20 @@
                            const float* prev_slots, float* lstm_h, float* lstm_c, int state_valid, float* post_slots,
                            float* kernel_dist, float* attn, int B, int T, void* ws, size_t ws_bytes, void* stream);
 size_t sf_savi_encode_fork_workspace_bytes(const sf_savi_encoder* m, int B, int T);
+typedef struct {
+  const float* img;
+  const float* noise;
+  float* post;
+  long long post_bs;
+  const float* img0;
+  const float* noise0;
+  float* post0;
+  long long reserved;
+} sf_encode_io;
+int sf_savi_encode_io_ok(const sf_savi_encoder* m, int B, int T);
+int sf_encode_io_set(sf_encode_io* io, const sf_encode_io* values, void* stream);
+int sf_savi_encode_io_f32(const sf_savi_encoder* m, const sf_encode_io* io, const float* img, const float* noise, float* post_slots,
+                          float* kernel_dist, float* attn, int B, int T, void* ws, size_t ws_bytes, void* stream);
 size_t sf_savi_encode_batched_workspace_bytes(const sf_savi_encoder* m, int B, int T);
 int sf_set_encode_fuse_next(int on);
 int sf_get_encode_fuse_next(void);
@@ -561,6 +577,7 @@
 int sf_get_slot_attn_planes(void);
 int sf_set_pixel_tok(int on);
 int sf_get_pixel_tok(void);
+int sf_encode_dense_records(int on);
 int sf_savi_chain_ok(const sf_savi_encoder* m, int B, int T);
 size_t sf_savi_planes_bytes(const sf_savi_encoder* m, int B, int T);
 size_t sf_savi_features_workspace_bytes(const sf_savi_encoder* m, int B, int T);
diff --git a/slotformer_amd/_lib.py b/slotformer_amd/_lib.py
--- a/slotformer_amd/_lib.py
+++ b/slotformer_amd/_lib.py
@@ -109,6 +109,10 @@
          ('sa_q_w_p', C.c_void_p), ('sa_fold_q_w', FP), ('sa_fold_q_w_t', FP), ('sa_fold_gru_ih_t', FP), ('sa_fold_q_w_p', C.c_void_p),
          ('sa_fold_gru_ih_p', C.c_void_p), ('pred_packed', C.POINTER(C.c_void_p)), ('enc_fc1_p', C.c_void_p), ('enc_fc2_p', C.c_void_p),
          ('conv_w_frag', C.c_void_p * 8), ('pm_w0_p', C.c_void_p), ('pm_w2_p', C.c_void_p), ('kd_w0_p', C.c_void_p)])
+
+
+class sf_encode_io(C.Structure):
+    _fields_ = [('img', FP), ('noise', FP), ('post', FP), ('post_bs', C.c_longlong), ('img0', FP), ('noise0', FP), ('post0', FP), ('reserved', C.c_longlong)]
 
 
 class sf_slate_block(C.Structure):
@@ -206,6 +210,7 @@
     'sf_slot_update_f32': (I, [FP, FP, I, FP] + [FP] * 10 + [FP, I, I, I, I, F32, VP]),
     'sf_slot_update_packed_f32': (I, [FP, FP, I, FP, VP, VP, FP, FP, FP, FP, VP, FP, VP, FP, FP, FP, FP, VP, FP, I, I, I, I, F32, VP]),
     'sf_slot_attn_iter_planes_f32': (I, [VP, LL, FP, FP, FP, FP, LL, I, I, I, F32, F32, VP]),
+    'sf_slot_attn_iter_planes_dense_f32': (I, [VP, LL, FP, FP, FP, FP, LL, I, I, I, F32, F32, VP]),
     'sf_slot_prologue_f32': (I, [FP] * 8 + [I, FP, FP, FP, LL, FP, LL, FP, FP, FP, FP, FP, I, I, I, F32, VP]),
     'sf_slot_update_packed_next_f32': (I, [FP, FP, I, FP, VP, VP, FP, FP, FP, FP, VP, FP, VP, FP, FP, FP, FP, VP, FP, I, I, I, I, F32,
                                            FP, LL, I, FP, FP, VP, FP, VP, FP, I, VP, FP, FP, LL, FP, LL, FP, VP]),
@@ -355,6 +360,9 @@
                                    VP]),
     'sf_savi_encode_fork_workspace_bytes': (SZ, [C.POINTER(sf_savi_encoder), I, I]),
     'sf_savi_encode_batched_workspace_bytes': (SZ, [C.POINTER(sf_savi_encoder), I, I]),
+    'sf_savi_encode_io_ok': (I, [C.POINTER(sf_savi_encoder), I, I]),
+    'sf_encode_io_set': (I, [VP, C.POINTER(sf_encode_io), VP]),
+    'sf_savi_encode_io_f32': (I, [C.POINTER(sf_savi_encoder), VP, FP, FP, FP, FP, FP, I, I, VP, SZ, VP]),
     'sf_set_encode_fuse_next': (I, [I]),
     'sf_get_encode_fuse_next': (I, []),
     'sf_set_slot_chain': (I, [I]),
@@ -363,6 +371,7 @@
     'sf_get_slot_attn_planes': (I, []),
     'sf_set_pixel_tok': (I, [I]),
     'sf_get_pixel_tok': (I, []),
+    'sf_encode_dense_records': (I, [I]),
     'sf_savi_chain_ok': (I, [C.POINTER(sf_savi_encoder), I, I]),
     'sf_savi_planes_bytes': (SZ, [C.POINTER(sf_savi_encoder), I, I]),
     'sf_savi_features_workspace_bytes': (SZ, [C.POINTER(sf_savi_encoder), I, I]),
diff --git a/slotformer_amd/csrc/conv_first.hip b/slotformer_amd/csrc/conv_first.hip
--- a/slotformer_amd/csrc/conv_first.hip
+++ b/slotformer_amd/csrc/conv_first.hip
@@ -22,8 +22,10 @@
 __global__ __launch_bounds__(CF_NT, CF_WPS) void conv_first_kernel(const float* __restrict__ img, long long frame_stride,
                                                            const float* __restrict__ w, const float* __restrict__ bias,
                                                            const float* __restrict__ add, float* __restrict__ out, int Ho,
-                                                           int Hin, int Win, int relu, int fgroup, long long group_stride, int ntiles) {
+                                                           int Hin, int Win, int relu, int fgroup, long long group_stride, int ntiles,
+                                                           const sf_encode_io* __restrict__ io) {
   using G = CfGeo<STRIDE>;
+  if (io) img = io->img + (img - io->img0);
   constexpr int HR = G::HR, HC = G::HC, HCP = G::HCP;
   constexpr int NH = (CF_CI * HR * HC + CF_NT - 1) / CF_NT;
   extern __shared__ __attribute__((aligned(16))) float smem[];
@@ -137,7 +139,7 @@
 
 template <int STRIDE>
 static int launch_cf(const float* img, long long frame_stride, const float* w, const float* bias, const float* add,
-                     float* out, int F, int Ho, int Hin, int Win, int relu, int fgroup, long long group_stride, hipStream_t st) {
+                     float* out, int F, int Ho, int Hin, int Win, int relu, int fgroup, long long group_stride, hipStream_t st, const sf_encode_io* io) {
   auto kern = conv_first_kernel<STRIDE>;
   constexpr size_t lds = CfGeo<STRIDE>::lds;
   static_assert(lds <= 80 * 1024, "first conv: two workgroups per CU");
@@ -147,7 +149,7 @@
   int grid = (CF_WPS / 2) * sf_stream_cus((void*)st);
   if (grid > ntiles) grid = ntiles;
   if (grid < 1) grid = 1;
-  hipLaunchKernelGGL(kern, dim3(grid), dim3(CF_NT), lds, st, img, frame_stride, w, bias, add, out, Ho, Hin, Win, relu, fgroup, group_stride, ntiles);
+  hipLaunchKernelGGL(kern, dim3(grid), dim3(CF_NT), lds, st, img, frame_stride, w, bias, add, out, Ho, Hin, Win, relu, fgroup, group_stride, ntiles, io);
   sf_prof_end(SF_K_CONV_FIRST, st);
   SF_CHECK_LAUNCH();
   return 0;
@@ -158,11 +160,14 @@
   return sf_conv_first_grouped_ex(img, frame_stride, F > 0 ? F : 1, 0, w, bias, add, out, F, Cin, Hin, Win, Cout, ks, stride, relu, st);
 }
 int sf_conv_first_grouped_ex(const float* img, long long frame_stride, int fgroup, long long group_stride, const float* w, const float* bias,
-                             const float* add, float* out, int F, int Cin, int Hin, int Win, int Cout, int ks, int stride, int relu, hipStream_t st) {
-  if (Cin != CF_CI || Cout != CF_CO || ks != CF_KS || F <= 0 || fgroup <= 0) return 1;
-  if (stride == 2 && Hin == 128 && Win == 128) return launch_cf<2>(img, frame_stride, w, bias, add, out, F, 64, Hin, Win, relu, fgroup, group_stride, st);
-  if (stride == 1 && Hin == 64 && Win == 64) return launch_cf<1>(img, frame_stride, w, bias, add, out, F, 64, Hin, Win, relu, fgroup, group_stride, st);
-  return 1;
+                             const float* add, float* out, int F, int Cin, int Hin, int Win, int Cout, int ks, int stride, int relu, hipStream_t st,
+                             const sf_encode_io* io) {
+  if (!sf_conv_first_ok(Cin, Cout, ks, Hin, Win, stride) || F <= 0 || fgroup <= 0) return 1;
+  if (stride == 2) return launch_cf<2>(img, frame_stride, w, bias, add, out, F, 64, Hin, Win, relu, fgroup, group_stride, st, io);
+  return launch_cf<1>(img, frame_stride, w, bias, add, out, F, 64, Hin, Win, relu, fgroup, group_stride, st, io);
+}
+bool sf_conv_first_ok(int Cin, int Cout, int ks, int Hin, int Win, int stride) {
+  return Cin == CF_CI && Cout == CF_CO && ks == CF_KS && ((stride == 2 && Hin == 128 && Win == 128) || (stride == 1 && Hin == 64 && Win == 64));
 }
 
 extern "C" int sf_conv2d_nchw_in_grouped_f32(const float* img, long long frame_stride, int fgroup, long long group_stride, const float* weight,
diff --git a/slotformer_amd/csrc/engine.hip b/slotformer_amd/csrc/engine.hip
--- a/slotformer_amd/csrc/engine.hip
+++ b/slotformer_amd/csrc/engine.hip
@@ -545,6 +545,7 @@
   const void *q_w_p = nullptr, *gru_ih_p = nullptr;
   enum Update { VALU, WIDE, MFMA } update = VALU;
   int p_step = 1;
+  bool dense_records = false;
   bool pred_step = false;
   bool prologue = false;
   bool fuse_next = false;
@@ -625,6 +626,8 @@
   p.update = !su_packed ? EncodePlan::VALU : sf_slot_update_mfma_ok(D, Hm, P) ? EncodePlan::MFMA
             : sf_slot_update_wide_ok(D, Hm, P) ? EncodePlan::WIDE : EncodePlan::VALU;
   if (fold && P == HW / 256 && (planes || sf_slot_attn_sparse_records_n(nullptr, nullptr, HW, D, N))) p.p_step = 2;
+  p.dense_records = planes && p.update == EncodePlan::MFMA && p.p_step == 2 && sf_switch(SF_SW_ENCODE_DENSE_RECORDS);
+  if (p.dense_records) p.p_step = 1;
   p.pred_step = m->pred_type == 1 && m->pred_packed && precision >= 1;
   p.prologue = m->pred_type == 0 && !m->pred_rnn && m->kd_mode == 1 && m->pm_w0_t && m->pm_w2_t && m->kd_w0_t && p.q_w_t;
   p.fuse_next = p.prologue && p.update == EncodePlan::MFMA && m->pm_w0_p && m->pm_w2_p && m->kd_w0_p && m->pm_ln_g && m->pm_ln_b && m->pm_b0 &&
@@ -664,12 +667,13 @@
   return 0;
 }
 
-int enc_cnn_all_steps(const sf_savi_encoder* m, const float* img, int B, int T, float* const* big, hipStream_t st) {
+int enc_cnn_all_steps(const sf_savi_encoder* m, const float* img, int B, int T, float* const* big, hipStream_t st, const sf_encode_io* io = nullptr) {
   const int res = m->resolution, c1 = m->enc_channels[1];
   const long long frame_elems = (long long)3 * res * res;
   const int rc = sf_conv_first_grouped_ex(img, (long long)T * frame_elems, B, frame_elems, m->conv_w[0], m->conv_b[0], nullptr, big[0], B * T,
-                                          m->enc_channels[0], res, res, c1, m->enc_ks, res == 128 ? 2 : 1, 1, st);
+                                          m->enc_channels[0], res, res, c1, m->enc_ks, res == 128 ? 2 : 1, 1, st, io);
   if (rc < 0 || rc > 1) return rc;
+  if (rc == 1 && io) return sf_set_err(-1, "the first convolution of this shape cannot read through a pointer record", __FILE__, __LINE__);
   for (int t = 0; t < T && rc == 1; ++t)
     SF_TRY(sf_conv2d_nchw_in_f32(img + (long long)t * frame_elems, (long long)T * frame_elems, m->conv_w[0], m->conv_b[0], nullptr,
                                  big[0] + (long long)t * B * ENC_HW * c1, B, m->enc_channels[0], res, res, c1, m->enc_ks, res == 128 ? 2 : 1, 1, st));
@@ -724,6 +728,7 @@
   const float *img, *feat_pre, *noise;
   float *lstm_h, *lstm_c, *post, *kernel_dist, *attn;
   int B, T;
+  const sf_encode_io* io;
 };
 
 int enc_step_features(const EncodeArgs& a, const EncodePlan& p, const EncodeWs& w, int t, float* kv, hipStream_t st) {
@@ -822,8 +827,9 @@
     rc = sf_slot_prologue_ex(prev, m->init_latents, m->pm_ln_g, m->pm_ln_b, m->pm_w0_t, m->pm_b0, m->pm_w2_t, m->pm_b2, m->pred_norm_first, m->kd_w0_t,
                              m->kd_b0, a.noise ? a.noise + (long long)t * N * D : nullptr, (long long)T * N * D,
                              a.kernel_dist ? a.kernel_dist + (long long)t * N * 2 * D : nullptr, (long long)T * N * 2 * D, m->sa_q_ln_g, m->sa_q_ln_b,
-                             p.q_w_t, w.rows.a, w.rows.q, a.B, N, D, ln_eps, st);
+                             p.q_w_t, w.rows.a, w.rows.q, a.B, N, D, ln_eps, st, a.io);
   *one_launch = rc == 0;
+  if (rc == 1 && a.io) return sf_set_err(-1, "the slot prologue of this model cannot read through a pointer record", __FILE__, __LINE__);
   if (rc != 1) return rc;
   const float* lat;
   SF_TRY(enc_predict(a, p, w, prev, st, &lat));
@@ -849,13 +855,14 @@
   const int HW = ENC_HW, N = m->num_slots, D = m->slot_size, Hm = m->slot_mlp_size, Ce = m->enc_out_channels, T = a.T, B = a.B, P = sf_sa_pick_partials(HW);
   const float ln_eps = 1e-5f, scale = 1.0f / sqrtf((float)D);
   const long long attn_bs = (long long)T * N * HW, post_bs = (long long)T * N * D;
+  const int Pr = p.dense_records ? P / 2 : P;
   float *s_in = w.rows.a, *s_out = w.rows.b;
   for (int it = 0; it < m->num_iterations; ++it) {
     const bool last_it = (it == m->num_iterations - 1), nx_on = next && last_it;
     float* aout = (a.attn && last_it) ? a.attn + (long long)t * N * HW : nullptr;
     float* post = last_it ? a.post + (long long)t * N * D : nullptr;
     if (p.feat == EncodePlan::FOLD_PLANES)
-      SF_TRY(sf_slot_attn_planes_ex(kv, HW, w.rows.q, w.pnum, w.pden, aout, attn_bs, B, HW, N, scale, m->sa_eps, st));
+      SF_TRY(sf_slot_attn_planes_ex(kv, HW, w.rows.q, w.pnum, w.pden, aout, attn_bs, B, HW, N, scale, m->sa_eps, st, p.dense_records));
     else if (p.fold())
       SF_TRY(sf_slot_attn_iter_ex(kv, kv, Ce, (long long)HW * Ce, w.rows.q, w.pnum, w.pden, aout, attn_bs, B, HW, N, D, scale, m->sa_eps, st));
     else
@@ -867,10 +874,10 @@
       nx.noise = a.noise ? a.noise + (long long)(t + 1) * N * D : nullptr; nx.noise_bs = (long long)T * N * D;
       nx.kdist_out = a.kernel_dist ? a.kernel_dist + (long long)(t + 1) * N * 2 * D : nullptr; nx.kdist_bs = (long long)T * N * 2 * D;
       nx.slots = w.rows.a;
-      SF_TRY(sf_slot_update_mfma_ex(w.pnum, w.pden, P, s_in, p.gru_ih_p, m->sa_gru_hh_p, m->gru_b_ih, m->gru_b_hh, m->mlp_ln_g, m->mlp_ln_b,
+      SF_TRY(sf_slot_update_mfma_ex(w.pnum, w.pden, Pr, s_in, p.gru_ih_p, m->sa_gru_hh_p, m->gru_b_ih, m->gru_b_hh, m->mlp_ln_g, m->mlp_ln_b,
                                     m->sa_mlp_w1_p, m->mlp_b1, m->sa_mlp_w2_p, m->mlp_b2, (nx_on && s_out == w.rows.a) ? w.rows.lat : s_out, post, post_bs,
                                     m->sa_q_ln_g, m->sa_q_ln_b, p.q_w_p, (last_it && !nx_on) ? nullptr : w.rows.q, B, N, ln_eps, st, nx_on ? &nx : nullptr,
-                                    p.p_step));
+                                    p.p_step, a.io));
     } else if (p.update == EncodePlan::WIDE) {
       SF_TRY(sf_slot_update_wide_ex(w.pnum, w.pden, P, s_in, p.gru_ih_p, m->sa_gru_hh_p, m->gru_b_ih, m->gru_b_hh, m->mlp_ln_g, m->mlp_ln_b,
                                     m->sa_mlp_w1_p, m->mlp_b1, m->sa_mlp_w2_p, m->mlp_b2, s_out, post, post_bs, m->sa_q_ln_g, m->sa_q_ln_b,
@@ -994,9 +1001,45 @@
 }
 
 
+static bool enc_io_plan_ok(const sf_savi_encoder* m, const EncodePlan& p) {
+  return p.batched && !p.chain && !p.fork && p.n_pre == 0 && p.prologue && p.update == EncodePlan::MFMA && !m->pred_rnn &&
+         sf_conv_first_ok(m->enc_channels[0], m->enc_channels[1], m->enc_ks, m->resolution, m->resolution, m->resolution == 128 ? 2 : 1);
+}
+static int savi_encode_run(const sf_savi_encoder* m, const sf_encode_io* io, const float* img, const float* feat_pre, int n_pre, const float* noise,
+                           const float* prev_slots, float* lstm_h, float* lstm_c, int state_valid, float* post_slots, float* kernel_dist, float* attn,
+                           int B, int T, void* ws, size_t ws_bytes, void* stream, void* side_stream);
+static __global__ void encode_io_set_kernel(sf_encode_io* dst, sf_encode_io v) {
+  static_assert(sizeof(sf_encode_io) == 64, "sf_encode_io: eight 8-byte words");
+  if (threadIdx.x < 8) ((long long*)dst)[threadIdx.x] = ((const long long*)&v)[threadIdx.x];
+}
+int sf_encode_io_set(sf_encode_io* io, const sf_encode_io* values, void* stream) {
+  SF_REQUIRE(io && values, "sf_encode_io_set: null pointer");
+  SF_REQUIRE(values->img && values->img0 && values->post && values->post0 && (values->noise == nullptr) == (values->noise0 == nullptr),
+             "sf_encode_io_set: img / post and their recorded twins are required; noise is NULL exactly when noise0 is");
+  SF_REQUIRE((((uintptr_t)values->img | (uintptr_t)values->noise | (uintptr_t)values->post) & 15) == 0 && values->post_bs % 4 == 0,
+             "sf_encode_io_set: buffers must be 16-byte aligned");
+  hipLaunchKernelGGL(encode_io_set_kernel, dim3(1), dim3(64), 0, (hipStream_t)stream, io, *values);
+  SF_CHECK_LAUNCH();
+  return 0;
+}
 int sf_savi_encode_fork_f32(const sf_savi_encoder* m, const float* img, const float* feat_pre, int n_pre, const float* noise,
                             const float* prev_slots, float* lstm_h, float* lstm_c, int state_valid, float* post_slots,
                             float* kernel_dist, float* attn, int B, int T, void* ws, size_t ws_bytes, void* stream, void* side_stream) {
+  return savi_encode_run(m, nullptr, img, feat_pre, n_pre, noise, prev_slots, lstm_h, lstm_c, state_valid, post_slots, kernel_dist, attn, B, T, ws, ws_bytes,
+                         stream, side_stream);
+}
+int sf_savi_encode_io_ok(const sf_savi_encoder* m, int B, int T) {
+  if (!m || B < 1 || T < 1 || m->enc_layers < 1 || m->enc_layers > 8) return 0;
+  return enc_io_plan_ok(m, plan_encode(m, B, T, 0, false, ~(size_t)0)) ? 1 : 0;
+}
+int sf_savi_encode_io_f32(const sf_savi_encoder* m, const sf_encode_io* io, const float* img, const float* noise, float* post_slots, float* kernel_dist,
+                          float* attn, int B, int T, void* ws, size_t ws_bytes, void* stream) {
+  SF_REQUIRE(io, "sf_savi_encode_io_f32: null pointer record");
+  return savi_encode_run(m, io, img, nullptr, 0, noise, nullptr, nullptr, nullptr, 0, post_slots, kernel_dist, attn, B, T, ws, ws_bytes, stream, nullptr);
+}
+static int savi_encode_run(const sf_savi_encoder* m, const sf_encode_io* io, const float* img, const float* feat_pre, int n_pre, const float* noise,
+                           const float* prev_slots, float* lstm_h, float* lstm_c, int state_valid, float* post_slots, float* kernel_dist, float* attn,
+                           int B, int T, void* ws, size_t ws_bytes, void* stream, void* side_stream) {
   SF_REQUIRE(m && img && post_slots && ws, "null pointer");
   SF_REQUIRE(n_pre >= 0 && n_pre <= T && (n_pre == 0 || feat_pre != nullptr), "bad precomputed-feature arguments");
   SF_REQUIRE(B >= 1 && T >= 1, "bad batch / clip length");
@@ -1018,12 +1061,14 @@
     SF_REQUIRE(lstm_h && lstm_c && m->pred_hidden > 0 && m->lstm_w_ih && m->lstm_w_hh && m->lstm_b_ih &&
                    m->lstm_b_hh && m->proj_w && m->proj_b, "null LSTM state / weight");
   const EncodePlan p = plan_encode(m, B, T, n_pre, side_stream != nullptr && side_stream != stream, ws_bytes);
+  SF_REQUIRE(!io || enc_io_plan_ok(m, p), "sf_savi_encode_io_f32: this call's plan has kernels that cannot read through a pointer record (sf_savi_encode_io_ok; "
+                                         "workspace of sf_savi_encode_batched_workspace_bytes)");
   for (int i = 0; i < m->enc_layers; ++i) SF_REQUIRE(m->conv_w[i] != nullptr, "null conv weight");
   SfArena bp(ws, ws_bytes);
   EncodeWs w;
   SF_REQUIRE(ws_bytes >= enc_ws_bytes(m, B, T, p) && enc_ws_take(bp, w, m, B, T, p), "workspace too small");
   const hipStream_t st_main = (hipStream_t)stream, st = p.fork ? (hipStream_t)side_stream : st_main;
-  const EncodeArgs a{m, img, feat_pre, noise, lstm_h, lstm_c, post_slots, kernel_dist, attn, B, T};
+  const EncodeArgs a{m, img, feat_pre, noise, lstm_h, lstm_c, post_slots, kernel_dist, attn, B, T, io};
   const int N = m->num_slots, D = m->slot_size;
   const float* prev = prev_slots;
   if (m->pred_rnn && (prev == nullptr || !state_valid)) {
@@ -1035,7 +1080,7 @@
     SF_TRY(enc_feature_planes(m, img, B, T, w.big, w.planes, st_main));
     return enc_slots_chain(m, w.planes, noise, prev, post_slots, (long long)T * N * D, kernel_dist, attn, 1, B, T, w.rows, st_main);
   }
-  if (p.batched) SF_TRY(enc_cnn_all_steps(m, img, B, T, w.big, st_main));
+  if (p.batched) SF_TRY(enc_cnn_all_steps(m, img, B, T, w.big, st_main, io));
   bool next_done = false;
   for (int t = 0; t < T; ++t) {
     float* kv = w.kv + (size_t)(t % p.KV) * B * ENC_HW * 2 * D;
diff --git a/slotformer_amd/csrc/sf_internal.h b/slotformer_amd/csrc/sf_internal.h
--- a/slotformer_amd/csrc/sf_internal.h
+++ b/slotformer_amd/csrc/sf_internal.h
@@ -60,7 +60,7 @@
                            const void* gru_hh_p, const float* gru_b_ih, const float* gru_b_hh, const float* ln_g, const float* ln_b,
                            const void* w1_p, const float* b1, const void* w2_p, const float* b2, float* slots_out, float* out2,
                            long long out2_bs, const float* q_ln_g, const float* q_ln_b, const void* q_w_p, float* q_out, int B, int N,
-                           float ln_eps, hipStream_t st, const SfNextStep* next = nullptr, int p_step = 1);
+                           float ln_eps, hipStream_t st, const SfNextStep* next = nullptr, int p_step = 1, const sf_encode_io* io = nullptr);
 bool sf_slot_attn_sparse_records(const float* k, const float* v, int HW, int D);
 bool sf_slot_attn_sparse_records_n(const float* k, const float* v, int HW, int D, int N);
 bool sf_slot_update_wide_ok(int D, int H, int P);
@@ -78,7 +78,7 @@
                         const float* pm_b0, const float* pm_w2_t, const float* pm_b2, int norm_first, const float* kd_w_t,
                         const float* kd_b, const float* noise, long long noise_bs, float* kdist_out, long long kdist_bs,
                         const float* q_ln_g, const float* q_ln_b, const float* q_w_t, float* slots_out, float* q_out, int B,
-                        int N, int D, float ln_eps, hipStream_t st);
+                        int N, int D, float ln_eps, hipStream_t st, const sf_encode_io* io = nullptr);
 int sf_slot_attn_iter_ex(const float* k, const float* v, int ld, long long batch_stride, const float* q,
                          float* part_num, float* part_den, float* attn_out, long long attn_batch_stride, int B,
                          int HW, int N, int D, float scale, float eps, hipStream_t st);
@@ -116,6 +116,8 @@
 
 bool sf_layer_fused_ok(int d, int heads, int ffn, int L);
 int sf_conv_first_grouped_ex(const float* img, long long frame_stride, int fgroup, long long group_stride, const float* w, const float* bias,
-                             const float* add, float* out, int F, int Cin, int Hin, int Win, int Cout, int ks, int stride, int relu, hipStream_t st);
+                             const float* add, float* out, int F, int Cin, int Hin, int Win, int Cout, int ks, int stride, int relu, hipStream_t st,
+                             const sf_encode_io* io = nullptr);
+bool sf_conv_first_ok(int Cin, int Cout, int ks, int Hin, int Win, int stride);
 int sf_conv_first_ex(const float* img, long long frame_stride, const float* w, const float* bias, const float* add,
                      float* out, int F, int Cin, int Hin, int Win, int Cout, int ks, int stride, int relu, hipStream_t st);
diff --git a/slotformer_amd/csrc/sf_switches.cpp b/slotformer_amd/csrc/sf_switches.cpp
--- a/slotformer_amd/csrc/sf_switches.cpp
+++ b/slotformer_amd/csrc/sf_switches.cpp
@@ -23,6 +23,7 @@
      {nullptr, 1, NO_ENV},
      {nullptr, 1, NO_ENV},
      {"SF_CONV_WS", 1, FLAG},
+     {nullptr, 1, NO_ENV},
 };
 
 std::atomic<int> g_slot[SF_SW_NUM];
@@ -74,4 +75,8 @@
 int sf_set_slot_attn_planes(int on) { return sf_switch_set(SF_SW_SLOT_ATTN_PLANES, on != 0); }
 int sf_get_pixel_tok(void) { return sf_switch(SF_SW_PIXEL_TOK); }
 int sf_set_pixel_tok(int on) { return sf_switch_set(SF_SW_PIXEL_TOK, on != 0); }
+int sf_encode_dense_records(int on) {
+  if (on >= 0) sf_switch_set(SF_SW_ENCODE_DENSE_RECORDS, on != 0);
+  return sf_switch(SF_SW_ENCODE_DENSE_RECORDS);
 }
+}
diff --git a/slotformer_amd/csrc/sf_switches.h b/slotformer_amd/csrc/sf_switches.h
--- a/slotformer_amd/csrc/sf_switches.h
+++ b/slotformer_amd/csrc/sf_switches.h
@@ -12,6 +12,7 @@
   SF_SW_SLOT_ATTN_PLANES,
   SF_SW_PIXEL_TOK,
   SF_SW_CONV_WS,
+  SF_SW_ENCODE_DENSE_RECORDS,
   SF_SW_NUM
 };
 
diff --git a/slotformer_amd/csrc/slot_attn.hip b/slotformer_amd/csrc/slot_attn.hip
--- a/slotformer_amd/csrc/slot_attn.hip
+++ b/slotformer_amd/csrc/slot_attn.hip
@@ -497,8 +497,9 @@
   float* q_out;
 };
 
-__global__ __launch_bounds__(768) void sa_slot_prologue_kernel(SpArgs a, int R, int N, int D, int pmax, float ln_eps) {
+__global__ __launch_bounds__(768) void sa_slot_prologue_kernel(SpArgs a, int R, int N, int D, int pmax, float ln_eps, const sf_encode_io* __restrict__ io) {
   extern __shared__ __attribute__((aligned(16))) float su_lds[];
+  if (io && a.noise) a.noise = io->noise + (a.noise - io->noise0);
   const int D2 = 2 * D;
   float* s_x = su_lds;
   float* s_ln = s_x + D * SU_R;
@@ -589,7 +590,7 @@
                         const float* pm_b0, const float* pm_w2_t, const float* pm_b2, int norm_first, const float* kd_w_t,
                         const float* kd_b, const float* noise, long long noise_bs, float* kdist_out, long long kdist_bs,
                         const float* q_ln_g, const float* q_ln_b, const float* q_w_t, float* slots_out, float* q_out, int B,
-                        int N, int D, float ln_eps, hipStream_t st) {
+                        int N, int D, float ln_eps, hipStream_t st, const sf_encode_io* io) {
   if ((D % 64) != 0 || 2 * D > 768 || !kd_w_t || !kd_b || !q_w_t || !q_ln_g || !q_ln_b || !slots_out || !q_out || !init) return 1;
   if (prev && (!pm_ln_g || !pm_ln_b || !pm_w0_t || !pm_b0 || !pm_w2_t || !pm_b2)) return 1;
   if (B == 0) return 0;
@@ -602,7 +603,7 @@
   SF_TRY(sf_ensure_dyn_lds((const void*)sa_slot_prologue_kernel, lds));
   SpArgs a{prev, init, pm_ln_g, pm_ln_b, pm_w0_t, pm_b0, pm_w2_t, pm_b2, norm_first, kd_w_t, kd_b, noise, noise_bs, kdist_out,
            kdist_bs, q_ln_g, q_ln_b, q_w_t, slots_out, q_out};
-  hipLaunchKernelGGL(sa_slot_prologue_kernel, dim3((R + SU_R - 1) / SU_R), dim3(threads), lds, st, a, R, N, D, pmax, ln_eps);
+  hipLaunchKernelGGL(sa_slot_prologue_kernel, dim3((R + SU_R - 1) / SU_R), dim3(threads), lds, st, a, R, N, D, pmax, ln_eps, io);
   SF_CHECK_LAUNCH();
   return 0;
 }
diff --git a/slotformer_amd/csrc/slot_chain.h b/slotformer_amd/csrc/slot_chain.h
--- a/slotformer_amd/csrc/slot_chain.h
+++ b/slotformer_amd/csrc/slot_chain.h
@@ -26,6 +26,6 @@
                      hipStream_t st);
 bool sf_slot_attn_planes_ok(int HW, int D, int N);
 int sf_slot_attn_planes_ex(const void* planes, long long batch_stride_rows, const float* q, float* part_num, float* part_den, float* attn_out,
-                           long long attn_batch_stride, int B, int HW, int N, float scale, float eps, hipStream_t st);
+                           long long attn_batch_stride, int B, int HW, int N, float scale, float eps, hipStream_t st, bool dense = false);
 int sf_pixel_mlp_feat_planes_ex(const float* x, const float* ln0_g, const float* ln0_b, const float* w1, const float* b1, const float* w2,
                                 const float* b2, const float* ln1_g, const float* ln1_b, void* planes, int M, float eps, hipStream_t st);
diff --git a/slotformer_amd/csrc/slot_chain.hip b/slotformer_amd/csrc/slot_chain.hip
--- a/slotformer_amd/csrc/slot_chain.hip
+++ b/slotformer_amd/csrc/slot_chain.hip
@@ -194,7 +194,7 @@
     for (int w = 0; w < NW; ++w) s += red[(w * 8 + n) * SC_REDP + d];
     if constexpr (GIO) {
       ((float __attribute__((address_space(1)))*)pnum)[idx] = s;
-      ((float __attribute__((address_space(1)))*)pnum)[zero_off_num + idx] = 0.f;
+      if (zero_off_num) ((float __attribute__((address_space(1)))*)pnum)[zero_off_num + idx] = 0.f;
     } else {
       pnL[idx] = s;
     }
@@ -205,7 +205,7 @@
     for (int w = 0; w < NW; ++w) s += redd[w * 8 + t];
     if constexpr (GIO) {
       ((float __attribute__((address_space(1)))*)pden)[t] = s;
-      ((float __attribute__((address_space(1)))*)pden)[zero_off_den + t] = 0.f;
+      if (zero_off_den) ((float __attribute__((address_space(1)))*)pden)[zero_off_den + t] = 0.f;
     } else {
       pdL[t] = s;
     }
@@ -331,33 +331,33 @@
 template <bool ATTN>
 __global__ __launch_bounds__(64 * SP_NW, 2) void sa_attn_planes_kernel(const __bf16* __restrict__ planes, long long batch_stride_rows, const float* __restrict__ q,
                                                                        float scale, float eps, float* __restrict__ part_num, float* __restrict__ part_den,
-                                                                       float* __restrict__ attn, long long attn_bs, int HW, int N, int P) {
+                                                                       float* __restrict__ attn, long long attn_bs, int HW, int N, int P, int pstep) {
   extern __shared__ __attribute__((aligned(16))) float sp_lds[];
   const int b = blockIdx.y, chunk = blockIdx.x;
   const __bf16* frame = planes + (long long)b * batch_stride_rows * 256;
-  float* pn = part_num + (((long long)b * P + 2 * chunk) * N) * SC_D;
-  float* pd = part_den + ((long long)b * P + 2 * chunk) * N;
-  sc_attend_core<ATTN, SP_NW, true>(frame, q + (long long)b * N * SC_D, scale, eps, HW, N, chunk * SP_PIX, SP_PIX / SP_NW, pn, pd, (long long)N * SC_D, N,
-                                    ATTN ? attn + (long long)b * attn_bs : nullptr, (char*)sp_lds, 0);
+  float* pn = part_num + (((long long)b * P + pstep * chunk) * N) * SC_D;
+  float* pd = part_den + ((long long)b * P + pstep * chunk) * N;
+  sc_attend_core<ATTN, SP_NW, true>(frame, q + (long long)b * N * SC_D, scale, eps, HW, N, chunk * SP_PIX, SP_PIX / SP_NW, pn, pd,
+                                    pstep == 2 ? (long long)N * SC_D : 0, pstep == 2 ? N : 0, ATTN ? attn + (long long)b * attn_bs : nullptr, (char*)sp_lds, 0);
 }
 
 bool sf_slot_attn_planes_ok(int HW, int D, int N) { return D == SC_D && HW % SP_PIX == 0 && N >= 1 && N <= 8; }
 
 int sf_slot_attn_planes_ex(const void* planes, long long batch_stride_rows, const float* q, float* part_num, float* part_den, float* attn_out,
-                           long long attn_batch_stride, int B, int HW, int N, float scale, float eps, hipStream_t st) {
+                           long long attn_batch_stride, int B, int HW, int N, float scale, float eps, hipStream_t st, bool dense) {
   SF_REQUIRE(planes && q && part_num && part_den, "sf_slot_attn_planes_ex: null pointer");
   SF_REQUIRE(sf_slot_attn_planes_ok(HW, SC_D, N) && B >= 0, "sf_slot_attn_planes_ex: slot size 128, HW a multiple of 512, at most 8 slots");
   if (B == 0) return 0;
-  const int P = HW / 256;
+  const int pstep = dense ? 1 : 2, P = HW / SP_PIX * pstep;
   sf_prof_begin(SF_K_SA_ITER, st, (double)B * HW * 512.0);
   if (attn_out) {
     SF_TRY(sf_ensure_dyn_lds((const void*)sa_attn_planes_kernel<true>, SP_LDS));
     hipLaunchKernelGGL(sa_attn_planes_kernel<true>, dim3(HW / SP_PIX, B), dim3(64 * SP_NW), SP_LDS, st, (const __bf16*)planes, batch_stride_rows, q, scale, eps,
-                       part_num, part_den, attn_out, attn_batch_stride, HW, N, P);
+                       part_num, part_den, attn_out, attn_batch_stride, HW, N, P, pstep);
   } else {
     SF_TRY(sf_ensure_dyn_lds((const void*)sa_attn_planes_kernel<false>, SP_LDS));
     hipLaunchKernelGGL(sa_attn_planes_kernel<false>, dim3(HW / SP_PIX, B), dim3(64 * SP_NW), SP_LDS, st, (const __bf16*)planes, batch_stride_rows, q, scale, eps,
-                       part_num, part_den, nullptr, 0, HW, N, P);
+                       part_num, part_den, nullptr, 0, HW, N, P, pstep);
   }
   sf_prof_end(SF_K_SA_ITER, st);
   SF_CHECK_LAUNCH();
@@ -367,6 +367,11 @@
 extern "C" int sf_slot_attn_iter_planes_f32(const void* planes, long long batch_stride_rows, const float* q, float* part_num, float* part_den,
                                             float* attn_out, long long attn_batch_stride, int B, int HW, int N, float scale, float eps, void* stream) {
   return sf_slot_attn_planes_ex(planes, batch_stride_rows, q, part_num, part_den, attn_out, attn_batch_stride, B, HW, N, scale, eps, (hipStream_t)stream);
+}
+extern "C" int sf_slot_attn_iter_planes_dense_f32(const void* planes, long long batch_stride_rows, const float* q, float* part_num, float* part_den,
+                                                  float* attn_out, long long attn_batch_stride, int B, int HW, int N, float scale, float eps, void* stream) {
+  return sf_slot_attn_planes_ex(planes, batch_stride_rows, q, part_num, part_den, attn_out, attn_batch_stride, B, HW, N, scale, eps, (hipStream_t)stream,
+                                true);
 }
 
 bool sf_slot_chain_ok(int D, int H, int HW, int N) { return D == SC_D && H == UM_H && HW >= 256 && HW % (SC_NW * SC_TP) == 0 && N >= 1 && N <= 8; }
diff --git a/slotformer_amd/csrc/slot_update_mfma.hip b/slotformer_amd/csrc/slot_update_mfma.hip
--- a/slotformer_amd/csrc/slot_update_mfma.hip
+++ b/slotformer_amd/csrc/slot_update_mfma.hip
@@ -3,6 +3,16 @@
 template <bool NEXT>
 __global__ __launch_bounds__(UM_NT) void sa_slot_update_mfma_kernel(UmArgs a) {
   extern __shared__ __attribute__((aligned(16))) float um_lds[];
+  um_body<NEXT>(a, um_lds, blockIdx.x);
+}
+template <bool NEXT>
+__global__ __launch_bounds__(UM_NT) void sa_slot_update_mfma_io_kernel(UmArgs a, const sf_encode_io* __restrict__ io) {
+  extern __shared__ __attribute__((aligned(16))) float um_lds[];
+  if (a.out2) {
+    a.out2 = io->post + (a.out2 - io->post0);
+    a.out2_bs = io->post_bs;
+  }
+  if (NEXT && a.noise) a.noise = io->noise + (a.noise - io->noise0);
   um_body<NEXT>(a, um_lds, blockIdx.x);
 }
 
@@ -12,7 +22,7 @@
                            const void* gru_hh_p, const float* gru_b_ih, const float* gru_b_hh, const float* ln_g, const float* ln_b,
                            const void* w1_p, const float* b1, const void* w2_p, const float* b2, float* slots_out, float* out2,
                            long long out2_bs, const float* q_ln_g, const float* q_ln_b, const void* q_w_p, float* q_out, int B, int N,
-                           float ln_eps, hipStream_t st, const SfNextStep* next, int p_step) {
+                           float ln_eps, hipStream_t st, const SfNextStep* next, int p_step, const sf_encode_io* io) {
   SF_REQUIRE(part_num && part_den && slots_prev && slots_out && gru_ih_p && gru_hh_p && gru_b_ih && gru_b_hh && ln_g && ln_b && w1_p &&
                  b1 && w2_p && b2, "sf_slot_update_mfma_ex: null pointer");
   SF_REQUIRE(!next || (q_out && next->pm_ln_g && next->pm_ln_b && next->pm_w0_p && next->pm_b0 && next->pm_w2_p && next->pm_b2 && next->kd_w_p &&
@@ -22,8 +32,13 @@
   SF_REQUIRE(N >= 1 && P >= 1 && P <= 64 && (p_step == 1 || (p_step == 2 && P % 2 == 0)), "bad slot shape");
   if (B == 0) return 0;
   static_assert(UM_LDS_NEXT <= 160 * 1024, "slot update: LDS budget");
-  SF_TRY(next ? sf_ensure_dyn_lds((const void*)sa_slot_update_mfma_kernel<true>, (size_t)(UM_LDS_NEXT))
-              : sf_ensure_dyn_lds((const void*)sa_slot_update_mfma_kernel<false>, (size_t)(UM_LDS)));
+  if (io && !out2 && !(next && next->noise)) io = nullptr;
+  if (io)
+    SF_TRY(next ? sf_ensure_dyn_lds((const void*)sa_slot_update_mfma_io_kernel<true>, (size_t)(UM_LDS_NEXT))
+                : sf_ensure_dyn_lds((const void*)sa_slot_update_mfma_io_kernel<false>, (size_t)(UM_LDS)));
+  else
+    SF_TRY(next ? sf_ensure_dyn_lds((const void*)sa_slot_update_mfma_kernel<true>, (size_t)(UM_LDS_NEXT))
+                : sf_ensure_dyn_lds((const void*)sa_slot_update_mfma_kernel<false>, (size_t)(UM_LDS)));
   UmArgs a;
   memset(&a, 0, sizeof(a));
   a.part_num = part_num; a.part_den = part_den; a.P = P / p_step; a.pstep = p_step; a.slots_prev = slots_prev;
@@ -39,7 +54,11 @@
   }
   sf_prof_begin(SF_K_SA_UPDATE, st,
                 2.0 * R * ((double)6 * UM_D * UM_D + 2.0 * UM_D * UM_H + (q_out ? (double)UM_D * UM_D : 0.0) + (next ? 6.0 * UM_D * UM_D : 0.0)));
-  if (next)
+  if (io && next)
+    hipLaunchKernelGGL(sa_slot_update_mfma_io_kernel<true>, dim3((R + UM_ROWS - 1) / UM_ROWS), dim3(UM_NT), UM_LDS_NEXT, st, a, io);
+  else if (io)
+    hipLaunchKernelGGL(sa_slot_update_mfma_io_kernel<false>, dim3((R + UM_ROWS - 1) / UM_ROWS), dim3(UM_NT), UM_LDS, st, a, io);
+  else if (next)
     hipLaunchKernelGGL(sa_slot_update_mfma_kernel<true>, dim3((R + UM_ROWS - 1) / UM_ROWS), dim3(UM_NT), UM_LDS_NEXT, st, a);
   else
     hipLaunchKernelGGL(sa_slot_update_mfma_kernel<false>, dim3((R + UM_ROWS - 1) / UM_ROWS), dim3(UM_NT), UM_LDS, st, a);
diff --git a/slotformer_amd/engine.py b/slotformer_amd/engine.py
--- a/slotformer_amd/engine.py
+++ b/slotformer_amd/engine.py
@@ -389,6 +389,32 @@
     return post, kdist, attn
 
 
+def savi_encode_io_ok(m, B, T):
+    return bool(lib().sf_savi_encode_io_ok(C.byref(encoder_plan(m).struct), int(B), int(T)))
+
+
+def encode_io_set(io, img, noise, post, post_bs, img0, noise0, post0):
+    rec = _lib.sf_encode_io(img, noise, post, int(post_bs), img0, noise0, post0, 0)
+    check(lib().sf_encode_io_set(io.data_ptr(), C.byref(rec), stream()))
+
+
+def savi_encode_io(m, io, img, noise, post, ws_slot=0):
+    _require_inference(m, img)
+    ops._chk(img, noise, post)
+    plan = encoder_plan(m)
+    s = plan.struct
+    B, T = img.shape[:2]
+    if tuple(img.shape[2:]) != (3, s.resolution, s.resolution) or tuple(post.shape) != (B, T, s.num_slots, s.slot_size):
+        raise RuntimeError(f'img must be [B,T,3,{s.resolution},{s.resolution}] and post [B,T,N,D], got {tuple(img.shape)}, {tuple(post.shape)}')
+    if io.dtype != torch.uint8 or io.numel() != C.sizeof(_lib.sf_encode_io) or not io.is_cuda:
+        raise RuntimeError('io must be a uint8 device tensor of sizeof(sf_encode_io) bytes')
+    kdist = torch.empty(B, T, s.num_slots, 2 * s.slot_size, device=img.device, dtype=torch.float32) if s.kd_mode else None
+    ws = workspace_for(img.device, ('enc', ws_slot), lib().sf_savi_encode_batched_workspace_bytes, C.byref(plan.struct), B, T)
+    check(lib().sf_savi_encode_io_f32(C.byref(plan.struct), io.data_ptr(), img.data_ptr(), ptr(noise), post.data_ptr(), ptr(kdist), None, B, T,
+                                      ws.data_ptr(), ws.numel(), stream()))
+    return kdist
+
+
 def savi_chain_ok(m, B, T):
     plan = encoder_plan(m)
     return bool(lib().sf_savi_chain_ok(C.byref(plan.struct), int(B), int(T)))
diff --git a/slotformer_amd/ops.py b/slotformer_amd/ops.py
--- a/slotformer_amd/ops.py
+++ b/slotformer_amd/ops.py
@@ -230,17 +230,17 @@
     return pn, pd, attn
 
 
-def slot_attn_iter_planes(planes, q, eps=1e-6, want_attn=False):
+def slot_attn_iter_planes(planes, q, eps=1e-6, want_attn=False, dense=False):
     _chk(q)
     if not (planes.is_cuda and planes.dtype == torch.bfloat16 and planes.is_contiguous() and planes.shape[-1] == 256):
         raise RuntimeError('slot_attn_iter_planes needs contiguous bfloat16 rows [B, HW, 256] on a HIP device')
     B, HW, _ = planes.shape
-    N, P = q.shape[1], HW // 256
+    N, P = q.shape[1], HW // (512 if dense else 256)
     pn = torch.empty(B, P, N, 128, device=q.device, dtype=torch.float32)
     pd = torch.empty(B, P, N, device=q.device, dtype=torch.float32)
     attn = torch.empty(B, N, HW, device=q.device, dtype=torch.float32) if want_attn else None
-    check(lib().sf_slot_attn_iter_planes_f32(planes.data_ptr(), HW, ptr(q), ptr(pn), ptr(pd), ptr(attn), N * HW, B, HW, N, 128.0**-0.5, eps,
-                                             stream()))
+    fn = lib().sf_slot_attn_iter_planes_dense_f32 if dense else lib().sf_slot_attn_iter_planes_f32
+    check(fn(planes.data_ptr(), HW, ptr(q), ptr(pn), ptr(pd), ptr(attn), N * HW, B, HW, N, 128.0**-0.5, eps, stream()))
     return pn, pd, attn
 
 
diff --git a/slotformer_amd/pipeline.py b/slotformer_amd/pipeline.py
--- a/slotformer_amd/pipeline.py
+++ b/slotformer_amd/pipeline.py
@@ -216,6 +216,7 @@
         self.use_graph = bool(use_graph)
         self.encode_graph = bool(int(os.environ.get('SF_PIPE_ENCODE_GRAPH', '1'))) if encode_graph is None else bool(encode_graph)
         self._enc_graphs = {}
+        self.encode_staged = [0, 0, 0]
         self.encode_fork = bool(encode_fork)
         self.drain_latency_form = self.G * self.B < 128
         self._key = ('pipe', id(self))
@@ -503,6 +504,22 @@
         noise = engine.kernel_noise(self.savi, noise, hi - lo, self.T, self.dev)
         if self.encode_graph:
             eg = self._encode_graph_for(lane, hi - lo, 0 if feat_pre is None else feat_pre.shape[0], img.shape[-1], noise is not None)
+            if eg['io'] is not None:
+                out = dst[lo:hi, :self.T]
+                direct = [self._io_direct(img, eg['img']), self._io_direct(noise, eg['noise']), self._io_direct(out, eg['post'], any_batch_stride=True)]
+                if not direct[0]:
+                    eg['img'].copy_(img)
+                if not direct[1]:
+                    eg['noise'].copy_(noise)
+                for i, d in enumerate(direct):
+                    self.encode_staged[i] += not d
+                at = [(t if d else own) for t, own, d in zip((img, noise, out), (eg['img'], eg['noise'], eg['post']), direct)]
+                engine.encode_io_set(eg['io'], at[0].data_ptr(), None if noise is None else at[1].data_ptr(), at[2].data_ptr(), at[2].stride(0),
+                                     eg['img'].data_ptr(), None if noise is None else eg['noise'].data_ptr(), eg['post'].data_ptr())
+                eg['graph'].replay()
+                if not direct[2]:
+                    out.copy_(eg['post'])
+                return
             eg['img'].copy_(img)
             if noise is not None:
                 eg['noise'].copy_(noise)
@@ -531,6 +548,16 @@
             return LANE0_WORDS_3 if lane == 0 else LANE1_WORDS_3
         return [0xffffffff] * 8
 
+    @staticmethod
+    def _io_direct(t, like, any_batch_stride=False):
+        if like is None:
+            return True
+        if not (torch.is_tensor(t) and t.device == like.device and t.dtype == torch.float32 and t.shape == like.shape and t.data_ptr() % 16 == 0):
+            return False
+        if t.is_contiguous():
+            return True
+        return any_batch_stride and t.stride()[1:] == like.stride()[1:] and t.stride(0) >= like.stride(0) and t.stride(0) % 4 == 0
+
     def _encode_graph_for(self, lane, nv, k, res, with_noise):
         key = (lane, nv, k, res, with_noise)
         eg = self._enc_graphs.get(key)
@@ -539,7 +566,17 @@
             cl = list(self.savi.enc_channels)[-1]
             eg = {'img': torch.zeros(nv, self.T, 3, res, res, device=self.dev),
                   'noise': torch.zeros(nv, self.T, self.N, self.D, device=self.dev) if with_noise else None,
-                  'feat': torch.zeros(k, nv, 64 * 64, cl, device=self.dev) if k else None}
+                  'feat': torch.zeros(k, nv, 64 * 64, cl, device=self.dev) if k else None, 'io': None}
+            use_io = k == 0 and not self.encode_fork and engine.savi_encode_io_ok(self.savi, nv, self.T)
+            if use_io:
+                eg['io'] = torch.zeros(64, device=self.dev, dtype=torch.uint8)
+                eg['post'] = torch.zeros(nv, self.T, self.N, self.D, device=self.dev)
+
+            def encode_once():
+                if use_io:
+                    engine.savi_encode_io(self.savi, eg['io'], eg['img'], eg['noise'], eg['post'], ws_slot=ws)
+                    return eg['post']
+                return engine.savi_encode(self.savi, eg['img'], noise=eg['noise'], feat_pre=eg['feat'], ws_slot=ws, side_stream=side2)[0]
             ws = self._key + ('encg', ) + key
             side = torch.cuda.Stream(device=self.dev)
             side.wait_stream(cur)
@@ -552,11 +589,15 @@
                 self._lib.sf_stream_set_cus(C.c_void_p(side.cuda_stream), lane_cus)
             try:
                 with torch.cuda.stream(side):
-                    engine.savi_encode(self.savi, eg['img'], noise=eg['noise'], feat_pre=eg['feat'], ws_slot=ws, side_stream=side2)
+                    if use_io:
+                        engine.encode_io_set(eg['io'], eg['img'].data_ptr(), None if not with_noise else eg['noise'].data_ptr(), eg['post'].data_ptr(),
+                                             eg['post'].stride(0), eg['img'].data_ptr(), None if not with_noise else eg['noise'].data_ptr(),
+                                             eg['post'].data_ptr())
+                    encode_once()
                     side.synchronize()
                     g = torch.cuda.CUDAGraph()
                     with _lib.CAPTURE_GATE, torch.cuda.graph(g, stream=side, capture_error_mode='thread_local'):
-                        post, _, _ = engine.savi_encode(self.savi, eg['img'], noise=eg['noise'], feat_pre=eg['feat'], ws_slot=ws, side_stream=side2)
+                        post = encode_once()
                 cur.wait_stream(side)
             finally:
                 if lane_cus:
diff --git a/slotformer_amd/switches.py b/slotformer_amd/switches.py
--- a/slotformer_amd/switches.py
+++ b/slotformer_amd/switches.py
@@ -31,6 +31,10 @@
     'pixel_tok': ('sf_set_pixel_tok', 'sf_get_pixel_tok', None, 1, "the per-pixel chain of the encoder in its pixel-stationary form (0: the tile kernels; another summation order)"),
 }
 
+SET_OR_READ = {
+    'encode_dense_records': ('sf_encode_dense_records', 1, "the encode without device work its slots do not need: dense partial records out of the Slot-Attention kernel on bf16 planes (0: interleaved zero records; the same bits)"),
+}
+
 
 def check_environment(environ=None):
     environ = os.environ if environ is None else environ
```

Result: no change. 727,200 (median of 6 runs) (+0.2%).
